# CV-Project2025/Project-NeRF

Hardware: AMD Instinct MI355X
Metric: train rays/sec + 800x800 render FPS, NeRF-Synthetic Lego; PSNR parity (higher is better)
Workload: dtype bf16; 1 GPU; Part 2 vanilla NeRF train step (L10/L4 Fourier, 8x256 skip-4 MLP, view 128), batch sampling included; rays_per_gpu=4096, samples_per_ray=64, global_rays=4096, parallelism=ray-dp1, weights=random init (seed 0), frames=100 x 800x800 RGBA resident in HBM (uniform noise)

## Files before the change

### include/nerf_hip.h

```cpp
#ifndef NERF_HIP_H
#define NERF_HIP_H

#include <stddef.h>
#include <stdint.h>

#ifdef __cplusplus
extern "C" {
#endif

#define NERF_OK 0
#define NERF_EINVAL (-22)
#define NERF_ELAUNCH (-5)
#define NERF_ENOSYS (-38)

#define NERF_ABI_VERSION 11

typedef void* nerf_stream_t;

const char* nerf_last_error(void);
int nerf_abi_version(void);

int nerf_set_option(const char* name, int value);
int nerf_get_option(const char* name, int* value_out);

int nerf_sample_rays(const float* rays_o, const float* rays_d, const float* u,
                     int64_t n_rays, int n_samples, float near_plane, float far_plane,
                     float* z_out, float* pts_out, float* dirs_out, nerf_stream_t stream);

int nerf_gather_rays(const float* images, const float* poses, const int64_t* img_idx, const int64_t* pix_y,
                     const int64_t* pix_x, int64_t batch, int n_images, int H, int W, float focal,
                     float scene_scale, float* rays_o, float* rays_d, float* rgba, nerf_stream_t stream);

int nerf_gather_batch(const float* images, const float* poses, const int64_t* flat_idx, int64_t batch, int n_images,
                      int H, int W, float focal, float scene_scale, const float* bg, float* rays_o, float* rays_d,
                      float* rgba, float* target, nerf_stream_t stream);

int nerf_train_batch(const float* images, const float* poses, int n_images, int H, int W, float focal,
                     float scene_scale, const float* bg, uint64_t seed, uint64_t counter, int64_t batch,
                     int n_samples, float near_plane, float far_plane, int perturb, float* rays_o, float* rays_d,
                     float* rgba, float* target, float* z_out, nerf_stream_t stream);

int nerf_train_batch_shard(const float* images, const float* poses, int n_images, int H, int W, float focal,
                     float scene_scale, const float* bg, uint64_t seed, uint64_t counter, int64_t first_ray, int64_t batch,
                     int n_samples, float near_plane, float far_plane, int perturb, float* rays_o, float* rays_d,
                     float* rgba, float* target, float* z_out, nerf_stream_t stream);

int nerf_active_mask(const float* pts, int64_t n, const uint8_t* binary_grid, int resolution,
                     float bound, uint8_t* mask_out, int64_t* idx_out, nerf_stream_t stream);

int nerf_sample_compact(const float* rays_o, const float* rays_d, const float* u, int64_t n_rays,
                        int n_samples, float near_plane, float far_plane, const uint8_t* binary_grid,
                        int resolution, float bound, float* z_out, int* slot_of_sample, float* pts_compact,
                        float* dirs_compact, unsigned* active_count, nerf_stream_t stream);
int nerf_sample_compact_jitter(const float* rays_o, const float* rays_d, uint64_t seed, uint64_t counter,
                               int64_t n_rays, int n_samples, float near_plane, float far_plane,
                               const uint8_t* binary_grid, int resolution, float bound, float* z_out,
                               int* slot_of_sample, float* pts_compact, float* dirs_compact,
                               unsigned* active_count, nerf_stream_t stream);
int nerf_sample_compact_jitter_shard(const float* rays_o, const float* rays_d, uint64_t seed, uint64_t counter,
                                     int64_t first_ray, int64_t n_rays, int n_samples, float near_plane, float far_plane,
                                     const uint8_t* binary_grid, int resolution, float bound, float* z_out,
                                     int* slot_of_sample, float* pts_compact, float* dirs_compact,
                                     unsigned* active_count, nerf_stream_t stream);
#define NERF_COMPACT_CHAIN_WORDS 40
int nerf_sample_compact_jitter_chain(const float* rays_o, const float* rays_d, uint64_t seed, uint64_t counter,
                                     int64_t first_ray, int64_t n_rays, int n_samples, float near_plane, float far_plane,
                                     const uint8_t* binary_grid, int resolution, float bound, float* z_out,
                                     int* slot_of_sample, float* pts_compact, float* dirs_compact,
                                     unsigned* chain_state, int turn, unsigned* count_host, unsigned seq, nerf_stream_t stream);

int nerf_train_batch_compact(const float* images, const float* poses, int n_images, int H, int W, float focal,
                             float scene_scale, const float* bg, uint64_t seed, uint64_t counter, int64_t first_ray,
                             int64_t batch, int n_samples, float near_plane, float far_plane,
                             const uint8_t* binary_grid, int resolution, float bound, float* rays_o, float* rays_d,
                             float* rgba, float* target, float* z_out, int* slot_of_sample, float* pts_compact,
                             float* dirs_compact, unsigned* active_count, nerf_stream_t stream);
int nerf_train_batch_compact_chain(const float* images, const float* poses, int n_images, int H, int W, float focal,
                                   float scene_scale, const float* bg, uint64_t seed, uint64_t counter, int64_t first_ray,
                                   int64_t batch, int n_samples, float near_plane, float far_plane,
                                   const uint8_t* binary_grid, int resolution, float bound, float* rays_o, float* rays_d,
                                   float* rgba, float* target, float* z_out, int* slot_of_sample, float* pts_compact,
                                   float* dirs_compact, unsigned* chain_state, int turn, unsigned* count_host, unsigned seq,
                                   nerf_stream_t stream);

size_t nerf_sample_compact_ordered_scratch_bytes(int64_t n_rays, int n_samples);
int nerf_sample_compact_ordered(const float* rays_o, const float* rays_d, const float* u, int draw, uint64_t seed, uint64_t counter,
                                int64_t first_ray, int64_t n_rays, int n_samples, float near_plane, float far_plane,
                                const uint8_t* binary_grid, int resolution, float bound, float* z_out, int* slot_of_sample,
                                float* pts_compact, float* dirs_compact, unsigned* active_count, void* scratch,
                                size_t scratch_bytes, nerf_stream_t stream);

int nerf_sample_pdf(const float* z_coarse, const float* weights, const float* u, int64_t n_rays,
                    int n_coarse, int n_fine, float* z_out, nerf_stream_t stream);

int nerf_grid_lattice(float bound, int resolution, float* pts_out, nerf_stream_t stream);
int nerf_grid_update(const float* sigma, float* grid, uint8_t* binary_grid, int64_t n_cells,
                     float decay, int dynamic, float threshold, unsigned long long* active_count,
                     nerf_stream_t stream);

int nerf_fourier_encode(const float* x, int64_t n, int dim, int n_freq, float* out,
                        nerf_stream_t stream);

int nerf_composite_fwd(const float* rgb, const float* sigma, const float* z, const float* rays_d,
                       const float* bg, int64_t bg_rows, const float* extra,
                       int64_t n_rays, int n_samples,
                       float* out_rgb, float* out_depth, float* out_acc,
                       float* extra_map, float* weights_out, nerf_stream_t stream);

int nerf_composite_bwd(const float* rgb, const float* sigma, const float* z, const float* rays_d,
                       const float* bg, int64_t bg_rows, const float* extra,
                       const float* g_rgb, const float* g_depth, const float* g_acc,
                       const float* g_extra, int64_t n_rays, int n_samples,
                       float* d_rgb, float* d_sigma, float* d_extra, nerf_stream_t stream);

int nerf_composite_fwd_indexed(const float* rgb_compact, const float* sigma_compact, const int* slot_of_sample,
                               const float* z, const float* rays_d, const float* bg, int64_t bg_rows,
                               int64_t n_rays, int n_samples, float* out_rgb, float* out_depth,
                               float* out_acc, nerf_stream_t stream);
int nerf_composite_bwd_indexed(const float* rgb_compact, const float* sigma_compact, const int* slot_of_sample,
                               const float* z, const float* rays_d, const float* bg, int64_t bg_rows,
                               const float* g_rgb, const float* g_depth, const float* g_acc, int64_t n_rays,
                               int n_samples, float* d_rgb_compact, float* d_sigma_compact,
                               nerf_stream_t stream);

#define NERF_MLP_PARAM_COUNT 595844

size_t nerf_mlp_packed_bytes(void);
int nerf_mlp_pack(const float* params_f32, void* packed, nerf_stream_t stream);
int nerf_mlp_pack_streams(const float* params_f32, void* packed, int which, nerf_stream_t stream);

size_t nerf_mlp_stash_bytes(int64_t n);
int nerf_mlp_fwd(const void* packed, const float* rays_o, const float* rays_d, const float* z,
                 int64_t n, int n_samples, float* rgb, float* sigma, void* stash,
                 nerf_stream_t stream);

int nerf_mlp_fwd_encoded(const void* packed, const float* x_enc, const float* d_enc, int64_t n, float* rgb,
                         float* sigma, void* stash, nerf_stream_t stream);

size_t nerf_mlp_bwd_workspace_bytes(int64_t n);
int nerf_mlp_bwd(const void* packed, const void* stash, const float* rgb, const float* sigma,
                 const float* d_rgb, const float* d_sigma, int64_t n, float* grads_f32,
                 void* workspace, nerf_stream_t stream);
int nerf_mlp_bwd_dgrad(const void* packed, const void* stash, const float* rgb, const float* sigma,
                       const float* d_rgb, const float* d_sigma, int64_t n, void* workspace,
                       nerf_stream_t stream);
int nerf_mlp_bwd_dgrad_ex(const void* packed, const void* stash, const float* rgb, const float* sigma,
                          const float* d_rgb, const float* d_sigma, int64_t n, void* workspace,
                          const float* amax_dev, nerf_stream_t stream);
int64_t nerf_mlp_wgrad_part_split(void);
int nerf_mlp_bwd_wgrad_part(const void* stash, const void* workspace, int64_t n, float* grads_f32, int part,
                            nerf_stream_t stream);
int nerf_mlp_bwd_wgrad(const void* stash, const void* workspace, int64_t n, float* grads_f32,
                       nerf_stream_t stream);

int nerf_hash_encode_fwd(const float* pts, int64_t n, const float* table, int n_levels,
                         const float* scale_host, const unsigned* res_host, const unsigned* size_host,
                         const unsigned* offset_host, const unsigned* dense_host, float bound,
                         float* out_f32, void* out_nat_bf16, unsigned* idx_out, nerf_stream_t stream);
int nerf_hash_encode_fwd_f16(const float* pts, int64_t n, const void* table_f16, int n_levels,
                         const float* scale_host, const unsigned* res_host, const unsigned* size_host,
                         const unsigned* offset_host, const unsigned* dense_host, float bound,
                         float* out_f32, void* out_nat_bf16, nerf_stream_t stream);
int nerf_hash_encode_fwd_nat(const float* pts, int64_t n, const float* table_f32, const void* table_f16, int n_levels,
                             const float* scale_host, const unsigned* res_host, const unsigned* size_host,
                             const unsigned* offset_host, const unsigned* dense_host, float bound,
                             void* out_nat, int nat_dtype, nerf_stream_t stream);
int nerf_hash_encode_fwd_nat_tables(const float* pts, int64_t n, const void* tables_f16, int n_tables, int64_t table_stride,
                                    int n_levels, const float* scale_host, const unsigned* res_host, const unsigned* size_host,
                                    const unsigned* offset_host, const unsigned* dense_host, float bound, void* out_nat,
                                    int64_t out_stride_bytes, int nat_dtype, nerf_stream_t stream);
int nerf_f32_to_f16(const float* src, void* dst_f16, int64_t n, nerf_stream_t stream);
int nerf_hash_encode_bwd(const float* pts, int64_t n, int n_levels, const float* scale_host,
                         const unsigned* res_host, const unsigned* size_host, const unsigned* offset_host,
                         const unsigned* dense_host, float bound, const float* d_feat, float* d_table,
                         nerf_stream_t stream);
int nerf_hash_encode_bwd_levels(const float* pts, int64_t n, int n_levels, const float* scale_host,
                         const unsigned* res_host, const unsigned* size_host, const unsigned* offset_host,
                         const unsigned* dense_host, float bound, const float* d_feat, float* d_table, int first_level, int end_level,
                         nerf_stream_t stream);
size_t nerf_hash_encode_bwd_workspace_bytes(int64_t n, int n_levels);
int nerf_hash_encode_bwd_ws(const float* pts, int64_t n, int n_levels, const float* scale_host,
                         const unsigned* res_host, const unsigned* size_host, const unsigned* offset_host,
                         const unsigned* dense_host, float bound, const float* d_feat, float* d_table, int first_level, int end_level,
                         void* workspace, size_t workspace_bytes, nerf_stream_t stream);
int nerf_hash_encode_bwd_ws_store(const float* pts, int64_t n, int n_levels, const float* scale_host,
                                  const unsigned* res_host, const unsigned* size_host, const unsigned* offset_host,
                                  const unsigned* dense_host, float bound, const float* d_feat, float* d_table,
                                  int first_level, int end_level, void* workspace, size_t workspace_bytes,
                                  nerf_stream_t stream);
size_t nerf_hash_encode_bwd_tables_workspace_bytes(int64_t n, int n_levels, int n_tables);
int nerf_hash_encode_bwd_ws_store_tables(const float* pts, int64_t n, int n_tables, int64_t table_stride, int n_levels,
                                         const float* scale_host, const unsigned* res_host, const unsigned* size_host,
                                         const unsigned* offset_host, const unsigned* dense_host, float bound,
                                         const float* d_feat, int64_t dfeat_stride, float* d_table, void* workspace,
                                         size_t workspace_bytes, nerf_stream_t stream);
int nerf_hash_encode_bwd_ws_store_tables_spec(const float* pts, int64_t n, int n_tables, int64_t table_stride, int n_levels,
                                              const float* scale_host, const unsigned* res_host, const unsigned* size_host,
                                              const unsigned* offset_host, const unsigned* dense_host, float bound,
                                              const float* d_feat, int64_t dfeat_stride, float* d_table, void* workspace,
                                              size_t workspace_bytes, void* status_host, nerf_stream_t stream);
int nerf_hash_encode_fwd_f16_hist(const float* pts, int64_t n, const void* table_f16, int n_levels,
                                  const float* scale_host, const unsigned* res_host, const unsigned* size_host,
                                  const unsigned* offset_host, const unsigned* dense_host, float bound,
                                  void* out_nat_bf16, void* bwd_workspace, size_t bwd_workspace_bytes, nerf_stream_t stream);
#define NERF_AMAX_WORDS 32
int nerf_hash_encode_bwd_ws_slots(void* workspace, int64_t n, int n_levels, void** amax_bits_out, void** grad_lm_out);
int nerf_hash_encode_bwd_ws_store_precounted(const float* pts, int64_t n, int n_levels, const float* scale_host,
                                             const unsigned* res_host, const unsigned* size_host,
                                             const unsigned* offset_host, const unsigned* dense_host, float bound,
                                             float* d_table, void* workspace, size_t workspace_bytes, nerf_stream_t stream);
int nerf_hash_encode_bwd_spec_begin(void* workspace, nerf_stream_t stream);
int nerf_hash_encode_bwd_ws_store_spec(const float* pts, int64_t n, int n_levels, const float* scale_host,
                                       const unsigned* res_host, const unsigned* size_host, const unsigned* offset_host,
                                       const unsigned* dense_host, float bound, const float* d_feat, float* d_table, void* workspace,
                                       size_t workspace_bytes, void* status_host, nerf_stream_t stream);
int nerf_imlp_bwd_amax(const void* packed, void* workspace, const float* rgb, const float* sigma, const float* d_rgb,
                       const float* d_sigma, int64_t n, float* grads_f32, float* d_feat, void* amax_bits, nerf_stream_t stream);
const void* nerf_hash_encode_bwd_spec_status(const void* workspace);

int nerf_hash_encode_bwd_input(const float* pts, int64_t n, const float* table, int n_levels,
                               const float* scale_host, const unsigned* res_host, const unsigned* size_host,
                               const unsigned* offset_host, const unsigned* dense_host, float bound,
                               const float* d_feat, float* d_pts, nerf_stream_t stream);
int nerf_hash_encode_bwd_input_f16(const float* pts, int64_t n, const void* table_f16, int n_levels,
                                   const float* scale_host, const unsigned* res_host, const unsigned* size_host,
                                   const unsigned* offset_host, const unsigned* dense_host, float bound,
                                   const float* d_feat, float* d_pts, nerf_stream_t stream);
int nerf_hash_encode_bwd_input_f16_accum(const float* pts, int64_t n, const void* table_f16, int n_levels,
                                         const float* scale_host, const unsigned* res_host, const unsigned* size_host,
                                         const unsigned* offset_host, const unsigned* dense_host, float bound,
                                         const float* d_feat, float* d_pts, nerf_stream_t stream);
int nerf_hash_encode_bwd_input_lm_f16(const float* pts, int64_t n, const void* table_f16, int n_levels,
                                      const float* scale_host, const unsigned* res_host, const unsigned* size_host,
                                      const unsigned* offset_host, const unsigned* dense_host, float bound,
                                      const void* grad_lm, float* d_pts, int accumulate, nerf_stream_t stream);


size_t nerf_imlp_packed_bytes(void);
size_t nerf_imlp_workspace_bytes(int64_t n);
size_t nerf_imlp_hash_operand_offset(int64_t n);
int nerf_imlp_pack(const float* params_f32, void* packed, nerf_stream_t stream);
int nerf_imlp_fwd(const void* packed, void* workspace, const float* dirs, int64_t n, float* rgb,
                  float* sigma, int train, nerf_stream_t stream);
int nerf_imlp_fwd_encoded(const void* packed, void* workspace, const float* x_enc, const float* d_enc, int64_t n,
                          float* rgb, float* sigma, int train, nerf_stream_t stream);
int nerf_imlp_bwd(const void* packed, void* workspace, const float* rgb, const float* sigma,
                  const float* d_rgb, const float* d_sigma, int64_t n, float* grads_f32,
                  float* d_feat, nerf_stream_t stream);
int nerf_imlp_bwd_lm(const void* packed, void* workspace, const float* rgb, const float* sigma,
                     const float* d_rgb, const float* d_sigma, int64_t n, float* grads_f32,
                     void* grad_lm, void* amax_bits, nerf_stream_t stream);

size_t nerf_render_rays_workspace_bytes(int64_t chunk_rays, int n_samples);
int nerf_render_rays_fwd(const void* packed, const float* rays_o, const float* rays_d, int64_t n_rays,
                         int n_samples, float near_plane, float far_plane, const float* bg, int64_t bg_rows,
                         int64_t chunk_rays, void* workspace, float* out_rgb, float* out_depth, float* out_acc,
                         nerf_stream_t stream);

size_t nerf_instant_render_workspace_bytes(int64_t chunk_rays, int n_samples);
int nerf_instant_render_rays_fwd(const void* imlp_packed, const float* table_f32, const void* table_f16, int n_levels,
                                 const float* scale_host, const unsigned* res_host, const unsigned* size_host,
                                 const unsigned* offset_host, const unsigned* dense_host, float hash_bound,
                                 const uint8_t* binary_grid, int grid_resolution, float grid_bound,
                                 const float* rays_o, const float* rays_d, int64_t n_rays, int n_samples,
                                 float near_plane, float far_plane, const float* bg, int64_t bg_rows,
                                 int64_t chunk_rays, void* workspace, float* out_rgb, float* out_depth, float* out_acc,
                                 nerf_stream_t stream);

size_t nerf_render_rays_grid_workspace_bytes(int64_t chunk_rays, int n_samples);
int nerf_render_rays_grid_fwd(const void* packed, const uint8_t* binary_grid, int grid_resolution, float grid_bound,
                              const float* rays_o, const float* rays_d, int64_t n_rays, int n_samples,
                              float near_plane, float far_plane, const float* bg, int64_t bg_rows,
                              int64_t chunk_rays, void* workspace, float* out_rgb, float* out_depth, float* out_acc,
                              nerf_stream_t stream);

#define NERF_SUM_WS_FLOATS 12288
int nerf_composite_mse_bwd(const float* rgb, const float* sigma, const int* slot_of_sample, const float* z,
                           const float* rays_d, const float* bg, int64_t bg_rows, const float* target,
                           float loss_weight, int64_t n_rays, int n_samples, float* pred_out, float* loss_accum,
                           float* d_rgb, float* d_sigma, float* amax_accum, float* sum_ws, nerf_stream_t stream);
int nerf_composite_mse_reg_bwd(const float* rgb, const float* sigma, const int* slot_of_sample, const float* z,
                               const float* rays_d, const float* bg, int64_t bg_rows, const float* target,
                               float loss_weight, const float* extra, float reg_weight, int64_t n_rays, int n_samples,
                               float* pred_out, float* extra_map, float* loss_accum, float* reg_accum, float* d_rgb,
                               float* d_sigma, float* d_extra, float* sum_ws, nerf_stream_t stream);

int nerf_adam_step(float* params, const float* grads, float* exp_avg, float* exp_avg_sq,
                   int64_t n, int step, float lr, float beta1, float beta2, float eps,
                   float weight_decay, const float* grad_scale_dev, nerf_stream_t stream);

#define NERF_NORMSQ_WS_FLOATS 4136
int nerf_tv_normsq(const float* params, float* grads, int64_t n, float tv_weight, float grad_scale,
                   float* normsq_dev, nerf_stream_t stream);
int nerf_tv_normsq_accum(const float* params, float* grads, int64_t n, float tv_weight, float grad_scale,
                         float* normsq_dev, nerf_stream_t stream);
int nerf_tv_normsq_accum_tables(const float* params, float* grads, int64_t n, int n_tables, float tv_weight, float grad_scale,
                                float* normsq_dev, nerf_stream_t stream);
int nerf_adamw_clip_step(float* params, const float* grads, float* exp_avg, float* exp_avg_sq, int64_t n,
                         int step, float lr, float beta1, float beta2, float eps, float weight_decay,
                         const float* normsq_dev, float max_norm, float grad_scale, nerf_stream_t stream);
int nerf_adamw_clip_step_shadow(float* params, const float* grads, float* exp_avg, float* exp_avg_sq, int64_t n,
                         int step, float lr, float beta1, float beta2, float eps, float weight_decay,
                         const float* normsq_dev, float max_norm, float grad_scale, void* params_f16_out, nerf_stream_t stream);

size_t nerf_tv_codes_bytes(int64_t n);
int nerf_tv_normsq_codes(const float* params, const float* grads, int64_t n, int n_tables, float tv_weight, float grad_scale,
                         float* normsq_dev, int accumulate, void* tv_codes, nerf_stream_t stream);
int nerf_adamw_clip_step_tv(float* params, const float* grads, float* exp_avg, float* exp_avg_sq, int64_t n, int step, float lr,
                            float beta1, float beta2, float eps, float weight_decay, const float* normsq_dev, float max_norm,
                            float grad_scale, const void* tv_codes, int64_t tv_split, float tv_weight_lo, int64_t seg_lo,
                            float tv_weight_hi, int64_t seg_hi, int64_t lr_split, float lr_hi, void* params_f16_out,
                            nerf_stream_t stream);

int nerf_tv_normsq_codes_piece(const float* params, const float* grads, int64_t n, int64_t table_elems, int halo, float tv_weight,
                               float grad_scale, float* normsq_dev, int accumulate, void* tv_codes, nerf_stream_t stream);
int nerf_adamw_clip_step_tv_piece(float* params, const float* grads, float* exp_avg, float* exp_avg_sq, int64_t n, int step, float lr,
                                  float beta1, float beta2, float eps, float weight_decay, const float* normsq_dev, float max_norm,
                                  float grad_scale, const void* tv_codes, float tv_weight, int64_t table_elems, int halo_lo,
                                  void* params_f16_out, nerf_stream_t stream);

int nerf_clip_adamw_small(float* params, float* grads, float* exp_avg, float* exp_avg_sq, int64_t n, int step, float lr, float beta1,
                          float beta2, float eps, float weight_decay, float max_norm, float grad_scale, float* normsq_out,
                          int zero_grads, nerf_stream_t stream);

int64_t nerf_p4_param_count(void);
size_t nerf_p4_packed_bytes(void);
size_t nerf_p4_workspace_bytes(int64_t n);
size_t nerf_p4_infer_workspace_bytes(int64_t n);
size_t nerf_p4_workspace_offset(int64_t n, int which);
int nerf_p4_pack(const float* params_f32, void* packed, nerf_stream_t stream);
int nerf_p4_sample_inputs(const int* slot_of_sample, const float* pts_compact, const float* ray_times, int64_t n_rays,
                          int n_samples, float coord_noise_std, float time_noise_std, uint64_t seed, uint64_t counter,
                          int64_t first_ray, float* x_deform, float* t_deform, nerf_stream_t stream);
int nerf_p4_deform_fwd(const void* packed, const float* params_f32, void* workspace, const float* pts, const float* t_deform,
                       const float* blend, int64_t n, float* delta_x, float* x_canonical, int train, nerf_stream_t stream);
int nerf_p4_canon_fwd(const void* packed, void* workspace, const float* t_deform, const float* dirs, int64_t n, float* rgb,
                      float* sigma, int train, nerf_stream_t stream);
int nerf_p4_canon_bwd(const void* packed, void* workspace, const float* rgb, const float* sigma, const float* d_rgb,
                      const float* d_sigma, int64_t n, float* grads_f32, void* amax_bits, void* grad_lm, nerf_stream_t stream);
int nerf_p4_deform_bwd(const void* packed, const float* params_f32, void* workspace, const float* d_delta_x, int64_t n,
                       float* grads_f32, void* amax_bits, void* grad_lm, nerf_stream_t stream);

int64_t nerf_p3_deform_param_count(void);
size_t nerf_p3_deform_packed_bytes(void);
size_t nerf_p3_deform_workspace_bytes(int64_t n);
int nerf_p3_deform_pack(const float* params_f32, void* packed, nerf_stream_t stream);
int nerf_p3_deform_fwd(const void* packed, void* workspace, const float* x_code, const float* pts, const float* t_deform,
                       int64_t n, float* delta_x, float* x_canonical, int train, nerf_stream_t stream);
int nerf_p3_deform_bwd(const void* packed, void* workspace, const float* d_delta_x, int64_t n, float* grads_f32,
                       nerf_stream_t stream);

int64_t nerf_p3_canon_param_count(int time_dim);
size_t nerf_p3_canon_packed_bytes(void);
size_t nerf_p3_canon_workspace_bytes(int64_t n);
int nerf_p3_canon_pack(const float* params_f32, int time_dim, void* packed, nerf_stream_t stream);
int nerf_p3_canon_fwd(const void* packed, void* workspace, const float* x, const float* t, const float* dirs, int64_t n,
                      float* rgb, float* sigma, int train, nerf_stream_t stream);
int nerf_p3_canon_bwd(const void* packed, void* workspace, const float* x, const float* rgb, const float* sigma,
                      const float* d_rgb, const float* d_sigma, int64_t n, int time_dim, float* grads_f32, float* d_x,
                      nerf_stream_t stream);

int64_t nerf_p1_param_count(int L_embed, int use_pe, int hidden, int layers);
size_t nerf_p1_packed_bytes(int L_embed, int use_pe, int hidden, int layers);
// ... 37 lines not shown
```

### project-nerf_amd/_lib.py

```python
import ctypes
import os

_HERE = os.path.dirname(os.path.abspath(__file__))
LIB_PATH = os.path.join(_HERE, "libnerf_hip.so")

c_f32p = ctypes.c_void_p
c_ptr = ctypes.c_void_p
i64 = ctypes.c_int64
i32 = ctypes.c_int
f32 = ctypes.c_float
size_t = ctypes.c_size_t

PROTOTYPES = {
    "nerf_last_error": (ctypes.c_char_p, []),
    "nerf_abi_version": (i32, []),
    "nerf_set_option": (i32, [ctypes.c_char_p, i32]),
    "nerf_get_option": (i32, [ctypes.c_char_p, ctypes.POINTER(i32)]),
    "nerf_sample_rays": (i32, [c_ptr, c_ptr, c_ptr, i64, i32, f32, f32, c_ptr, c_ptr, c_ptr, c_ptr]),
    "nerf_gather_rays": (i32, [c_ptr, c_ptr, c_ptr, c_ptr, c_ptr, i64, i32, i32, i32, f32, f32, c_ptr, c_ptr, c_ptr, c_ptr]),
    "nerf_gather_batch": (i32, [c_ptr, c_ptr, c_ptr, i64, i32, i32, i32, f32, f32, c_ptr, c_ptr, c_ptr, c_ptr, c_ptr, c_ptr]),
    "nerf_train_batch": (i32, [c_ptr, c_ptr, i32, i32, i32, f32, f32, c_ptr, ctypes.c_uint64, ctypes.c_uint64, i64, i32, f32, f32,
                               i32, c_ptr, c_ptr, c_ptr, c_ptr, c_ptr, c_ptr]),
    "nerf_train_batch_shard": (i32, [c_ptr, c_ptr, i32, i32, i32, f32, f32, c_ptr, ctypes.c_uint64, ctypes.c_uint64, i64, i64, i32, f32, f32,
                                     i32, c_ptr, c_ptr, c_ptr, c_ptr, c_ptr, c_ptr]),
    "nerf_active_mask": (i32, [c_ptr, i64, c_ptr, i32, f32, c_ptr, c_ptr, c_ptr]),
    "nerf_sample_compact": (i32, [c_ptr, c_ptr, c_ptr, i64, i32, f32, f32, c_ptr, i32, f32, c_ptr, c_ptr, c_ptr, c_ptr, c_ptr, c_ptr]),
    "nerf_sample_compact_jitter": (i32, [c_ptr, c_ptr, ctypes.c_uint64, ctypes.c_uint64, i64, i32, f32, f32, c_ptr, i32, f32,
                                         c_ptr, c_ptr, c_ptr, c_ptr, c_ptr, c_ptr]),
    "nerf_sample_compact_jitter_shard": (i32, [c_ptr, c_ptr, ctypes.c_uint64, ctypes.c_uint64, i64, i64, i32, f32, f32, c_ptr, i32, f32,
                                               c_ptr, c_ptr, c_ptr, c_ptr, c_ptr, c_ptr]),
    "nerf_sample_compact_jitter_chain": (i32, [c_ptr, c_ptr, ctypes.c_uint64, ctypes.c_uint64, i64, i64, i32, f32, f32, c_ptr, i32, f32,
                                               c_ptr, c_ptr, c_ptr, c_ptr, c_ptr, i32, c_ptr, ctypes.c_uint32, c_ptr]),
    "nerf_train_batch_compact": (i32, [c_ptr, c_ptr, i32, i32, i32, f32, f32, c_ptr, ctypes.c_uint64, ctypes.c_uint64, i64, i64, i32, f32, f32,
                                       c_ptr, i32, f32, c_ptr, c_ptr, c_ptr, c_ptr, c_ptr, c_ptr, c_ptr, c_ptr, c_ptr, c_ptr]),
    "nerf_train_batch_compact_chain": (i32, [c_ptr, c_ptr, i32, i32, i32, f32, f32, c_ptr, ctypes.c_uint64, ctypes.c_uint64, i64, i64, i32, f32,
                                             f32, c_ptr, i32, f32, c_ptr, c_ptr, c_ptr, c_ptr, c_ptr, c_ptr, c_ptr, c_ptr, c_ptr, i32, c_ptr,
                                             ctypes.c_uint32, c_ptr]),
    "nerf_composite_fwd_indexed": (i32, [c_ptr, c_ptr, c_ptr, c_ptr, c_ptr, c_ptr, i64, i64, i32, c_ptr, c_ptr, c_ptr, c_ptr]),
    "nerf_composite_bwd_indexed": (i32, [c_ptr, c_ptr, c_ptr, c_ptr, c_ptr, c_ptr, i64, c_ptr, c_ptr, c_ptr, i64, i32, c_ptr, c_ptr, c_ptr]),
    "nerf_sample_pdf": (i32, [c_ptr, c_ptr, c_ptr, i64, i32, i32, c_ptr, c_ptr]),
    "nerf_grid_lattice": (i32, [f32, i32, c_ptr, c_ptr]),
    "nerf_grid_update": (i32, [c_ptr, c_ptr, c_ptr, i64, f32, i32, f32, c_ptr, c_ptr]),
    "nerf_fourier_encode": (i32, [c_ptr, i64, i32, i32, c_ptr, c_ptr]),
    "nerf_composite_fwd": (i32, [c_ptr, c_ptr, c_ptr, c_ptr, c_ptr, i64, c_ptr, i64, i32,
                                 c_ptr, c_ptr, c_ptr, c_ptr, c_ptr, c_ptr]),
    "nerf_composite_bwd": (i32, [c_ptr, c_ptr, c_ptr, c_ptr, c_ptr, i64, c_ptr, c_ptr, c_ptr, c_ptr,
                                 c_ptr, i64, i32, c_ptr, c_ptr, c_ptr, c_ptr]),
    "nerf_render_rays_workspace_bytes": (size_t, [i64, i32]),
    "nerf_render_rays_fwd": (i32, [c_ptr, c_ptr, c_ptr, i64, i32, f32, f32, c_ptr, i64, i64, c_ptr, c_ptr, c_ptr, c_ptr, c_ptr]),
    "nerf_instant_render_workspace_bytes": (size_t, [i64, i32]),
    "nerf_instant_render_rays_fwd": (i32, [c_ptr, c_ptr, c_ptr, i32, c_ptr, c_ptr, c_ptr, c_ptr, c_ptr, f32, c_ptr, i32, f32, c_ptr, c_ptr, i64, i32,
                                           f32, f32, c_ptr, i64, i64, c_ptr, c_ptr, c_ptr, c_ptr, c_ptr]),
    "nerf_render_rays_grid_workspace_bytes": (size_t, [i64, i32]),
    "nerf_render_rays_grid_fwd": (i32, [c_ptr, c_ptr, i32, f32, c_ptr, c_ptr, i64, i32, f32, f32, c_ptr, i64, i64, c_ptr, c_ptr, c_ptr, c_ptr,
                                        c_ptr]),
    "nerf_mlp_packed_bytes": (size_t, []),
    "nerf_mlp_pack": (i32, [c_ptr, c_ptr, c_ptr]),
    "nerf_mlp_pack_streams": (i32, [c_ptr, c_ptr, i32, c_ptr]),
    "nerf_mlp_stash_bytes": (size_t, [i64]),
    "nerf_mlp_fwd": (i32, [c_ptr, c_ptr, c_ptr, c_ptr, i64, i32, c_ptr, c_ptr, c_ptr, c_ptr]),
    "nerf_mlp_fwd_encoded": (i32, [c_ptr, c_ptr, c_ptr, i64, c_ptr, c_ptr, c_ptr, c_ptr]),
    "nerf_mlp_bwd_workspace_bytes": (size_t, [i64]),
    "nerf_mlp_bwd": (i32, [c_ptr, c_ptr, c_ptr, c_ptr, c_ptr, c_ptr, i64, c_ptr, c_ptr, c_ptr]),
    "nerf_mlp_bwd_dgrad": (i32, [c_ptr, c_ptr, c_ptr, c_ptr, c_ptr, c_ptr, i64, c_ptr, c_ptr]),
    "nerf_mlp_bwd_wgrad": (i32, [c_ptr, c_ptr, i64, c_ptr, c_ptr]),
    "nerf_mlp_bwd_dgrad_ex": (i32, [c_ptr, c_ptr, c_ptr, c_ptr, c_ptr, c_ptr, i64, c_ptr, c_ptr, c_ptr]),
    "nerf_composite_mse_bwd": (i32, [c_ptr, c_ptr, c_ptr, c_ptr, c_ptr, c_ptr, i64, c_ptr, f32, i64, i32, c_ptr, c_ptr,
                                     c_ptr, c_ptr, c_ptr, c_ptr, c_ptr]),
    "nerf_mlp_wgrad_part_split": (i64, []),
    "nerf_mlp_bwd_wgrad_part": (i32, [c_ptr, c_ptr, i64, c_ptr, i32, c_ptr]),
    "nerf_hash_encode_fwd": (i32, [c_ptr, i64, c_ptr, i32, c_ptr, c_ptr, c_ptr, c_ptr, c_ptr, f32, c_ptr, c_ptr, c_ptr, c_ptr]),
    "nerf_hash_encode_fwd_f16": (i32, [c_ptr, i64, c_ptr, i32, c_ptr, c_ptr, c_ptr, c_ptr, c_ptr, f32, c_ptr, c_ptr, c_ptr]),
    "nerf_hash_encode_fwd_nat": (i32, [c_ptr, i64, c_ptr, c_ptr, i32, c_ptr, c_ptr, c_ptr, c_ptr, c_ptr, f32, c_ptr, i32, c_ptr]),
    "nerf_hash_encode_fwd_nat_tables": (i32, [c_ptr, i64, c_ptr, i32, i64, i32, c_ptr, c_ptr, c_ptr, c_ptr, c_ptr, f32, c_ptr, i64, i32, c_ptr]),
    "nerf_f32_to_f16": (i32, [c_ptr, c_ptr, i64, c_ptr]),
    "nerf_hash_encode_bwd": (i32, [c_ptr, i64, i32, c_ptr, c_ptr, c_ptr, c_ptr, c_ptr, f32, c_ptr, c_ptr, c_ptr]),
    "nerf_hash_encode_bwd_levels": (i32, [c_ptr, i64, i32, c_ptr, c_ptr, c_ptr, c_ptr, c_ptr, f32, c_ptr, c_ptr, i32, i32, c_ptr]),
    "nerf_hash_encode_bwd_workspace_bytes": (size_t, [i64, i32]),
    "nerf_hash_encode_bwd_ws": (i32, [c_ptr, i64, i32, c_ptr, c_ptr, c_ptr, c_ptr, c_ptr, f32, c_ptr, c_ptr, i32, i32, c_ptr, size_t, c_ptr]),
    "nerf_hash_encode_bwd_ws_store": (i32, [c_ptr, i64, i32, c_ptr, c_ptr, c_ptr, c_ptr, c_ptr, f32, c_ptr, c_ptr, i32, i32, c_ptr, size_t, c_ptr]),
    "nerf_hash_encode_bwd_tables_workspace_bytes": (size_t, [i64, i32, i32]),
    "nerf_hash_encode_bwd_ws_store_tables": (i32, [c_ptr, i64, i32, i64, i32, c_ptr, c_ptr, c_ptr, c_ptr, c_ptr, f32, c_ptr, i64, c_ptr, c_ptr, size_t, c_ptr]),
    "nerf_hash_encode_bwd_ws_store_tables_spec": (i32, [c_ptr, i64, i32, i64, i32, c_ptr, c_ptr, c_ptr, c_ptr, c_ptr, f32, c_ptr, i64, c_ptr, c_ptr, size_t,
                                                        c_ptr, c_ptr]),
    "nerf_hash_encode_fwd_f16_hist": (i32, [c_ptr, i64, c_ptr, i32, c_ptr, c_ptr, c_ptr, c_ptr, c_ptr, f32, c_ptr, c_ptr, size_t, c_ptr]),
    "nerf_hash_encode_bwd_ws_slots": (i32, [c_ptr, i64, i32, ctypes.POINTER(c_ptr), ctypes.POINTER(c_ptr)]),
    "nerf_hash_encode_bwd_ws_store_precounted": (i32, [c_ptr, i64, i32, c_ptr, c_ptr, c_ptr, c_ptr, c_ptr, f32, c_ptr, c_ptr, size_t, c_ptr]),
    "nerf_hash_encode_bwd_spec_begin": (i32, [c_ptr, c_ptr]),
    "nerf_hash_encode_bwd_ws_store_spec": (i32, [c_ptr, i64, i32, c_ptr, c_ptr, c_ptr, c_ptr, c_ptr, f32, c_ptr, c_ptr, c_ptr, size_t, c_ptr, c_ptr]),
    "nerf_imlp_bwd_amax": (i32, [c_ptr, c_ptr, c_ptr, c_ptr, c_ptr, c_ptr, i64, c_ptr, c_ptr, c_ptr, c_ptr]),
    "nerf_hash_encode_bwd_spec_status": (c_ptr, [c_ptr]),
    "nerf_imlp_bwd_lm": (i32, [c_ptr, c_ptr, c_ptr, c_ptr, c_ptr, c_ptr, i64, c_ptr, c_ptr, c_ptr, c_ptr]),
    "nerf_hash_encode_bwd_input": (i32, [c_ptr, i64, c_ptr, i32, c_ptr, c_ptr, c_ptr, c_ptr, c_ptr, f32, c_ptr, c_ptr, c_ptr]),
    "nerf_hash_encode_bwd_input_f16": (i32, [c_ptr, i64, c_ptr, i32, c_ptr, c_ptr, c_ptr, c_ptr, c_ptr, f32, c_ptr, c_ptr, c_ptr]),
    "nerf_hash_encode_bwd_input_f16_accum": (i32, [c_ptr, i64, c_ptr, i32, c_ptr, c_ptr, c_ptr, c_ptr, c_ptr, f32, c_ptr, c_ptr, c_ptr]),
    "nerf_hash_encode_bwd_input_lm_f16": (i32, [c_ptr, i64, c_ptr, i32, c_ptr, c_ptr, c_ptr, c_ptr, c_ptr, f32, c_ptr, c_ptr, i32, c_ptr]),
    "nerf_imlp_packed_bytes": (size_t, []),
    "nerf_imlp_workspace_bytes": (size_t, [i64]),
    "nerf_imlp_hash_operand_offset": (size_t, [i64]),
    "nerf_imlp_pack": (i32, [c_ptr, c_ptr, c_ptr]),
    "nerf_imlp_fwd": (i32, [c_ptr, c_ptr, c_ptr, i64, c_ptr, c_ptr, i32, c_ptr]),
    "nerf_imlp_fwd_encoded": (i32, [c_ptr, c_ptr, c_ptr, c_ptr, i64, c_ptr, c_ptr, i32, c_ptr]),
    "nerf_imlp_bwd": (i32, [c_ptr, c_ptr, c_ptr, c_ptr, c_ptr, c_ptr, i64, c_ptr, c_ptr, c_ptr]),
    "nerf_adam_step": (i32, [c_ptr, c_ptr, c_ptr, c_ptr, i64, i32, f32, f32, f32, f32, f32, c_ptr, c_ptr]),
    "nerf_tv_normsq": (i32, [c_ptr, c_ptr, i64, f32, f32, c_ptr, c_ptr]),
    "nerf_tv_normsq_accum": (i32, [c_ptr, c_ptr, i64, f32, f32, c_ptr, c_ptr]),
    "nerf_tv_normsq_accum_tables": (i32, [c_ptr, c_ptr, i64, i32, f32, f32, c_ptr, c_ptr]),
    "nerf_composite_mse_reg_bwd": (i32, [c_ptr, c_ptr, c_ptr, c_ptr, c_ptr, c_ptr, i64, c_ptr, f32, c_ptr, f32, i64, i32, c_ptr, c_ptr,
                                         c_ptr, c_ptr, c_ptr, c_ptr, c_ptr, c_ptr, c_ptr]),
    "nerf_sample_compact_ordered_scratch_bytes": (size_t, [i64, i32]),
    "nerf_sample_compact_ordered": (i32, [c_ptr, c_ptr, c_ptr, i32, ctypes.c_uint64, ctypes.c_uint64, i64, i64, i32, f32, f32, c_ptr, i32, f32,
                                          c_ptr, c_ptr, c_ptr, c_ptr, c_ptr, c_ptr, size_t, c_ptr]),
    "nerf_p4_param_count": (i64, []),
    "nerf_p4_packed_bytes": (size_t, []),
    "nerf_p4_workspace_bytes": (size_t, [i64]),
    "nerf_p4_infer_workspace_bytes": (size_t, [i64]),
    "nerf_p4_workspace_offset": (size_t, [i64, i32]),
    "nerf_p4_pack": (i32, [c_ptr, c_ptr, c_ptr]),
    "nerf_p4_sample_inputs": (i32, [c_ptr, c_ptr, c_ptr, i64, i32, f32, f32, ctypes.c_uint64, ctypes.c_uint64, i64, c_ptr, c_ptr, c_ptr]),
    "nerf_p4_deform_fwd": (i32, [c_ptr, c_ptr, c_ptr, c_ptr, c_ptr, c_ptr, i64, c_ptr, c_ptr, i32, c_ptr]),
    "nerf_p4_canon_fwd": (i32, [c_ptr, c_ptr, c_ptr, c_ptr, i64, c_ptr, c_ptr, i32, c_ptr]),
    "nerf_p4_canon_bwd": (i32, [c_ptr, c_ptr, c_ptr, c_ptr, c_ptr, c_ptr, i64, c_ptr, c_ptr, c_ptr, c_ptr]),
    "nerf_p4_deform_bwd": (i32, [c_ptr, c_ptr, c_ptr, c_ptr, i64, c_ptr, c_ptr, c_ptr, c_ptr]),
    "nerf_p3_deform_param_count": (i64, []),
    "nerf_p3_deform_packed_bytes": (size_t, []),
    "nerf_p3_deform_workspace_bytes": (size_t, [i64]),
    "nerf_p3_deform_pack": (i32, [c_ptr, c_ptr, c_ptr]),
    "nerf_p3_deform_fwd": (i32, [c_ptr, c_ptr, c_ptr, c_ptr, c_ptr, i64, c_ptr, c_ptr, i32, c_ptr]),
    "nerf_p3_deform_bwd": (i32, [c_ptr, c_ptr, c_ptr, i64, c_ptr, c_ptr]),
    "nerf_p3_canon_param_count": (i64, [i32]),
    "nerf_p3_canon_packed_bytes": (size_t, []),
    "nerf_p3_canon_workspace_bytes": (size_t, [i64]),
    "nerf_p3_canon_pack": (i32, [c_ptr, i32, c_ptr, c_ptr]),
    "nerf_p3_canon_fwd": (i32, [c_ptr, c_ptr, c_ptr, c_ptr, c_ptr, i64, c_ptr, c_ptr, i32, c_ptr]),
    "nerf_p3_canon_bwd": (i32, [c_ptr, c_ptr, c_ptr, c_ptr, c_ptr, c_ptr, c_ptr, i64, i32, c_ptr, c_ptr, c_ptr]),
    "nerf_p1_param_count": (i64, [i32, i32, i32, i32]),
    "nerf_p1_packed_bytes": (size_t, [i32, i32, i32, i32]),
    "nerf_p1_workspace_bytes": (size_t, [i64, i32, i32, i32, i32]),
    "nerf_p1_pack": (i32, [c_ptr, i32, i32, i32, i32, c_ptr, c_ptr]),
    "nerf_p1_fwd": (i32, [c_ptr, c_ptr, i64, i32, i32, i32, i32, c_ptr, c_ptr]),
    "nerf_p1_fwd_loss_bwd": (i32, [c_ptr, c_ptr, c_ptr, c_ptr, c_ptr, i64, i32, i32, i32, i32, c_ptr, c_ptr, c_ptr]),
    "nerf_p2_param_count": (i64, [i32] * 6),
    "nerf_p2_packed_bytes": (size_t, [i32] * 6),
    "nerf_p2_workspace_bytes": (size_t, [i64] + [i32] * 6),
    "nerf_p2_pack": (i32, [c_ptr] + [i32] * 6 + [c_ptr, c_ptr]),
    "nerf_p2_fwd": (i32, [c_ptr, c_ptr, c_ptr, c_ptr, i64, i32] + [i32] * 6 + [c_ptr, c_ptr, c_ptr]),
    "nerf_p2_fwd_train": (i32, [c_ptr, c_ptr, c_ptr, c_ptr, c_ptr, i64, i32] + [i32] * 6 + [c_ptr, c_ptr, c_ptr]),
    "nerf_p2_bwd": (i32, [c_ptr, c_ptr, c_ptr, c_ptr, c_ptr, c_ptr, i64] + [i32] * 6 + [c_ptr, c_ptr]),
    "nerf_imlp_shape_param_count": (i64, [i32] * 3),
    "nerf_imlp_shape_packed_bytes": (size_t, [i32] * 3),
    "nerf_imlp_shape_workspace_bytes": (size_t, [i64] + [i32] * 3),
    "nerf_imlp_shape_hash_operand_offset": (size_t, [i64] + [i32] * 3),
    "nerf_imlp_shape_pack": (i32, [c_ptr] + [i32] * 3 + [c_ptr, c_ptr]),
    "nerf_imlp_shape_fwd": (i32, [c_ptr, c_ptr, c_ptr, i64] + [i32] * 3 + [c_ptr, c_ptr, i32, c_ptr]),
    "nerf_imlp_shape_bwd": (i32, [c_ptr, c_ptr, c_ptr, c_ptr, c_ptr, c_ptr, i64] + [i32] * 3 + [c_ptr, c_ptr, c_ptr]),
    "nerf_tv_codes_bytes": (size_t, [i64]),
    "nerf_tv_normsq_codes": (i32, [c_ptr, c_ptr, i64, i32, f32, f32, c_ptr, i32, c_ptr, c_ptr]),
    "nerf_clip_adamw_small": (i32, [c_ptr, c_ptr, c_ptr, c_ptr, i64, i32, f32, f32, f32, f32, f32, f32, f32, c_ptr, i32, c_ptr]),
    "nerf_adamw_clip_step_tv": (i32, [c_ptr, c_ptr, c_ptr, c_ptr, i64, i32, f32, f32, f32, f32, f32, c_ptr, f32, f32, c_ptr, i64, f32, i64,
                                      f32, i64, i64, f32, c_ptr, c_ptr]),
    "nerf_tv_normsq_codes_piece": (i32, [c_ptr, c_ptr, i64, i64, i32, f32, f32, c_ptr, i32, c_ptr, c_ptr]),
    "nerf_adamw_clip_step_tv_piece": (i32, [c_ptr, c_ptr, c_ptr, c_ptr, i64, i32, f32, f32, f32, f32, f32, c_ptr, f32, f32, c_ptr, f32, i64, i32,
                                            c_ptr, c_ptr]),
    "nerf_adamw_clip_step": (i32, [c_ptr, c_ptr, c_ptr, c_ptr, i64, i32, f32, f32, f32, f32, f32, c_ptr, f32, f32, c_ptr]),
    "nerf_adamw_clip_step_shadow": (i32, [c_ptr, c_ptr, c_ptr, c_ptr, i64, i32, f32, f32, f32, f32, f32, c_ptr, f32, f32, c_ptr, c_ptr]),
}

ABI_VERSION = 11

_lib = None


class NerfHipError(RuntimeError):
    pass


def load():
    global _lib
    if _lib is not None:
        return _lib
    if not os.path.exists(LIB_PATH):
        raise NerfHipError(
            f"{LIB_PATH} not found: build it with `python project-nerf_amd/build.py` "
            "(hipcc --offload-arch=gfx950).  There is no fallback path.")
    import torch
    lib = ctypes.CDLL(LIB_PATH, mode=ctypes.RTLD_GLOBAL)
    for name, (res, args) in PROTOTYPES.items():
        fn = getattr(lib, name)
        fn.restype = res
        fn.argtypes = args
    if lib.nerf_abi_version() != ABI_VERSION:
        raise NerfHipError(f"ABI version mismatch: {LIB_PATH} reports {lib.nerf_abi_version()}, this binding was written against "
                           f"{ABI_VERSION} (rebuild with `python project-nerf_amd/build.py`)")
    _lib = lib
    return lib


NORMSQ_WS_FLOATS = 4136
COMPACT_CHAIN_WORDS = 40
SUM_WS_FLOATS = 12288


def set_option(name: str, value: int) -> None:
    check(load().nerf_set_option(name.encode(), int(value)), f"nerf_set_option({name})")


def get_option(name: str) -> int:
    out = i32(0)
    check(load().nerf_get_option(name.encode(), ctypes.byref(out)), f"nerf_get_option({name})")
    return out.value


def check(code, what):
    if code != 0:
        msg = load().nerf_last_error().decode("utf-8", "replace")
        raise NerfHipError(f"{what} failed ({code}): {msg}")
```

### project-nerf_amd/csrc/adam.hip

```cpp
#include "common.h"

namespace nerf {

typedef float f4 __attribute__((ext_vector_type(4)));

__device__ __forceinline__ void adam_update(float& p, float g, float& m, float& v, float lr, float beta1, float beta2,
                                            float eps, float wd, float inv_bc1, float inv_sqrt_bc2) {
  float pi = p;
  if (wd != 0.0f) pi *= (1.0f - lr * wd);
  const float mi = beta1 * m + (1.0f - beta1) * g;
  const float vi = beta2 * v + (1.0f - beta2) * g * g;
  m = mi;
  v = vi;
  p = pi - (lr * inv_bc1) * (mi / (sqrtf(vi) * inv_sqrt_bc2 + eps));
}

template <bool VEC>
__device__ __forceinline__ void adam_sweep(float* __restrict__ p, const float* __restrict__ g, float* __restrict__ m,
                                           float* __restrict__ v, int64_t n, float gs, float lr, float beta1, float beta2,
                                           float eps, float wd, float inv_bc1, float inv_sqrt_bc2, _Float16* __restrict__ shadow = nullptr) {
  const int64_t tid = blockIdx.x * (int64_t)blockDim.x + threadIdx.x, stride = (int64_t)gridDim.x * blockDim.x;
  const int64_t n4 = VEC ? n / 4 : 0;
  for (int64_t i = tid; i < n4; i += stride) {
    f4 pp = reinterpret_cast<f4*>(p)[i], mm = reinterpret_cast<f4*>(m)[i], vv = reinterpret_cast<f4*>(v)[i];
    const f4 gg = reinterpret_cast<const f4*>(g)[i];
#pragma unroll
    for (int e = 0; e < 4; ++e) {
      float pe = pp[e], me = mm[e], ve = vv[e];
      adam_update(pe, gg[e] * gs, me, ve, lr, beta1, beta2, eps, wd, inv_bc1, inv_sqrt_bc2);
      pp[e] = pe; mm[e] = me; vv[e] = ve;
    }
    reinterpret_cast<f4*>(m)[i] = mm;
    reinterpret_cast<f4*>(v)[i] = vv;
    reinterpret_cast<f4*>(p)[i] = pp;
    if (shadow != nullptr) {
      typedef _Float16 h4 __attribute__((ext_vector_type(4)));
      h4 hh = {(_Float16)pp[0], (_Float16)pp[1], (_Float16)pp[2], (_Float16)pp[3]};
      reinterpret_cast<h4*>(shadow)[i] = hh;
    }
  }
  for (int64_t i = 4 * n4 + tid; i < n; i += stride) {
    adam_update(p[i], g[i] * gs, m[i], v[i], lr, beta1, beta2, eps, wd, inv_bc1, inv_sqrt_bc2);
    if (shadow != nullptr) shadow[i] = (_Float16)p[i];
  }
}

template <bool VEC>
__global__ void __launch_bounds__(256)
adam_kernel(float* __restrict__ p, const float* __restrict__ g, float* __restrict__ m,
            float* __restrict__ v, int64_t n, float lr, float beta1, float beta2, float eps, float wd,
            float inv_bc1, float inv_sqrt_bc2, const float* __restrict__ grad_scale) {
  adam_sweep<VEC>(p, g, m, v, n, grad_scale ? *grad_scale : 1.0f, lr, beta1, beta2, eps, wd, inv_bc1, inv_sqrt_bc2);
}

__host__ inline bool aligned16(const void* a, const void* b, const void* c, const void* d) {
  return (((uintptr_t)a | (uintptr_t)b | (uintptr_t)c | (uintptr_t)d) & 15) == 0;
}

}

extern "C" int nerf_adam_step(float* params, const float* grads, float* exp_avg, float* exp_avg_sq,
                              int64_t n, int step, float lr, float beta1, float beta2, float eps,
                              float weight_decay, const float* grad_scale_dev, nerf_stream_t stream) {
  NERF_REQUIRE(n >= 0 && step >= 1, "nerf_adam_step: n=%lld step=%d", (long long)n, step);
  if (n == 0) return NERF_OK;
  NERF_REQUIRE(params && grads && exp_avg && exp_avg_sq, "nerf_adam_step: NULL pointer");
  const double bc1 = 1.0 - pow((double)beta1, step), bc2 = 1.0 - pow((double)beta2, step);
  int64_t blocks = (n / 4 + 255) / 256 + 1;
  if (blocks > 2048) blocks = 2048;
  if (nerf::aligned16(params, grads, exp_avg, exp_avg_sq))
    hipLaunchKernelGGL(nerf::adam_kernel<true>, dim3((int)blocks), dim3(256), 0, nerf::as_stream(stream), params,
                       grads, exp_avg, exp_avg_sq, n, lr, beta1, beta2, eps, weight_decay,
                       (float)(1.0 / bc1), (float)(1.0 / sqrt(bc2)), grad_scale_dev);
  else
    hipLaunchKernelGGL(nerf::adam_kernel<false>, dim3((int)blocks), dim3(256), 0, nerf::as_stream(stream), params,
                       grads, exp_avg, exp_avg_sq, n, lr, beta1, beta2, eps, weight_decay,
                       (float)(1.0 / bc1), (float)(1.0 / sqrt(bc2)), grad_scale_dev);
  return nerf::check_launch("nerf_adam_step");
}

namespace nerf {

__device__ __forceinline__ float sgn(float x) { return (x > 0.0f) - (x < 0.0f); }

__device__ __forceinline__ float tv_term(float prev, float cur, float next, bool has_prev, bool has_next) {
  float t = 0.0f;
  if (has_prev) t += sgn(cur - prev);
  if (has_next) t -= sgn(next - cur);
  return t;
}

template <bool VEC>
__global__ void __launch_bounds__(256)
tv_normsq_kernel(const float* __restrict__ p, float* __restrict__ g, int64_t n, float tv_scale, float grad_scale,
                 float* __restrict__ normsq, int64_t seg) {
  auto starts = [seg](int64_t e) { return e == 0 || e == seg || e == 2 * seg || e == 3 * seg; };
  const bool rewrite = tv_scale != 0.0f || grad_scale != 1.0f;
  float local = 0.0f;
// ... 477 lines not shown
```

### project-nerf_amd/csrc/api.cpp

```cpp
#include <stdlib.h>
#include <string.h>
#include <mutex>
#include "common.h"

namespace nerf {
static thread_local char g_err[512] = "";

int fail(int code, const char* fmt, ...) {
  va_list ap;
  va_start(ap, fmt);
  vsnprintf(g_err, sizeof(g_err), fmt, ap);
  va_end(ap);
  return code;
}

struct OptionSlot { const char* name; const char* env; int Options::*field; };
static const OptionSlot kSlots[] = {
    {"chain_legacy", "NERF_CHAIN_LEGACY", &Options::chain_legacy},
    {"fwd_cycles", "NERF_FWD_CYCLES", &Options::fwd_cycles},
    {"wgrad_overhead", "NERF_WGRAD_OVH", &Options::wgrad_overhead},
    {"wgrad_bw_x16", "NERF_WGRAD_BW", &Options::wgrad_bw_x16},
    {"wgrad_fixed", "NERF_WGRAD_FIXED", &Options::wgrad_fixed},
    {"wgrad_debug", "NERF_WGRAD_DEBUG", &Options::wgrad_debug},
    {"wgrad_small_span", "NERF_WGRAD_SMALL_SPAN", &Options::wgrad_small_span},
    {"wgrad_small_cap", "NERF_WGRAD_SMALL_CAP", &Options::wgrad_small_cap},
    {"wgrad_only", "NERF_WGRAD_ONLY", &Options::wgrad_only},
    {"hash_bwd_only_level", "NERF_HASH_BWD_ONLY_LEVEL", &Options::hash_bwd_only_level},
    {"hash_bwd_atomic", "NERF_HASH_BWD_ATOMIC", &Options::hash_bwd_atomic},
    {"wgrad_atomic", "NERF_WGRAD_ATOMIC", &Options::wgrad_atomic},
    {"wgrad_k16", "NERF_WGRAD_K16", &Options::wgrad_k16},
    {"wgrad_big_only", "NERF_WGRAD_BIG_ONLY", &Options::wgrad_big_only},
    {"infer_shape32", "NERF_INFER_SHAPE32", &Options::infer_shape32},
    {"infer64", "NERF_INFER64", &Options::infer64},
    {"stash_fp8", "NERF_STASH_FP8", &Options::stash_fp8},
    {"chain_grid", "NERF_CHAIN_GRID", &Options::chain_grid},
    {"wgrad_grid", "NERF_WGRAD_GRID", &Options::wgrad_grid},
    {"hash_fwd_lds_kb", "NERF_HASH_FWD_LDS_KB", &Options::hash_fwd_lds_kb},
    {"hash_xcd", "NERF_HASH_XCD", &Options::hash_xcd},
    {"composite_wgs_per_cu", "NERF_COMPOSITE_WGS", &Options::composite_wgs_per_cu},
    {"deterministic", "NERF_DETERMINISTIC", &Options::deterministic},
    {"tv_blocks", "NERF_TV_BLOCKS", &Options::tv_blocks},
};

Options& options() {
  static Options o;
  static std::once_flag once;
  std::call_once(once, [] {
    for (const OptionSlot& s : kSlots)
      if (const char* v = getenv(s.env)) o.*(s.field) = (*v == 0) ? 1 : atoi(v);
  });
  return o;
}

namespace {
constexpr int kMaxDevices = 64, kMaxKernels = 64;
struct DeviceFacts {
  int n_cu = 0;
  int n_kernels = 0;
  const void* kernels[kMaxKernels];
};
DeviceFacts g_dev[kMaxDevices];
std::mutex g_dev_mutex;
}

int device_cu_count(int* n_cu) {
  int dev = 0;
  if (hipGetDevice(&dev) != hipSuccess || dev < 0 || dev >= kMaxDevices) return fail(NERF_ELAUNCH, "cannot query the current device");
  std::lock_guard<std::mutex> lock(g_dev_mutex);
  if (g_dev[dev].n_cu == 0) {
    hipDeviceProp_t prop;
    if (hipGetDeviceProperties(&prop, dev) != hipSuccess) return fail(NERF_ELAUNCH, "cannot query device %d", dev);
    g_dev[dev].n_cu = prop.multiProcessorCount;
  }
  *n_cu = g_dev[dev].n_cu;
  return NERF_OK;
}

int ensure_dynamic_lds(const void* kernel, int bytes, const char* what) {
  int dev = 0;
  if (hipGetDevice(&dev) != hipSuccess || dev < 0 || dev >= kMaxDevices) return fail(NERF_ELAUNCH, "cannot query the current device");
  std::lock_guard<std::mutex> lock(g_dev_mutex);
  DeviceFacts& d = g_dev[dev];
  for (int i = 0; i < d.n_kernels; ++i)
    if (d.kernels[i] == kernel) return NERF_OK;
  if (hipFuncSetAttribute(kernel, hipFuncAttributeMaxDynamicSharedMemorySize, bytes) != hipSuccess)
    return fail(NERF_ELAUNCH, "%s: cannot raise the dynamic LDS limit to %d on device %d", what, bytes, dev);
  if (d.n_kernels < kMaxKernels) d.kernels[d.n_kernels++] = kernel;
  return NERF_OK;
}
}

extern "C" const char* nerf_last_error(void) { return nerf::g_err; }
extern "C" int nerf_abi_version(void) { return NERF_ABI_VERSION; }

extern "C" int nerf_set_option(const char* name, int value) {
  NERF_REQUIRE(name != nullptr, "nerf_set_option: NULL name");
  for (const nerf::OptionSlot& s : nerf::kSlots)
    if (strcmp(s.name, name) == 0) {
      nerf::options().*(s.field) = value;
      return NERF_OK;
    }
  return nerf::fail(NERF_EINVAL, "nerf_set_option: unknown option '%s'", name);
}

extern "C" int nerf_get_option(const char* name, int* value) {
  NERF_REQUIRE(name != nullptr && value != nullptr, "nerf_get_option: NULL argument");
  for (const nerf::OptionSlot& s : nerf::kSlots)
    if (strcmp(s.name, name) == 0) {
      *value = nerf::options().*(s.field);
      return NERF_OK;
    }
  return nerf::fail(NERF_EINVAL, "nerf_get_option: unknown option '%s'", name);
// ... 2 lines not shown
```

### project-nerf_amd/csrc/common.h

```cpp
#pragma once
#include <hip/hip_runtime.h>
#include <stdarg.h>
#include <stdint.h>
#include <stdio.h>
#include "../../include/nerf_hip.h"

namespace nerf {

constexpr int kWave = 64;

int fail(int code, const char* fmt, ...);

inline int check_launch(const char* what) {
  hipError_t e = hipGetLastError();
  if (e != hipSuccess) return fail(NERF_ELAUNCH, "%s: %s", what, hipGetErrorString(e));
  return NERF_OK;
}

inline hipStream_t as_stream(nerf_stream_t s) { return reinterpret_cast<hipStream_t>(s); }

struct Options {
  int chain_legacy = 0;
  int fwd_cycles = 0;
  int wgrad_overhead = 98304;
  int wgrad_bw_x16 = 192;
  int wgrad_fixed = 2000;
  int wgrad_debug = 0;
  int wgrad_small_span = 32;
  int wgrad_small_cap = 3;
  int wgrad_only = -1;
  int hash_bwd_only_level = -1;
  int wgrad_big_only = 0;
  int wgrad_k16 = 0;
  int wgrad_atomic = 0;
  int hash_bwd_atomic = 0;
  int infer_shape32 = 0;
  int infer64 = 1;
  int stash_fp8 = 0;
  int chain_grid = 0;
  int wgrad_grid = 0;
  int composite_wgs_per_cu = 2;
  int hash_xcd = 1;
  int hash_fwd_lds_kb = 36;
  int tv_blocks = 0;
  int deterministic = 0;
};
Options& options();

int device_cu_count(int* n_cu);
int ensure_dynamic_lds(const void* kernel, int bytes, const char* what);

int hash_fwd_counted(const float* pts, const unsigned* count, int64_t capacity, const float* table_f32, const void* table_f16,
                     int n_levels, const float* scale_host, const unsigned* res_host, const unsigned* size_host,
                     const unsigned* offset_host, const unsigned* dense_host, float bound, void* out_nat, nerf_stream_t stream);
int imlp_fwd_counted(const void* packed, const void* hash_nat, const float* dirs, const unsigned* count, int64_t capacity, float* rgb,
                     float* sigma, nerf_stream_t stream);
int mlp_fwd_counted(const void* packed, const float* pts, const float* dirs, const unsigned* count, int64_t capacity, float* rgb,
                    float* sigma, nerf_stream_t stream);

#define NERF_REQUIRE(cond, ...) \
  do {                          \
    if (!(cond)) return ::nerf::fail(NERF_EINVAL, __VA_ARGS__); \
  } while (0)

__device__ __forceinline__ uint32_t squares32(uint64_t ctr, uint64_t key) {
  uint64_t x = ctr * key, y = x, z = y + key;
  x = x * x + y; x = (x >> 32) | (x << 32);
  x = x * x + z; x = (x >> 32) | (x << 32);
  x = x * x + y; x = (x >> 32) | (x << 32);
  return (uint32_t)((x * x + z) >> 32);
}

inline uint64_t squares_key(uint64_t seed) {
  uint64_t key = seed + 0x9E3779B97F4A7C15ull;
  key = (key ^ (key >> 30)) * 0xBF58476D1CE4E5B9ull;
  key = (key ^ (key >> 27)) * 0x94D049BB133111EBull;
  return (key ^ (key >> 31)) | 1ull;
}
__device__ __forceinline__ float squares_uniform(uint64_t counter, uint64_t index, uint64_t key) {
  return (float)(squares32((counter << 40) + index, key) >> 8) * 5.9604644775390625e-08f;
}

__device__ __forceinline__ float mul_rn(float a, float b) {
#pragma clang fp contract(off)
  return a * b;
}
__device__ __forceinline__ float add_rn(float a, float b) {
#pragma clang fp contract(off)
  return a + b;
}
__device__ __forceinline__ float sub_rn(float a, float b) {
#pragma clang fp contract(off)
  return a - b;
}

template <int N>
__device__ __forceinline__ float dpp_row_shr(float v, float identity) {
  return __builtin_bit_cast(float, __builtin_amdgcn_update_dpp(__builtin_bit_cast(int, identity),
                                                              __builtin_bit_cast(int, v),
                                                              0x110 + N, 0xF, 0xF, false));
}
template <int N>
__device__ __forceinline__ float dpp_row_shl(float v, float identity) {
  return __builtin_bit_cast(float, __builtin_amdgcn_update_dpp(__builtin_bit_cast(int, identity),
                                                              __builtin_bit_cast(int, v),
                                                              0x100 + N, 0xF, 0xF, false));
}
__device__ __forceinline__ float lane_read(float v, int lane) {
  return __builtin_bit_cast(float, __builtin_amdgcn_readlane(__builtin_bit_cast(int, v), lane));
}

__device__ __forceinline__ float wave_inclusive_prod(float v) {
  v *= dpp_row_shr<1>(v, 1.0f);
  v *= dpp_row_shr<2>(v, 1.0f);
  v *= dpp_row_shr<4>(v, 1.0f);
  v *= dpp_row_shr<8>(v, 1.0f);
  const int lane = __lane_id();
// ... 86 lines not shown
```

### project-nerf_amd/csrc/composite.hip

```cpp
#include "common.h"

namespace nerf {

constexpr int kMaxPerLane = 16;

template <int K>
struct RayCtx {
  float e[K];
  float alpha[K];
  float q[K];
  float T[K];
  float z[K];
  float delta[K];
};

__device__ __forceinline__ int64_t row_of(const int* __restrict__ slots, int64_t dense_index) {
  return slots == nullptr ? dense_index : (int64_t)slots[dense_index];
}

template <int K>
__device__ __forceinline__ void ray_setup(const float* __restrict__ sigma, const float* __restrict__ z,
                                          const float* __restrict__ rays_d, const int* __restrict__ slots,
                                          int64_t r, int S, int lane, RayCtx<K>& c, float* sig_out, int64_t* row_out) {
  const float dx = rays_d[r * 3 + 0], dy = rays_d[r * 3 + 1], dz = rays_d[r * 3 + 2];
// ... 95 lines not shown
      out_rgb[r * 3 + 2] = a2;
      out_depth[r] = ad;
      out_acc[r] = aw;
      if (extra_map != nullptr) {
        extra_map[r * 3 + 0] = x0;
        extra_map[r * 3 + 1] = x1;
        extra_map[r * 3 + 2] = x2;
      }
    }
  }
}

template <int K>
__global__ void __launch_bounds__(256)
composite_bwd_kernel(const float* __restrict__ rgb, const float* __restrict__ sigma,
                     const float* __restrict__ z, const float* __restrict__ rays_d,
                     const float* __restrict__ bg, int64_t bg_rows, const float* __restrict__ extra,
                     const float* __restrict__ g_rgb, const float* __restrict__ g_depth,
                     const float* __restrict__ g_acc, const float* __restrict__ g_extra,
                     const int* __restrict__ slots, int64_t R, int S,
                     float* __restrict__ d_rgb, float* __restrict__ d_sigma, float* __restrict__ d_extra) {
  const int lane = threadIdx.x & 63;
  const int64_t wave = (blockIdx.x * (int64_t)blockDim.x + threadIdx.x) >> 6;
  const int64_t nwave = ((int64_t)gridDim.x * blockDim.x) >> 6;
  for (int64_t r = wave; r < R; r += nwave) {
    RayCtx<K> c;
    float sg[K];
    int64_t row[K];
    ray_setup<K>(sigma, z, rays_d, slots, r, S, lane, c, sg, row);
    const float gr0 = g_rgb[r * 3 + 0], gr1 = g_rgb[r * 3 + 1], gr2 = g_rgb[r * 3 + 2];
    const float gd = g_depth ? g_depth[r] : 0.0f;
    float ga = g_acc ? g_acc[r] : 0.0f;
    if (bg != nullptr) {
      const float* b = bg + (bg_rows > 1 ? r * 3 : 0);
      ga -= gr0 * b[0] + gr1 * b[1] + gr2 * b[2];
    }
    float gx0 = 0.f, gx1 = 0.f, gx2 = 0.f;
    if (g_extra != nullptr) { gx0 = g_extra[r * 3 + 0]; gx1 = g_extra[r * 3 + 1]; gx2 = g_extra[r * 3 + 2]; }
    float G[K], w[K];
    float local = 0.0f;
#pragma unroll
    for (int k = 0; k < K; ++k) {
      const int s = lane * K + k;
      G[k] = 0.0f;
      w[k] = 0.0f;
      if (s < S) {
        w[k] = c.alpha[k] * c.T[k];
        float g = gd * c.z[k] + ga;
        if (row[k] >= 0) {
          const float* p = rgb + row[k] * 3;
          g += gr0 * p[0] + gr1 * p[1] + gr2 * p[2];
          float* o = d_rgb + row[k] * 3;
          o[0] = w[k] * gr0;
          o[1] = w[k] * gr1;
          o[2] = w[k] * gr2;
        }
        if (extra != nullptr && g_extra != nullptr && row[k] >= 0) {
          const float* q = extra + row[k] * 3;
          g += gx0 * q[0] + gx1 * q[1] + gx2 * q[2];
          if (d_extra != nullptr) {
            float* oe = d_extra + row[k] * 3;
            oe[0] = w[k] * gx0;
            oe[1] = w[k] * gx1;
            oe[2] = w[k] * gx2;
          }
        }
        G[k] = g;
        local += g * w[k];
      }
    }
    float after = wave_exclusive_suffix_sum(local);
#pragma unroll
    for (int k = K - 1; k >= 0; --k) {
      const int s = lane * K + k;
      if (s < S && row[k] >= 0) {
        const float dalpha = G[k] * c.T[k] - after / c.q[k];
        d_sigma[row[k]] = dalpha * c.delta[k] * c.e[k];
      }
      after += G[k] * w[k];
    }
  }
}

template <int K>
__global__ void __launch_bounds__(256)
composite_mse_bwd_kernel(const float* __restrict__ rgb, const float* __restrict__ sigma, const float* __restrict__ z,
                         const float* __restrict__ rays_d, const float* __restrict__ bg, int64_t bg_rows,
                         const float* __restrict__ target, float loss_weight, const int* __restrict__ slots, int64_t R, int S,
                         float* __restrict__ pred_out, float* __restrict__ loss_out, float* __restrict__ d_rgb,
                         float* __restrict__ d_sigma, float* __restrict__ amax_out,
                         const float* __restrict__ extra, float reg_weight, float* __restrict__ d_extra,
                         float* __restrict__ reg_out, float* __restrict__ extra_map, unsigned* __restrict__ sum_ws) {
  const int lane = threadIdx.x & 63;
  const int64_t wave = (blockIdx.x * (int64_t)blockDim.x + threadIdx.x) >> 6;
  const int64_t nwave = ((int64_t)gridDim.x * blockDim.x) >> 6;
  float loss_local = 0.0f, amax = 0.0f, reg_local = 0.0f;
  for (int64_t r = wave; r < R; r += nwave) {
    RayCtx<K> c;
    float sg[K];
    int64_t row[K];
    ray_setup<K>(sigma, z, rays_d, slots, r, S, lane, c, sg, row);
    float col[K][3], w[K];
    float a0 = 0.f, a1 = 0.f, a2 = 0.f, aw = 0.f;
    float m0 = 0.f, m1 = 0.f, m2 = 0.f;
#pragma unroll
    for (int k = 0; k < K; ++k) {
      const int s = lane * K + k;
      w[k] = 0.0f;
      col[k][0] = col[k][1] = col[k][2] = 0.0f;
      if (s < S) {
        w[k] = c.alpha[k] * c.T[k];
        if (row[k] >= 0) {
          const float* p = rgb + row[k] * 3;
          col[k][0] = p[0]; col[k][1] = p[1]; col[k][2] = p[2];
          a0 += w[k] * p[0]; a1 += w[k] * p[1]; a2 += w[k] * p[2];
          if (extra != nullptr) {
            const float* e = extra + row[k] * 3;
            m0 += w[k] * e[0]; m1 += w[k] * e[1]; m2 += w[k] * e[2];
          }
        }
        aw += w[k];
      }
    }
    a0 = wave_sum(a0); a1 = wave_sum(a1); a2 = wave_sum(a2); aw = wave_sum(aw);
    float gm0 = 0.f, gm1 = 0.f, gm2 = 0.f;
    if (extra != nullptr) {
      m0 = wave_sum(m0); m1 = wave_sum(m1); m2 = wave_sum(m2);
      gm0 = 2.0f * reg_weight * m0; gm1 = 2.0f * reg_weight * m1; gm2 = 2.0f * reg_weight * m2;
      if (lane == 0) {
        reg_local += reg_weight * (m0 * m0 + m1 * m1 + m2 * m2);
        if (extra_map != nullptr) { extra_map[r * 3 + 0] = m0; extra_map[r * 3 + 1] = m1; extra_map[r * 3 + 2] = m2; }
      }
    }
    float b0 = 0.f, b1 = 0.f, b2 = 0.f;
    if (bg != nullptr) {
      const float* b = bg + (bg_rows > 1 ? r * 3 : 0);
      b0 = b[0]; b1 = b[1]; b2 = b[2];
      const float rest = 1.0f - aw;
      a0 += rest * b0; a1 += rest * b1; a2 += rest * b2;
    }
    const float e0 = a0 - target[r * 3 + 0], e1 = a1 - target[r * 3 + 1], e2 = a2 - target[r * 3 + 2];
    if (lane == 0) {
      loss_local += (e0 * e0 + e1 * e1 + e2 * e2) * loss_weight;
      if (pred_out != nullptr) { pred_out[r * 3 + 0] = a0; pred_out[r * 3 + 1] = a1; pred_out[r * 3 + 2] = a2; }
    }
    const float gr0 = 2.0f * e0 * loss_weight, gr1 = 2.0f * e1 * loss_weight, gr2 = 2.0f * e2 * loss_weight;
    const float ga = -(gr0 * b0 + gr1 * b1 + gr2 * b2);
    float G[K], local = 0.0f;
#pragma unroll
    for (int k = 0; k < K; ++k) {
      const int s = lane * K + k;
      G[k] = 0.0f;
      if (s < S) {
        float g = ga;
        if (row[k] >= 0) {
          g += gr0 * col[k][0] + gr1 * col[k][1] + gr2 * col[k][2];
          if (extra != nullptr) {
            const float* e = extra + row[k] * 3;
            g += gm0 * e[0] + gm1 * e[1] + gm2 * e[2];
            float* oe = d_extra + row[k] * 3;
            oe[0] = w[k] * gm0; oe[1] = w[k] * gm1; oe[2] = w[k] * gm2;
          }
          float* o = d_rgb + row[k] * 3;
          const float d0 = w[k] * gr0, d1 = w[k] * gr1, d2 = w[k] * gr2;
          o[0] = d0; o[1] = d1; o[2] = d2;
          if (amax_out != nullptr)
            amax = fmaxf(amax, fmaxf(fabsf(d0 * col[k][0] * (1.0f - col[k][0])),
                                     fmaxf(fabsf(d1 * col[k][1] * (1.0f - col[k][1])), fabsf(d2 * col[k][2] * (1.0f - col[k][2])))));
        }
        G[k] = g;
        local += g * w[k];
      }
    }
    float after = wave_exclusive_suffix_sum(local);
#pragma unroll
    for (int k = K - 1; k >= 0; --k) {
      const int s = lane * K + k;
      if (s < S && row[k] >= 0) {
        const float dalpha = G[k] * c.T[k] - after / c.q[k];
        const float ds = dalpha * c.delta[k] * c.e[k];
        d_sigma[row[k]] = ds;
        if (amax_out != nullptr && sg[k] > 0.0f) amax = fmaxf(amax, fabsf(ds));
      }
      after += G[k] * w[k];
    }
  }
  __shared__ float part[12];
  loss_local = wave_sum(loss_local);
  reg_local = wave_sum(reg_local);
#pragma unroll
  for (int off = 32; off > 0; off >>= 1) amax = fmaxf(amax, __shfl_xor(amax, off));
  if (lane == 0) { part[threadIdx.x >> 6] = loss_local; part[4 + (threadIdx.x >> 6)] = amax; part[8 + (threadIdx.x >> 6)] = reg_local; }
  __syncthreads();
  if (sum_ws != nullptr) {
    if (threadIdx.x == 0) {
      float* ws = reinterpret_cast<float*>(sum_ws);
      ws[blockIdx.x] = (part[0] + part[1]) + (part[2] + part[3]);
      ws[gridDim.x + blockIdx.x] = (part[8] + part[9]) + (part[10] + part[11]);
      ws[2 * gridDim.x + blockIdx.x] = fmaxf(fmaxf(part[4], part[5]), fmaxf(part[6], part[7]));
    }
    return;
  }
  if (threadIdx.x == 0) {
    atomicAdd(loss_out, (part[0] + part[1]) + (part[2] + part[3]));
    if (reg_out != nullptr) atomicAdd(reg_out, (part[8] + part[9]) + (part[10] + part[11]));
    if (amax_out != nullptr) {
      const float m = fmaxf(fmaxf(part[4], part[5]), fmaxf(part[6], part[7]));
      if (m == m && m < 3.0e38f) atomicMax(reinterpret_cast<unsigned*>(amax_out), __builtin_bit_cast(unsigned, m));
    }
  }
}

__global__ void __launch_bounds__(256) composite_sums_kernel(const float* __restrict__ ws, int n_blocks, float* __restrict__ loss_out,
                                                             float* __restrict__ reg_out, float* __restrict__ amax_out) {
  __shared__ float part[3][4];
  float s0 = 0.0f, s1 = 0.0f, m = 0.0f;
  for (int b = threadIdx.x; b < n_blocks; b += 256) {
    s0 += ws[b];
    s1 += ws[n_blocks + b];
    const float v = ws[2 * n_blocks + b];
    if (v == v && v < 3.0e38f) m = fmaxf(m, v);
  }
  s0 = wave_sum(s0);
  s1 = wave_sum(s1);
#pragma unroll
  for (int off = 32; off > 0; off >>= 1) m = fmaxf(m, __shfl_xor(m, off));
  if ((threadIdx.x & 63) == 0) { part[0][threadIdx.x >> 6] = s0; part[1][threadIdx.x >> 6] = s1; part[2][threadIdx.x >> 6] = m; }
  __syncthreads();
  if (threadIdx.x == 0) {
    *loss_out += (part[0][0] + part[0][1]) + (part[0][2] + part[0][3]);
    if (reg_out != nullptr) *reg_out += (part[1][0] + part[1][1]) + (part[1][2] + part[1][3]);
    if (amax_out != nullptr) *amax_out = fmaxf(*amax_out, fmaxf(fmaxf(part[2][0], part[2][1]), fmaxf(part[2][2], part[2][3])));
  }
}

static int per_lane(int S) {
  const int k = (S + 63) / 64;
  return k <= 4 ? k : (k <= 6 ? 6 : (k <= 8 ? 8 : (k <= 12 ? 12 : 16)));
}

}

using namespace nerf;

#define DISPATCH_K(K, KERNEL, ...)                                                        \
  switch (K) {                                                                            \
    case 1: hipLaunchKernelGGL(KERNEL<1>, grid, dim3(256), 0, as_stream(stream), __VA_ARGS__); break; \
    case 2: hipLaunchKernelGGL(KERNEL<2>, grid, dim3(256), 0, as_stream(stream), __VA_ARGS__); break; \
    case 3: hipLaunchKernelGGL(KERNEL<3>, grid, dim3(256), 0, as_stream(stream), __VA_ARGS__); break; \
    case 4: hipLaunchKernelGGL(KERNEL<4>, grid, dim3(256), 0, as_stream(stream), __VA_ARGS__); break; \
    case 6: hipLaunchKernelGGL(KERNEL<6>, grid, dim3(256), 0, as_stream(stream), __VA_ARGS__); break; \
    case 8: hipLaunchKernelGGL(KERNEL<8>, grid, dim3(256), 0, as_stream(stream), __VA_ARGS__); break; \
    case 12: hipLaunchKernelGGL(KERNEL<12>, grid, dim3(256), 0, as_stream(stream), __VA_ARGS__); break; \
    default: hipLaunchKernelGGL(KERNEL<16>, grid, dim3(256), 0, as_stream(stream), __VA_ARGS__); break; \
  }

static int composite_fwd_impl(const float* rgb, const float* sigma, const float* z, const float* rays_d,
                              const float* bg, int64_t bg_rows, const float* extra, const int* slots,
                              int64_t n_rays, int n_samples, float* out_rgb, float* out_depth, float* out_acc,
                              float* extra_map, float* weights_out, nerf_stream_t stream) {
  NERF_REQUIRE(n_rays >= 0 && n_samples >= 1 && n_samples <= 64 * kMaxPerLane,
               "nerf_composite_fwd: n_rays=%lld n_samples=%d (max %d)", (long long)n_rays, n_samples,
               64 * kMaxPerLane);
  if (n_rays == 0) return NERF_OK;
  NERF_REQUIRE(rgb && sigma && z && rays_d && out_rgb && out_depth && out_acc,
               "nerf_composite_fwd: NULL pointer");
  NERF_REQUIRE(bg == nullptr || bg_rows == 1 || bg_rows == n_rays, "nerf_composite_fwd: bg_rows=%lld",
               (long long)bg_rows);
  NERF_REQUIRE((extra == nullptr) == (extra_map == nullptr), "nerf_composite_fwd: extra/extra_map mismatch");
  int64_t blocks = (n_rays + 3) / 4;
  if (blocks > 256 * 8) blocks = 256 * 8;
  const dim3 grid((int)blocks);
  DISPATCH_K(per_lane(n_samples), composite_fwd_kernel, rgb, sigma, z, rays_d, bg, bg_rows, extra, slots, n_rays,
             n_samples, out_rgb, out_depth, out_acc, extra_map, weights_out);
  return check_launch("nerf_composite_fwd");
}

extern "C" int nerf_composite_fwd(const float* rgb, const float* sigma, const float* z,
                                  const float* rays_d, const float* bg, int64_t bg_rows,
                                  const float* extra, int64_t n_rays, int n_samples, float* out_rgb,
                                  float* out_depth, float* out_acc, float* extra_map,
                                  float* weights_out, nerf_stream_t stream) {
  return composite_fwd_impl(rgb, sigma, z, rays_d, bg, bg_rows, extra, nullptr, n_rays, n_samples, out_rgb, out_depth,
                            out_acc, extra_map, weights_out, stream);
}

extern "C" int nerf_composite_fwd_indexed(const float* rgb_compact, const float* sigma_compact, const int* slot_of_sample,
                                          const float* z, const float* rays_d, const float* bg, int64_t bg_rows,
                                          int64_t n_rays, int n_samples, float* out_rgb, float* out_depth,
                                          float* out_acc, nerf_stream_t stream) {
  NERF_REQUIRE(n_rays == 0 || slot_of_sample != nullptr, "nerf_composite_fwd_indexed: slot map is NULL");
  return composite_fwd_impl(rgb_compact, sigma_compact, z, rays_d, bg, bg_rows, nullptr, slot_of_sample, n_rays, n_samples,
                            out_rgb, out_depth, out_acc, nullptr, nullptr, stream);
}

static int composite_bwd_impl(const float* rgb, const float* sigma, const float* z, const float* rays_d,
                              const float* bg, int64_t bg_rows, const float* extra, const float* g_rgb,
                              const float* g_depth, const float* g_acc, const float* g_extra, const int* slots,
                              int64_t n_rays, int n_samples, float* d_rgb, float* d_sigma, float* d_extra,
                              nerf_stream_t stream) {
  NERF_REQUIRE(n_rays >= 0 && n_samples >= 1 && n_samples <= 64 * kMaxPerLane,
               "nerf_composite_bwd: n_rays=%lld n_samples=%d", (long long)n_rays, n_samples);
  if (n_rays == 0) return NERF_OK;
  NERF_REQUIRE(rgb && sigma && z && rays_d && g_rgb && d_rgb && d_sigma, "nerf_composite_bwd: NULL pointer");
  NERF_REQUIRE(bg == nullptr || bg_rows == 1 || bg_rows == n_rays, "nerf_composite_bwd: bg_rows=%lld",
               (long long)bg_rows);
  int64_t blocks = (n_rays + 3) / 4;
  if (blocks > 256 * 8) blocks = 256 * 8;
  const dim3 grid((int)blocks);
  DISPATCH_K(per_lane(n_samples), composite_bwd_kernel, rgb, sigma, z, rays_d, bg, bg_rows, extra, g_rgb,
             g_depth, g_acc, g_extra, slots, n_rays, n_samples, d_rgb, d_sigma, d_extra);
  return check_launch("nerf_composite_bwd");
}

extern "C" int nerf_composite_bwd(const float* rgb, const float* sigma, const float* z,
                                  const float* rays_d, const float* bg, int64_t bg_rows,
                                  const float* extra, const float* g_rgb, const float* g_depth,
                                  const float* g_acc, const float* g_extra, int64_t n_rays,
                                  int n_samples, float* d_rgb, float* d_sigma, float* d_extra,
                                  nerf_stream_t stream) {
  return composite_bwd_impl(rgb, sigma, z, rays_d, bg, bg_rows, extra, g_rgb, g_depth, g_acc, g_extra, nullptr, n_rays,
                            n_samples, d_rgb, d_sigma, d_extra, stream);
}

extern "C" int nerf_composite_bwd_indexed(const float* rgb_compact, const float* sigma_compact, const int* slot_of_sample,
                                          const float* z, const float* rays_d, const float* bg, int64_t bg_rows,
                                          const float* g_rgb, const float* g_depth, const float* g_acc, int64_t n_rays,
                                          int n_samples, float* d_rgb_compact, float* d_sigma_compact,
                                          nerf_stream_t stream) {
  NERF_REQUIRE(n_rays == 0 || slot_of_sample != nullptr, "nerf_composite_bwd_indexed: slot map is NULL");
  return composite_bwd_impl(rgb_compact, sigma_compact, z, rays_d, bg, bg_rows, nullptr, g_rgb, g_depth, g_acc, nullptr,
                            slot_of_sample, n_rays, n_samples, d_rgb_compact, d_sigma_compact, nullptr, stream);
}

static int64_t mse_blocks(int64_t n_rays, bool partials) {
  int n_cu = 256;
  (void)device_cu_count(&n_cu);
  const int per_cu = partials ? 8 : (options().composite_wgs_per_cu < 1 ? 1 : options().composite_wgs_per_cu);
  int64_t cap = (int64_t)n_cu * per_cu;
  if (cap > kOrderedSumMaxBlocks) cap = kOrderedSumMaxBlocks;
  const int64_t blocks = (n_rays + 3) / 4;
  return blocks < cap ? blocks : cap;
}
static int finish_sums(const float* sum_ws, unsigned n_blocks, float* loss, float* reg, float* amax, nerf_stream_t stream) {
  static_assert(NERF_SUM_WS_FLOATS >= 3 * kOrderedSumMaxBlocks, "three partials per workgroup");
  if (sum_ws == nullptr) return NERF_OK;
  hipLaunchKernelGGL(composite_sums_kernel, dim3(1), dim3(256), 0, as_stream(stream), sum_ws, (int)n_blocks, loss, reg, amax);
  return check_launch("nerf_composite_mse_bwd (sums)");
}

extern "C" int nerf_composite_mse_bwd(const float* rgb, const float* sigma, const int* slot_of_sample, const float* z,
                                      const float* rays_d, const float* bg, int64_t bg_rows, const float* target,
                                      float loss_weight, int64_t n_rays, int n_samples, float* pred_out, float* loss_accum,
                                      float* d_rgb, float* d_sigma, float* amax_accum, float* sum_ws, nerf_stream_t stream) {
  NERF_REQUIRE(n_rays >= 0 && n_samples >= 1 && n_samples <= 64 * kMaxPerLane,
               "nerf_composite_mse_bwd: n_rays=%lld n_samples=%d (max %d)", (long long)n_rays, n_samples, 64 * kMaxPerLane);
  if (n_rays == 0) return NERF_OK;
  NERF_REQUIRE(rgb && sigma && z && rays_d && target && loss_accum && d_rgb && d_sigma, "nerf_composite_mse_bwd: NULL pointer");
  NERF_REQUIRE(bg == nullptr || bg_rows == 1 || bg_rows == n_rays, "nerf_composite_mse_bwd: bg_rows=%lld", (long long)bg_rows);
  const dim3 grid((unsigned)mse_blocks(n_rays, sum_ws != nullptr));
  DISPATCH_K(per_lane(n_samples), composite_mse_bwd_kernel, rgb, sigma, z, rays_d, bg, bg_rows, target, loss_weight,
             slot_of_sample, n_rays, n_samples, pred_out, loss_accum, d_rgb, d_sigma, amax_accum,
             (const float*)nullptr, 0.0f, (float*)nullptr, (float*)nullptr, (float*)nullptr, reinterpret_cast<unsigned*>(sum_ws));
  if (int rc = check_launch("nerf_composite_mse_bwd"); rc != NERF_OK) return rc;
  return finish_sums(sum_ws, grid.x, loss_accum, nullptr, amax_accum, stream);
}

extern "C" int nerf_composite_mse_reg_bwd(const float* rgb, const float* sigma, const int* slot_of_sample, const float* z,
                                          const float* rays_d, const float* bg, int64_t bg_rows, const float* target,
                                          float loss_weight, const float* extra, float reg_weight, int64_t n_rays, int n_samples,
                                          float* pred_out, float* extra_map, float* loss_accum, float* reg_accum, float* d_rgb,
                                          float* d_sigma, float* d_extra, float* sum_ws, nerf_stream_t stream) {
  NERF_REQUIRE(n_rays >= 0 && n_samples >= 1 && n_samples <= 64 * kMaxPerLane,
               "nerf_composite_mse_reg_bwd: n_rays=%lld n_samples=%d (max %d)", (long long)n_rays, n_samples, 64 * kMaxPerLane);
  if (n_rays == 0) return NERF_OK;
  NERF_REQUIRE(rgb && sigma && z && rays_d && target && loss_accum && d_rgb && d_sigma && extra && d_extra && reg_accum,
               "nerf_composite_mse_reg_bwd: NULL pointer");
  NERF_REQUIRE(bg == nullptr || bg_rows == 1 || bg_rows == n_rays, "nerf_composite_mse_reg_bwd: bg_rows=%lld", (long long)bg_rows);
  const dim3 grid((unsigned)mse_blocks(n_rays, sum_ws != nullptr));
  DISPATCH_K(per_lane(n_samples), composite_mse_bwd_kernel, rgb, sigma, z, rays_d, bg, bg_rows, target, loss_weight,
             slot_of_sample, n_rays, n_samples, pred_out, loss_accum, d_rgb, d_sigma, (float*)nullptr, extra, reg_weight, d_extra,
             reg_accum, extra_map, reinterpret_cast<unsigned*>(sum_ws));
  if (int rc = check_launch("nerf_composite_mse_reg_bwd"); rc != NERF_OK) return rc;
  return finish_sums(sum_ws, grid.x, loss_accum, reg_accum, nullptr, stream);
}
```

### project-nerf_amd/csrc/mlp_bwd.hip

```cpp
#include "mlp_chain_body.h"
#include "mlp_stash.h"

namespace nerf {
using namespace plan;

struct BwdArgs {
  const char* packed;
  const float* rgb;
  const float* sigma;
  const float* d_rgb;
  const float* d_sigma;
  int64_t n, n_pad;
  const uint4* st_mask;
  __bf16* dsmall;
  __bf16* dhv;
  __bf16* dfeat;
  __bf16* dh;
  float* amax;
  const float* amax_src;
};

__global__ void __launch_bounds__(256) bwd_amax_kernel(const BwdArgs a) {
  float m = 0.0f;
  for (int64_t n = blockIdx.x * 256 + threadIdx.x; n < a.n; n += (int64_t)gridDim.x * 256) {
// ... 11 lines not shown
    if (m == m && m < 3.0e38f) atomicMax(reinterpret_cast<unsigned*>(a.amax), __builtin_bit_cast(unsigned, m));
  }
}

__global__ void __launch_bounds__(kChainThreads, 2) mlp_bwd_kernel(const BwdArgs a) {
  extern __shared__ __attribute__((aligned(16))) char smem[];
  const int tid = threadIdx.x, lane = tid & 63;
  const int wave = __builtin_amdgcn_readfirstlane(tid >> 6);
  const int col = lane & 31, half = lane >> 5;
  chain_dgrad<kPackBwdOff>(a, smem, tid, lane, wave, col, half);
}

}

#include <stddef.h>
#include "mlp_stream_asm.h"

namespace nerf {

static_assert(offsetof(BwdArgs, n_pad) == 48 && offsetof(BwdArgs, st_mask) == 56 && offsetof(BwdArgs, dhv) == 72 &&
              offsetof(BwdArgs, dfeat) == 80 && offsetof(BwdArgs, dh) == 88, "kernarg offsets used by the stream asm");

template <bool IMG16>
__global__ void __launch_bounds__(kChainThreads, 2) mlp_bwd_stream_kernel(const BwdArgs a) {
  extern __shared__ __attribute__((aligned(16))) char smem[];
  const int tid = threadIdx.x, lane = tid & 63;
  const int wave = __builtin_amdgcn_readfirstlane(tid >> 6);
  const int col = lane & 31, half = lane >> 5;

  BwdChain::Ring ring;
  ring.init(a.packed + kPackBwdOff, smem + kBiasLdsBytes, wave, lane);
  ring.template issue<0>(0);
  ring.template issue<1>(1);
  asm volatile("s_waitcnt vmcnt(0)" ::: "memory");
  __syncthreads();

  const unsigned ab0 = lds_addr(smem + kBiasLdsBytes) + 16u * lane, ab1 = ab0 + kRingSlotBytes;
  const unsigned ldsw = __builtin_amdgcn_readfirstlane(lds_addr(smem + kBiasLdsBytes) + 1024u * wave);
  const unsigned voff = 1024u * wave + 16u * lane;
  const char* src = a.packed + kPackBwdOff;
  const void* karg = (const void*)__builtin_amdgcn_kernarg_segment_ptr();

  float gscale = 1.0f;
  if constexpr (!IMG16) {
    set_fp8_saturate();
    const float amax_in = *a.amax_src;
    if (a.amax_src != a.amax && blockIdx.x == 0 && tid == 0) *a.amax = amax_in;
    gscale = __builtin_bit_cast(float, __builtin_amdgcn_readfirstlane(__builtin_bit_cast(int, grad_image_scale(amax_in))));
  }
  const int64_t n_tiles = a.n_pad / kTileSamples;
  for (int64_t tile = blockIdx.x; tile < n_tiles; tile += gridDim.x) {
    const int64_t wave_tile = tile * 8 + wave;
    const int64_t n = wave_tile * kWaveSamples + col;
    const bool live = n < a.n;
    float g0 = 0.f, g1 = 0.f, g2 = 0.f, gs = 0.f;
    if (live) out_derivs(a, n, g0, g1, g2, gs);
    bf16x8 small, in_rgb, in_sigma;
#pragma unroll
    for (int j = 0; j < 8; ++j) small[j] = in_sigma[j] = (__bf16)0.0f;
    if (half == 0) {
      small[0] = (__bf16)g0; small[1] = (__bf16)g1; small[2] = (__bf16)g2; small[3] = (__bf16)gs;
      in_sigma[0] = (__bf16)gs;
    }
    if constexpr (IMG16) stash_nat(a.dsmall, wave_tile, 1, 0, col, half, small);
    else stash_nat8<true>(reinterpret_cast<char*>(a.dsmall), wave_tile, 1, 0, col, half, small, gscale);
    in_rgb = small;
    in_rgb[3] = (__bf16)0.0f;

    const unsigned lane32 = IMG16 ? block_lane_offset(col, half) : block8_lane_offset(col, half);
    const unsigned blk = IMG16 ? 2048u : 1024u;
    const unsigned so8 = (unsigned)wave_tile * (8u * blk) + lane32, so4 = (unsigned)wave_tile * (4u * blk) + lane32;
    const unsigned mo0 = (unsigned)tile * (72u * 512u * 2u) + 2u * tid;
    const bool more = tile + gridDim.x < n_tiles;
    const unsigned mo0n = more ? (unsigned)(tile + gridDim.x) * (72u * 512u * 2u) + 2u * tid : mo0;
    const unsigned first = __builtin_amdgcn_readfirstlane(tile == (int64_t)blockIdx.x ? 1u : 0u);
    if constexpr (IMG16) bwd16_stream_pass(ab0, ab1, in_rgb, in_sigma, src, voff, ldsw, so8, so4, mo0, mo0n, first, karg, gscale);
    else bwd_stream_pass(ab0, ab1, in_rgb, in_sigma, src, voff, ldsw, so8, so4, mo0, mo0n, first, karg, gscale);
  }
  asm volatile("s_waitcnt vmcnt(0)" ::: "memory");
}

}

using namespace nerf;

int nerf_launch_wgrad(const char* stash, const StashLayout& sl, const char* work, const BwdLayout& bl,
                      int64_t n, float* grads, int part, hipStream_t stream, size_t zero_lo, size_t zero_hi);

extern "C" size_t nerf_mlp_bwd_workspace_bytes(int64_t n) { return n > 0 ? bwd_layout(n).total : 0; }

static int launch_dgrad(const void* packed, const void* stash, const float* rgb, const float* sigma,
                        const float* d_rgb, const float* d_sigma, int64_t n, void* workspace,
                        const float* amax_dev, nerf_stream_t stream) {
  NERF_REQUIRE(n > 0 && n < (int64_t)1 << 31, "nerf_mlp_bwd: n=%lld out of range", (long long)n);
  NERF_REQUIRE(packed && stash && rgb && sigma && d_rgb && d_sigma && workspace, "nerf_mlp_bwd: NULL pointer");
  NERF_REQUIRE(((uintptr_t)packed & 255) == 0 && ((uintptr_t)stash & 255) == 0 && ((uintptr_t)workspace & 255) == 0,
               "nerf_mlp_bwd: packed/stash/workspace must be 256-byte aligned");
  const StashLayout sl = stash_layout(n);
  const BwdLayout bl = bwd_layout(n);
  BwdArgs a{};
  a.packed = static_cast<const char*>(packed);
  a.rgb = rgb; a.sigma = sigma; a.d_rgb = d_rgb; a.d_sigma = d_sigma;
  a.n = n; a.n_pad = bl.n_pad;
  a.st_mask = reinterpret_cast<const uint4*>(static_cast<const char*>(stash) + sl.mask);
  char* w = static_cast<char*>(workspace);
  a.dsmall = reinterpret_cast<__bf16*>(w + bl.dsmall);
  a.dhv = reinterpret_cast<__bf16*>(w + bl.dhv);
  a.dfeat = reinterpret_cast<__bf16*>(w + bl.dfeat);
  a.dh = reinterpret_cast<__bf16*>(w + bl.dh);
  a.amax = reinterpret_cast<float*>(w + bl.amax);
  a.amax_src = amax_dev != nullptr ? amax_dev : a.amax;
  int n_cu = 0;
  if (int rc = device_cu_count(&n_cu); rc != NERF_OK) return rc;
  const bool stream_family = chain_use_stream(n, true);
  const void* kernel = stream_family ? (bl.fp8 ? (const void*)mlp_bwd_stream_kernel<false> : (const void*)mlp_bwd_stream_kernel<true>)
                                     : (const void*)mlp_bwd_kernel;
  if (int rc = ensure_dynamic_lds(kernel, kChainLds, "nerf_mlp_bwd"); rc != NERF_OK) return rc;
  const int64_t tiles = bl.n_pad / kTileSamples;
  if (options().chain_grid > 0 && options().chain_grid < n_cu) n_cu = options().chain_grid;
  const int grid = (int)(tiles < n_cu ? tiles : n_cu);
  if (bl.fp8 && amax_dev == nullptr) {
    if (hipMemsetAsync(a.amax, 0, sizeof(float), as_stream(stream)) != hipSuccess)
      return fail(NERF_ELAUNCH, "nerf_mlp_bwd: memset failed");
    const int64_t want = (n + 1023) / 1024;
    hipLaunchKernelGGL(bwd_amax_kernel, dim3((int)(want < 1024 ? want : 1024)), dim3(256), 0, as_stream(stream), a);
  }
  if (stream_family && bl.fp8)
    hipLaunchKernelGGL(mlp_bwd_stream_kernel<false>, dim3(grid), dim3(kChainThreads), kChainLds, as_stream(stream), a);
  else if (stream_family)
    hipLaunchKernelGGL(mlp_bwd_stream_kernel<true>, dim3(grid), dim3(kChainThreads), kChainLds, as_stream(stream), a);
  else
    hipLaunchKernelGGL(mlp_bwd_kernel, dim3(grid), dim3(kChainThreads), kChainLds, as_stream(stream), a);
  return check_launch("nerf_mlp_bwd (dgrad chain)");
}

static int launch_wgrad(const void* stash, const void* workspace, int64_t n, float* grads_f32, int part,
                        nerf_stream_t stream) {
  NERF_REQUIRE(grads_f32 != nullptr, "nerf_mlp_bwd: grads_f32 is NULL");
  NERF_REQUIRE(part >= 0 && part <= 2, "nerf_mlp_bwd_wgrad_part: part=%d (0 all, 1 late layers, 2 early layers)", part);
  const size_t lo = part == 1 ? (size_t)plan::kW4 : 0, hi = part == 2 ? (size_t)plan::kW4 : (size_t)plan::kParamCount;
  if (n == 0) {
    if (hipMemsetAsync(grads_f32 + lo, 0, sizeof(float) * (hi - lo), as_stream(stream)) != hipSuccess)
      return fail(NERF_ELAUNCH, "nerf_mlp_bwd: memset failed");
    return NERF_OK;
  }
  NERF_REQUIRE(stash && workspace, "nerf_mlp_bwd: NULL pointer");
  return nerf_launch_wgrad(static_cast<const char*>(stash), stash_layout(n), static_cast<const char*>(workspace),
                           bwd_layout(n), n, grads_f32, part, as_stream(stream), lo, hi);
}

extern "C" int nerf_mlp_bwd_dgrad(const void* packed, const void* stash, const float* rgb, const float* sigma,
                                  const float* d_rgb, const float* d_sigma, int64_t n, void* workspace,
                                  nerf_stream_t stream) {
  if (n == 0) return NERF_OK;
  return launch_dgrad(packed, stash, rgb, sigma, d_rgb, d_sigma, n, workspace, nullptr, stream);
}

extern "C" int nerf_mlp_bwd_dgrad_ex(const void* packed, const void* stash, const float* rgb, const float* sigma,
                                     const float* d_rgb, const float* d_sigma, int64_t n, void* workspace,
                                     const float* amax_dev, nerf_stream_t stream) {
  if (n == 0) return NERF_OK;
  return launch_dgrad(packed, stash, rgb, sigma, d_rgb, d_sigma, n, workspace, amax_dev, stream);
}

extern "C" int nerf_mlp_bwd_wgrad(const void* stash, const void* workspace, int64_t n, float* grads_f32,
                                  nerf_stream_t stream) {
  return launch_wgrad(stash, workspace, n, grads_f32, 0, stream);
}

extern "C" int64_t nerf_mlp_wgrad_part_split(void) { return plan::kW4; }
// ... 17 lines not shown
```

### project-nerf_amd/csrc/mlp_pack.hip

```cpp
#include "common.h"
#include "mlp_plan.h"

namespace nerf {
using namespace plan;

struct FragTable {
  int v[kFwdFrags + kBwdFrags];
};

constexpr FragTable make_frag_table() {
  FragTable t{};
  int f = 0;
  for (int kind = 0; kind < kNumKinds; ++kind) {
    const int ks = step_ks(kind);
    for (int m = 0; m < step_of(kind).mt; ++m)
      for (int k = 0; k < ks; ++k) t.v[f++] = (kind << 16) | (m << 8) | k;
  }
  return t;
}
__constant__ FragTable g_frag_table = make_frag_table();

__device__ __forceinline__ int src_index(int kind, int row, int k, bool nat) {
  if (kind <= F_PTS7) {
    const int l = kind;
    const int in_dim = pts_in_dim(l);
    int col;
    if (l == 0) col = k < 63 ? k : -1;
    else if (l == 4) col = nat ? (k < 63 ? 256 + k : -1) : k;
    else col = k;
    return col < 0 ? -1 : pts_weight_off(l) + row * in_dim + col;
  }
  switch (kind) {
    case F_HEAD: return row < 256 ? kWFeat + row * 256 + k : (row == 256 ? kWSigma + k : -1);
    case F_VIEW: return nat ? (k < 27 ? kWView + row * 283 + 256 + k : -1) : kWView + row * 283 + k;
    case F_RGB: return row < 3 ? kWRgb + row * 128 + k : -1;
    case B_RGB: return k < 3 ? kWRgb + k * 128 + row : -1;
    case B_VIEW: return kWView + k * 283 + row;
    case B_HEAD: return nat ? (k == 0 ? kWSigma + row : -1) : kWFeat + k * 256 + row;
    default: {
      const int l = 7 - (kind - B_PTS7);
      return pts_weight_off(l) + k * pts_in_dim(l) + row;
    }
  }
}

__global__ void __launch_bounds__(256) pack16_kernel(const float* __restrict__ params, __bf16* __restrict__ packed_fwd16) {
  const int total = kFwdFrags * 64;
  for (int t = blockIdx.x * blockDim.x + threadIdx.x; t < total; t += gridDim.x * blockDim.x) {
    const int frag = t >> 6, lane = t & 63;
    const int desc = g_frag_table.v[frag];
    const int kind = desc >> 16, mt = (desc >> 8) & 0xFF, ks = desc & 0xFF;
    const Step st = step_of(kind);
    const int row = mt * 32 + 16 * (ks & 1) + (lane & 15), q = lane >> 4;
    const bool nat = ks >= st.ks_acc;
    const int kk = nat ? (ks - st.ks_acc) >> 1 : ks >> 1;
    typedef __bf16 bf16x8 __attribute__((ext_vector_type(8)));
    bf16x8 out;
#pragma unroll
    for (int j = 0; j < 8; ++j) {
      const int k = nat ? 32 * kk + 8 * q + j : 32 * kk + 16 * (j >> 2) + 4 * q + (j & 3);
      const int src = src_index(kind, row, k, nat);
      out[j] = (__bf16)(src >= 0 ? params[src] : 0.0f);
    }
    *reinterpret_cast<bf16x8*>(packed_fwd16 + (size_t)frag * 512 + lane * 8) = out;
  }
}

__global__ void __launch_bounds__(256)
pack_kernel(const float* __restrict__ params, __bf16* __restrict__ packed_fwd,
            __bf16* __restrict__ packed_bwd, float* __restrict__ bias) {
  const int total = (kFwdFrags + kBwdFrags) * 64;
  for (int t = blockIdx.x * blockDim.x + threadIdx.x; t < total; t += gridDim.x * blockDim.x) {
    const int frag = t >> 6, lane = t & 63;
    const int desc = g_frag_table.v[frag];
    const int kind = desc >> 16, mt = (desc >> 8) & 0xFF, ks = desc & 0xFF;
    const Step st = step_of(kind);
    const int row = mt * 32 + (lane & 31), h = lane >> 5;
    const bool nat = ks >= st.ks_acc;
    typedef __bf16 bf16x8 __attribute__((ext_vector_type(8)));
    bf16x8 out;
#pragma unroll
    for (int j = 0; j < 8; ++j) {
      const int k = frag_column(nat ? ks - st.ks_acc : ks, h, j, nat);
      const int src = src_index(kind, row, k, nat);
      out[j] = (__bf16)(src >= 0 ? params[src] : 0.0f);
    }
    __bf16* dst = frag < kFwdFrags ? packed_fwd + (size_t)frag * 512 : packed_bwd + (size_t)(frag - kFwdFrags) * 512;
    *reinterpret_cast<bf16x8*>(dst + lane * 8) = out;
  }
  for (int i = blockIdx.x * blockDim.x + threadIdx.x; i < kBiasFloats; i += gridDim.x * blockDim.x) {
    float b = 0.0f;
    if (i < 2048) b = params[pts_bias_off(i >> 8) + (i & 255)];
    else if (i < 2048 + 288) { const int r = i - 2048; b = r < 256 ? params[kBFeat + r] : (r == 256 ? params[kBSigma] : 0.0f); }
    else if (i < 2048 + 288 + 128) b = params[kBView + (i - 2048 - 288)];
    else { const int r = i - 2048 - 288 - 128; b = r < 3 ? params[kBRgb + r] : 0.0f; }
    bias[i] = b;
  }
}

}

extern "C" size_t nerf_mlp_packed_bytes(void) { return nerf::plan::kPackBytes; }

extern "C" int nerf_mlp_pack_streams(const float* params_f32, void* packed, int which, nerf_stream_t stream) {
  using namespace nerf;
  NERF_REQUIRE(params_f32 && packed, "nerf_mlp_pack: NULL pointer");
  NERF_REQUIRE(((uintptr_t)packed & 255) == 0, "nerf_mlp_pack: packed buffer must be 256-byte aligned");
  NERF_REQUIRE(which >= 1 && which <= 3, "nerf_mlp_pack_streams: which=%d (1 training streams + biases, 2 inference stream, 3 all)", which);
  char* base = static_cast<char*>(packed);
  if (which & 1)
    hipLaunchKernelGGL(pack_kernel, dim3(512), dim3(256), 0, as_stream(stream), params_f32,
                       reinterpret_cast<__bf16*>(base + plan::kPackFwdOff),
                       reinterpret_cast<__bf16*>(base + plan::kPackBwdOff),
                       reinterpret_cast<float*>(base + plan::kPackBiasOff));
  if (which & 2)
    hipLaunchKernelGGL(pack16_kernel, dim3(304), dim3(256), 0, as_stream(stream), params_f32,
                       reinterpret_cast<__bf16*>(base + plan::kPackFwd16Off));
  return check_launch("nerf_mlp_pack");
}

extern "C" int nerf_mlp_pack(const float* params_f32, void* packed, nerf_stream_t stream) {
  return nerf_mlp_pack_streams(params_f32, packed, 3, stream);
}
```

### project-nerf_amd/csrc/mlp_wgrad.h

```cpp
#pragma once
#include <hip/hip_runtime.h>
#include <stdint.h>

namespace nerf {

constexpr int kMaxJobs = 12;
constexpr int kWgStages = 4;
constexpr int kWgStageA = 16 * 1024, kWgStageB = 16 * 1024, kWgStageN = 4 * 1024;
constexpr int kWgStageBytes = kWgStageA + kWgStageB + kWgStageN;
constexpr int kWgLds = kWgStages * kWgStageBytes;
constexpr int kWgScratch = 256;
constexpr int kMaxTiles = 10;
constexpr size_t kSmallSlabBytes = 8u << 20;

struct WgradJob {
  const char* a;
  const char* b_acc;
  const char* b_nat;
  int a_bytes;
  int b_acc_bytes, b_nat_bytes;
  int a_nat;
  int mt_a;
  int nt_acc, nt_nat, ones;
  int split_n;
  int kind;
  int w_off, w_ld;
  int o_row0, o_valid;
  int acc_valid, acc_col0;
  int nat_valid, nat_col0;
  int bias_off, bias_nat_col;
  const char* a2;
  int w2_off, bias2_off, o2_row, n2;
  long long cost0;
  int cost;
  long long slab_off;
  int part0, n_parts, p_stride;
};

struct WgradArgs {
  WgradJob jobs[kMaxJobs];
  int n_jobs;
  int wave_tiles;
  long long total_cost;
  float* grads;
  float* slab;
  int slab_accumulate;
  const float* amax;
  int k16;
  int debug;
};

static inline WgradJob make_job(const char* w, size_t a_off, int a_bytes, int mt_a, size_t b_off, int nt_acc, size_t bn_off, int nt_nat,
                                int kind) {
  WgradJob j{};
  j.a = w + a_off; j.a_bytes = a_bytes; j.mt_a = mt_a;
  if (nt_acc) { j.b_acc = w + b_off; j.b_acc_bytes = nt_acc * 2048; j.nt_acc = nt_acc; }
  if (nt_nat) { j.b_nat = w + bn_off; j.b_nat_bytes = nt_nat * 2048; j.nt_nat = nt_nat; }
  j.bias_nat_col = -1; j.kind = kind;
  return j;
}

struct InstantImages { size_t hs1, h16, denc, hc1, hc2, dzs2, dzc1, dzc2, dsmall; };
static inline void instant_common_jobs(WgradArgs& wa, const char* w, const InstantImages& o, int s2, int c1, int c2, int c3) {
  { WgradJob j = make_job(w, o.dzs2, 2048, 1, o.hs1, 2, 0, 0, 7); j.w_off = s2; j.w_ld = 64; j.o_valid = 16; j.acc_valid = 64; wa.jobs[1] = j; }
  { WgradJob j = make_job(w, o.dzc1, 4096, 2, o.h16, 1, o.denc, 1, 8); j.w_off = c1; j.w_ld = 48; j.o_valid = 64; j.acc_valid = 16; j.nat_valid = 27; j.nat_col0 = 16; wa.jobs[2] = j; }
  { WgradJob j = make_job(w, o.dzc2, 4096, 2, o.hc1, 2, 0, 0, 7); j.w_off = c2; j.w_ld = 64; j.o_valid = 64; j.acc_valid = 64; wa.jobs[3] = j; }
  { WgradJob j = make_job(w, o.dsmall, 1024, 1, o.hc2, 2, 0, 0, 9); j.a_nat = 1; j.split_n = 1; j.w_off = c3; j.w_ld = 64; j.o_valid = 3; j.acc_valid = 64; wa.jobs[4] = j; }
}

int wgrad_launch(WgradArgs& args, int64_t n_samples, float* grads, hipStream_t stream, float* slab = nullptr,
                 size_t slab_bytes = 0, size_t zero_lo = 0, size_t zero_hi = 0);

}
```

### project-nerf_amd/csrc/mlp_wgrad.hip

```cpp
#include <stdlib.h>
#include "mlp_chain.h"
#include "mlp_stash.h"
#include "mlp_wgrad.h"

namespace nerf {
using namespace plan;

typedef short s16x4 __attribute__((ext_vector_type(4)));
typedef short s16x8 __attribute__((ext_vector_type(8)));
typedef __attribute__((address_space(3))) s16x4* lds_s16x4_t;

__device__ __forceinline__ void dma_1k(const char* gsrc_lane, unsigned lds_dst) {
  unsigned keep;
  asm volatile("s_mov_b32 %0, m0\n\ts_mov_b32 m0, %2\n\ts_nop 0\n\tglobal_load_lds_dwordx4 %1, off nt\n\ts_mov_b32 m0, %0"
               : "=&s"(keep) : "v"(gsrc_lane), "s"(lds_dst) : "memory");
}

template <int STRIDE>
__device__ __forceinline__ bf16x8 tr_frag(const char* p) {
  const s16x4 lo = __builtin_amdgcn_ds_read_tr16_b64_v4i16((lds_s16x4_t)(p));
  const s16x4 hi = __builtin_amdgcn_ds_read_tr16_b64_v4i16((lds_s16x4_t)(p + STRIDE));
  s16x8 v = {lo[0], lo[1], lo[2], lo[3], hi[0], hi[1], hi[2], hi[3]};
  return __builtin_bit_cast(bf16x8, v);
}

struct BigStage { static constexpr int A = kWgStageA, B = kWgStageB, Bytes = kWgStageBytes; };
struct SmallStage { static constexpr int A = 4096, B = 4096, N = 2048, Bytes = 4096 + 4096 + 2048; };
struct SmallStageP4 { static constexpr int A = 4096, B = 4096, N = 4096, Bytes = 4096 + 4096 + 4096; };
struct NatStage { static constexpr int A = kWgStageA, B = 0, Bytes = kWgStageA + 6 * 1024; };

struct LaneGeo {
  int lane, wave, fhalf, off_acc, off_nat;
  int off_acc8, off_nat8;
};

typedef int i32x2 __attribute__((ext_vector_type(2)));
typedef int i32x8 __attribute__((ext_vector_type(8)));
typedef __attribute__((address_space(3))) i32x2* lds_i32x2_t;
__device__ __forceinline__ long tr_frag8(const char* p) {
  return __builtin_bit_cast(long, __builtin_amdgcn_ds_read_tr8_b64_v2i32((lds_i32x2_t)(p)));
}
__device__ __forceinline__ int phi8(int r) { return (r & 3) + 8 * ((r & 15) >> 2) + 4 * (r >> 4); }

template <int NT_ACC, int NT_NAT, bool ONES, bool SPLIT, bool FP8, int NT>
__device__ __forceinline__ void flush_tiles(const WgradArgs& args, const WgradJob& job, const f32x16 (&acc)[NT], const LaneGeo g,
                                            bool active) {
  const int wave = g.wave, lane = g.lane;
  if (!active || (args.debug & 4)) return;
  const int c32 = lane & 31, hrow = lane >> 5;
  const int m_tile = SPLIT ? 0 : wave;
  const int c_acc = FP8 ? phi8(c32) : c32;
  float w_scale = 1.0f, b_scale = 1.0f;
  if constexpr (FP8) {
    b_scale = grad_image_scale(*args.amax);
    w_scale = b_scale * kActScale;
  }
#pragma unroll
  for (int k = 0; k < NT; ++k) {
    int col = -1, bias_here = 0;
    bool use = true;
    if constexpr (SPLIT) {
      if (k == 0) { use = wave < NT_ACC; const int i = wave * 32 + c_acc; if (i < job.acc_valid) col = job.acc_col0 + i; }
      else { use = ONES && wave == NT_ACC % 8; bias_here = (c32 == 0); }
    } else {
      if (k < NT_ACC) { const int i = k * 32 + c_acc; if (i < job.acc_valid) col = job.acc_col0 + i; }
      else if (k < NT_ACC + NT_NAT) {
        const int i = (k - NT_ACC) * 32 + c32;
        if (i < job.nat_valid) col = job.nat_col0 + i;
        bias_here = (i == job.bias_nat_col);
      } else bias_here = (c32 == 0);
    }
    if (!use) continue;
    const bool ones_tile = SPLIT ? k == 1 : k == NT_ACC + NT_NAT;
    if (args.slab != nullptr) {
      float* tile = args.slab + job.slab_off + (long long)((int)blockIdx.x - job.part0) * job.p_stride;
#pragma unroll
      for (int r = 0; r < 16; ++r) {
        const int row = (r & 3) + 8 * (r >> 2) + 4 * hrow;
        const int o = 32 * m_tile + ((FP8 && !SPLIT) ? phi8(row) : row) - job.o_row0;
        if (o >= 0 && o < job.o_valid) {
          if (col >= 0) tile[o * job.w_ld + col] = acc[k][r] * w_scale;
          if (bias_here) tile[job.o_valid * job.w_ld + o] = acc[k][r] * (ones_tile ? b_scale : w_scale);
        }
      }
      continue;
    }
// ... 475 lines not shown
  const int q8 = i16 >> 1, p8 = i16 & 1;
  g.off_acc8 = 256 * hh + 32 * q8 + 16 * g.fhalf + 8 * p8;
  g.off_nat8 = 512 * g.fhalf + 16 * (8 * hh + q8) + 8 * p8;

  const long long lo = args.total_cost * blockIdx.x / gridDim.x;
  const long long hi = args.total_cost * (blockIdx.x + 1) / gridDim.x;
  for (int j = 0; j < args.n_jobs; ++j) {
    const WgradJob job = args.jobs[j];
    const long long j0 = job.cost0, j1 = job.cost0 + (long long)job.cost * args.wave_tiles;
    if (hi <= j0 || lo >= j1) continue;
    const long long a0 = lo > j0 ? lo - j0 : 0, a1 = (hi < j1 ? hi : j1) - j0;
    const int wt0 = (int)((a0 + job.cost - 1) / job.cost), wt1 = (int)((a1 + job.cost - 1) / job.cost);
    if (wt0 >= wt1) continue;
    if constexpr (FP8) {
      switch (job.kind) {
        case 0: run_job8<8, 0, true>(args, job, wt0, wt1, smem, g); break;
        case 1: run_job8<8, 2, false>(args, job, wt0, wt1, smem, g); break;
        case 2: run_job8<0, 2, false>(args, job, wt0, wt1, smem, g); break;
        case 3: run_job8<8, 1, false>(args, job, wt0, wt1, smem, g); break;
        case 4: run_job<8, 0, true, true, true>(args, job, wt0, wt1, smem, g); break;
        default: run_job<4, 0, true, true, true>(args, job, wt0, wt1, smem, g); break;
      }
    } else {
    switch (job.kind) {
      case 0: run_job16<16, 16, 0, 8, 0, true, false>(args, job, wt0, wt1, smem, g); break;
      case 1: run_job16<16, 16, 4, 8, 2, false, false>(args, job, wt0, wt1, smem, g); break;
      case 2: run_job16<16, 0, 4, 0, 2, false, false>(args, job, wt0, wt1, smem, g); break;
      case 3: run_job16<8, 16, 2, 8, 1, false, false>(args, job, wt0, wt1, smem, g); break;
      case 4: run_job16<1, 16, 0, 8, 0, true, true>(args, job, wt0, wt1, smem, g); break;
      case 5: run_job16<1, 8, 0, 4, 0, true, true>(args, job, wt0, wt1, smem, g); break;
      case 13: run_job16<16, 16, 0, 8, 0, true, false, true>(args, job, wt0, wt1, smem, g); break;
      case 14: run_job16<16, 0, 6, 0, 3, false, false, false, NatStage>(args, job, wt0, wt1, smem, g); break;
      case 6: run_job<0, 1, false, false, false>(args, job, wt0, wt1, smem, g); break;
      case 7: run_job<2, 0, false, false, false>(args, job, wt0, wt1, smem, g); break;
      case 8: run_job<1, 1, false, false, false>(args, job, wt0, wt1, smem, g); break;
      default: run_job<2, 0, false, true, false>(args, job, wt0, wt1, smem, g); break;
    }
    }
  }
}

template <bool P4>
__global__ void __launch_bounds__(512, P4 ? 4 : 6) mlp_wgrad_small_kernel(const WgradArgs args) {
  using Stage = std::conditional_t<P4, SmallStageP4, SmallStage>;
  extern __shared__ __attribute__((aligned(16))) char smem[];
  LaneGeo g;
  g.lane = threadIdx.x & 63;
  g.wave = __builtin_amdgcn_readfirstlane(threadIdx.x >> 6);
  const int grp = g.lane >> 4, i16 = g.lane & 15, q = i16 >> 2, p = i16 & 3;
  const int hh = grp >> 1;
  g.fhalf = grp & 1;
  g.off_acc = 512 * hh + 128 * g.fhalf + 64 * (p & 1) + 16 * q + 8 * (p >> 1);
  g.off_nat = 32 * (8 * hh + q) + 16 * (p >> 1) + 8 * (p & 1) + 1024 * g.fhalf;
  g.off_acc8 = g.off_nat8 = 0;
  const long long lo = args.total_cost * blockIdx.x / gridDim.x;
  const long long hi = args.total_cost * (blockIdx.x + 1) / gridDim.x;
  for (int j = 0; j < args.n_jobs; ++j) {
    const WgradJob job = args.jobs[j];
    const long long j0 = job.cost0, j1 = job.cost0 + (long long)job.cost * args.wave_tiles;
    if (hi <= j0 || lo >= j1) continue;
    const long long a0 = lo > j0 ? lo - j0 : 0, a1 = (hi < j1 ? hi : j1) - j0;
    const int wt0 = (int)((a0 + job.cost - 1) / job.cost), wt1 = (int)((a1 + job.cost - 1) / job.cost);
    if (wt0 >= wt1) continue;
    if constexpr (P4) {
      switch (job.kind) {
        case 10: run_job16<4, 4, 0, 2, 0, true, false, false, Stage>(args, job, wt0, wt1, smem, g); continue;
        case 11: run_job16<4, 4, 2, 2, 1, false, false, false, Stage>(args, job, wt0, wt1, smem, g); continue;
        case 12: run_job16<4, 0, 4, 0, 2, false, false, false, Stage>(args, job, wt0, wt1, smem, g); continue;
        default: break;
      }
    }
    switch (job.kind) {
      case 6: run_job16<4, 0, 2, 0, 1, false, false, false, Stage>(args, job, wt0, wt1, smem, g); break;
      case 7:
        if (job.mt_a == 2) run_job16<4, 4, 0, 2, 0, false, false, false, Stage>(args, job, wt0, wt1, smem, g);
        else run_job16<2, 4, 0, 2, 0, false, false, false, Stage>(args, job, wt0, wt1, smem, g);
        break;
      case 8: run_job16<4, 2, 2, 1, 1, false, false, false, Stage>(args, job, wt0, wt1, smem, g); break;
      default: run_job16<1, 4, 0, 2, 0, false, true, false, Stage>(args, job, wt0, wt1, smem, g); break;
    }
  }
}

__global__ void __launch_bounds__(256) wgrad_reduce_kernel(const WgradArgs args) {
  const WgradJob& job = args.jobs[blockIdx.y];
  const int n_w = job.o_valid * job.w_ld, n_b = n_w + job.o_valid, n_all = n_b + job.n2;
  const float* tile = args.slab + job.slab_off;
  for (int i = blockIdx.x * blockDim.x + threadIdx.x; i < n_all; i += gridDim.x * blockDim.x) {
    float s0 = 0.0f, s1 = 0.0f, s2 = 0.0f, s3 = 0.0f;
    int t = 0;
    for (; t + 4 <= job.n_parts; t += 4) {
      s0 += tile[(long long)(t + 0) * job.p_stride + i];
      s1 += tile[(long long)(t + 1) * job.p_stride + i];
      s2 += tile[(long long)(t + 2) * job.p_stride + i];
      s3 += tile[(long long)(t + 3) * job.p_stride + i];
    }
    for (; t < job.n_parts; ++t) s0 += tile[(long long)t * job.p_stride + i];
    const float sum = (s0 + s1) + (s2 + s3);
    float* dst = i < n_w ? args.grads + job.w_off + i
               : i < n_b ? ((job.ones || job.bias_nat_col >= 0) ? args.grads + job.bias_off + (i - n_w) : nullptr)
               : i < n_all - 1 ? args.grads + job.w2_off + (i - n_b)
                               : args.grads + job.bias2_off;
    if (dst != nullptr) *dst = args.slab_accumulate ? *dst + sum : sum;
  }
}

}

using namespace nerf;

int nerf_launch_wgrad(const char* stash, const StashLayout& sl, const char* work, const BwdLayout& bl,
                      int64_t n, float* grads, int part, hipStream_t stream, size_t zero_lo, size_t zero_hi) {
  WgradArgs args{};
  const size_t np = (size_t)sl.n_pad, eb = sl.fp8 ? 1 : 2;
  if (sl.fp8 != bl.fp8) return fail(NERF_EINVAL, "nerf_mlp_bwd: stash and workspace disagree on the image width");
  args.amax = sl.fp8 ? reinterpret_cast<const float*>(work + bl.amax) : nullptr;
  const char* xenc = stash + sl.xenc;
  const char* denc = stash + sl.denc;
  auto st_h = [&](int l) { return stash + sl.h + (size_t)l * np * 256 * eb; };
  auto dh = [&](int l) { return work + bl.dh + (size_t)l * np * 256 * eb; };
  int nj = 0;
  auto add = [&](WgradJob j) {
    args.jobs[nj++] = j;
  };
  {
    WgradJob j{};
    j.a = dh(0); j.a_bytes = 16384; j.mt_a = 8;
    j.b_nat = xenc; j.b_nat_bytes = 4096; j.nt_nat = 2;
    j.w_off = kW0; j.w_ld = 63; j.o_valid = 256; j.nat_valid = 63; j.nat_col0 = 0;
    j.bias_off = kB0; j.bias_nat_col = 63; j.kind = 2;
    add(j);
  }
  for (int l = 1; l < 8; ++l) {
    WgradJob j{};
    j.a = dh(l); j.a_bytes = 16384; j.mt_a = 8;
    j.b_acc = st_h(l - 1); j.b_acc_bytes = 16384; j.nt_acc = 8;
    j.w_off = pts_weight_off(l); j.w_ld = pts_in_dim(l); j.o_valid = 256; j.acc_valid = 256;
    j.bias_off = pts_bias_off(l);
    if (l == 4) {
      j.b_nat = xenc; j.b_nat_bytes = 4096; j.nt_nat = 2; j.nat_valid = 63; j.nat_col0 = 256; j.bias_nat_col = 63;
      j.kind = 1;
    } else {
      j.ones = 1; j.bias_nat_col = -1; j.kind = 0;
    }
    add(j);
  }
  {
    WgradJob j{};
    j.a = work + bl.dfeat; j.a_bytes = 16384; j.mt_a = 8;
    j.b_acc = st_h(7); j.b_acc_bytes = 16384; j.nt_acc = 8; j.ones = 1; j.bias_nat_col = -1;
    j.w_off = kWFeat; j.w_ld = 256; j.o_valid = 256; j.acc_valid = 256; j.bias_off = kBFeat; j.kind = 0;
    if (!sl.fp8) {
      j.a2 = work + bl.dsmall; j.w2_off = kWSigma; j.bias2_off = kBSigma; j.o2_row = 3; j.n2 = 257; j.kind = 13;
    }
    add(j);
  }
  if (sl.fp8) {
    WgradJob j{};
    j.a = work + bl.dsmall; j.a_bytes = 1024; j.a_nat = 1; j.mt_a = 1; j.split_n = 1;
    j.b_acc = st_h(7); j.b_acc_bytes = 16384; j.nt_acc = 8; j.ones = 1; j.bias_nat_col = -1;
    j.w_off = kWSigma; j.w_ld = 256; j.o_row0 = 3; j.o_valid = 1; j.acc_valid = 256; j.bias_off = kBSigma; j.kind = 4;
    add(j);
  }
  {
    WgradJob j{};
    j.a = work + bl.dhv; j.a_bytes = 8192; j.mt_a = 4;
    j.b_acc = stash + sl.feat; j.b_acc_bytes = 16384; j.nt_acc = 8;
    j.b_nat = denc; j.b_nat_bytes = 2048; j.nt_nat = 1; j.nat_valid = 27; j.nat_col0 = 256; j.bias_nat_col = 27;
    j.w_off = kWView; j.w_ld = 283; j.o_valid = 128; j.acc_valid = 256; j.bias_off = kBView; j.kind = 3;
    add(j);
  }
  {
    WgradJob j{};
    j.a = work + bl.dsmall; j.a_bytes = 1024; j.a_nat = 1; j.mt_a = 1; j.split_n = 1;
    j.b_acc = stash + sl.hv; j.b_acc_bytes = 8192; j.nt_acc = 4; j.ones = 1; j.bias_nat_col = -1;
    j.w_off = kWRgb; j.w_ld = 128; j.o_row0 = 0; j.o_valid = 3; j.acc_valid = 128; j.bias_off = kBRgb; j.kind = 5;
    add(j);
  }
  if (part != 0) {
    const int lo = part == 1 ? 4 : 0, hi = part == 1 ? nj : 4;
    for (int j = lo; j < hi; ++j) args.jobs[j - lo] = args.jobs[j];
    nj = hi - lo;
  }
  args.n_jobs = nj;
  float* slab = bl.slab_bytes ? reinterpret_cast<float*>(const_cast<char*>(work) + bl.slab) : nullptr;
  return wgrad_launch(args, n, grads, stream, slab, bl.slab_bytes, zero_lo, zero_hi);
}

int nerf::wgrad_launch(WgradArgs& args, int64_t n, float* grads, hipStream_t stream, float* slab, size_t slab_bytes,
                       size_t zero_lo, size_t zero_hi) {
  int nj = args.n_jobs;
  const int overhead = options().wgrad_overhead;
  for (int j = 0; j < nj; ++j) {
    WgradJob& jb = args.jobs[j];
    const int bytes = jb.a_bytes + jb.b_acc_bytes + jb.b_nat_bytes + (jb.a2 ? 1024 : 0);
    jb.cost = bytes + overhead;
    if (args.amax != nullptr) {
      const int nt = jb.nt_acc + jb.nt_nat + jb.ones;
      const int per_simd = jb.split_n ? (jb.nt_acc > 4 ? 3 : 2) : (jb.mt_a > 4 ? 2 : 1) * nt;
      const int t_mfma = (jb.split_n || options().wgrad_k16 ? 32 * 4 : 64) * per_simd, t_dma = bytes * 16 / options().wgrad_bw_x16;
      jb.cost = (t_mfma > t_dma ? t_mfma : t_dma) + options().wgrad_fixed;
    }
  }
  args.wave_tiles = args.amax != nullptr ? (int)((n + 63) / 64) : (int)((n + 31) / 32);
  long long c = 0;
  for (int j = 0; j < nj; ++j) {
    args.jobs[j].cost0 = c;
    c += (long long)args.jobs[j].cost * args.wave_tiles;
  }
  args.total_cost = c;
  args.grads = grads;
  args.debug = options().wgrad_debug;
  args.k16 = options().wgrad_k16;
  if (options().wgrad_only >= 0) {
    const int kind = options().wgrad_only;
    int m = 0;
    for (int j = 0; j < args.n_jobs; ++j) if (args.jobs[j].kind == kind) args.jobs[m++] = args.jobs[j];
    args.n_jobs = m;
    nj = m;
    long long cc = 0;
    for (int j = 0; j < nj; ++j) { args.jobs[j].cost0 = cc; cc += (long long)args.jobs[j].cost * args.wave_tiles; }
    args.total_cost = cc;
  }

  int n_cu = 0;
  if (int rc = device_cu_count(&n_cu); rc != NERF_OK) return rc;
  const bool fp8 = args.amax != nullptr;
  if (int rc = ensure_dynamic_lds(fp8 ? (const void*)mlp_wgrad_kernel<true> : (const void*)mlp_wgrad_kernel<false>, kWgLds + kWgScratch,
                                  "nerf_mlp_bwd (wgrad)"); rc != NERF_OK) return rc;
  bool small = args.amax == nullptr && !options().wgrad_big_only, p4 = false;
  for (int j = 0; j < args.n_jobs; ++j) {
    const WgradJob& jb = args.jobs[j];
    p4 = p4 || (jb.kind >= 10 && jb.kind <= 12);
    small = small && jb.kind >= 6 && jb.a_bytes <= SmallStage::A && jb.b_acc_bytes <= SmallStage::B && jb.b_nat_bytes <= SmallStageP4::N;
  }
  if (p4 && !small) return fail(NERF_EINVAL, "wgrad: Part 4 job kinds run on the small-stage kernel only");
  long long want = (long long)args.wave_tiles * nj / 4;
  if (options().wgrad_grid > 0 && options().wgrad_grid < n_cu) n_cu = options().wgrad_grid;
  int grid = (int)(want < 1 ? 1 : (want > n_cu ? n_cu : want));
  if (small) {
    const long long span = options().wgrad_small_span > 0 ? options().wgrad_small_span : 4;
    const long long cap = (long long)(slab != nullptr ? 1 : (options().wgrad_small_cap > 0 ? options().wgrad_small_cap : 3)) * n_cu;
    const long long want3 = (long long)args.wave_tiles * nj / span;
    grid = (int)(want3 < 1 ? 1 : (want3 > cap ? cap : want3));
  }
  args.slab = nullptr;
  args.slab_accumulate = small ? 1 : 0;
  if (slab != nullptr && args.n_jobs > 0 && args.total_cost > 0) {
    bool ok = true;
    long long off = 0;
    for (int j = 0; j < args.n_jobs && ok; ++j) {
      WgradJob& jb = args.jobs[j];
      const long long j0 = jb.cost0, j1 = jb.cost0 + (long long)jb.cost * args.wave_tiles;
      int first = -1, last = -1, count = 0;
      for (int b = 0; b < grid; ++b) {
        const long long lo = args.total_cost * b / grid, hi = args.total_cost * (b + 1) / grid;
        if (hi <= j0 || lo >= j1) continue;
        const long long a0 = lo > j0 ? lo - j0 : 0, a1 = (hi < j1 ? hi : j1) - j0;
        const int wt0 = (int)((a0 + jb.cost - 1) / jb.cost), wt1 = (int)((a1 + jb.cost - 1) / jb.cost);
        if (wt0 >= wt1) continue;
        if (first < 0) first = b;
        last = b;
        ++count;
      }
      ok = count > 0 && count == last - first + 1;
      jb.part0 = first;
      jb.n_parts = count;
      jb.p_stride = (jb.o_valid * jb.w_ld + jb.o_valid + jb.n2 + 63) / 64 * 64;
      jb.slab_off = off;
      off += (long long)count * jb.p_stride;
    }
    if (ok && (size_t)off * sizeof(float) <= slab_bytes) args.slab = slab;
    if (args.slab != nullptr && small && hipMemsetAsync(slab, 0, (size_t)off * sizeof(float), stream) != hipSuccess)
      return fail(NERF_ELAUNCH, "tiny-MLP wgrad: memset failed");
    if (args.slab == nullptr && small) return fail(NERF_EINVAL, "tiny-MLP wgrad (option \"deterministic\"): partial tiles need %zu bytes, %zu given%s",
                                (size_t)off * sizeof(float), slab_bytes, ok ? "" : " (a job's workgroups are not contiguous)");
  }
  if (args.slab == nullptr && zero_hi > zero_lo &&
      hipMemsetAsync(grads + zero_lo, 0, sizeof(float) * (zero_hi - zero_lo), stream) != hipSuccess)
    return fail(NERF_ELAUNCH, "nerf_mlp_bwd: memset failed");
  if (small) {
    if (p4) hipLaunchKernelGGL(mlp_wgrad_small_kernel<true>, dim3(grid), dim3(512), kWgStages * SmallStageP4::Bytes, stream, args);
    else hipLaunchKernelGGL(mlp_wgrad_small_kernel<false>, dim3(grid), dim3(512), kWgStages * SmallStage::Bytes, stream, args);
    if (args.slab != nullptr) {
      if (int rc = check_launch("tiny-MLP wgrad"); rc != NERF_OK) return rc;
      hipLaunchKernelGGL(wgrad_reduce_kernel, dim3(16, args.n_jobs), dim3(256), 0, stream, args);
      return check_launch("tiny-MLP wgrad (reduce)");
    }
    return check_launch("tiny-MLP wgrad");
  }
  if (fp8) hipLaunchKernelGGL(mlp_wgrad_kernel<true>, dim3(grid), dim3(512), kWgLds + kWgScratch, stream, args);
  else hipLaunchKernelGGL(mlp_wgrad_kernel<false>, dim3(grid), dim3(512), kWgLds + kWgScratch, stream, args);
  if (args.slab != nullptr) {
    if (int rc = check_launch("nerf_mlp_bwd (wgrad)"); rc != NERF_OK) return rc;
    hipLaunchKernelGGL(wgrad_reduce_kernel, dim3(160, args.n_jobs), dim3(256), 0, stream, args);
    return check_launch("nerf_mlp_bwd (wgrad reduce)");
  }
  return check_launch("nerf_mlp_bwd (wgrad)");
}
```

### project-nerf_amd/engine.py

```python
from __future__ import annotations

import os
from typing import Dict, Optional, Tuple

import torch

from . import flat_params, ops
from .flat_engine import LapSlots, ViewSlots, cosine_lr, render_chunks

Tensor = torch.Tensor


def param_shapes():
    return [(k, shape) for k, _, shape in flat_params.nerf_decoder_table("", 63, 27)]


def default_init(seed: int = 0) -> Tensor:
    g = torch.Generator().manual_seed(seed)
    parts, fan_in = [], 1
    for name, shape in param_shapes():
        if name.endswith("weight"):
            fan_in = shape[1]
        parts.append(((torch.rand(shape, generator=g) * 2 - 1) / fan_in ** 0.5).reshape(-1))
    return torch.cat(parts)


def flatten_state_dict(sd: Dict[str, Tensor], prefix: str = "decoder.") -> Tensor:
    return flat_params.flatten(flat_params.nerf_decoder_table(prefix, 63, 27), sd)


def unflatten(flat: Tensor, prefix: str = "decoder.") -> Dict[str, Tensor]:
    return flat_params.unflatten(flat_params.nerf_decoder_table(prefix, 63, 27), flat)


class VanillaNerfEngine:
    def __init__(self, params: Optional[Tensor] = None, device: str = "cuda", lr: float = 5e-4,
                 near: float = 2.0, far: float = 6.0, white_bkgd: bool = True, seed: int = 0,
                 world_size: int = 1, grid_resolution: int = 128, bound: float = 1.5, grid_threshold: float = 0.01):
        self.device = torch.device(device)
        flat = default_init(seed) if params is None else params.detach().float().reshape(-1)
        assert flat.numel() == ops.MLP_PARAM_COUNT
        self.params = flat.to(self.device).contiguous()
        self.exp_avg = torch.zeros_like(self.params)
        self.exp_avg_sq = torch.zeros_like(self.params)
        self.grads = torch.empty_like(self.params)
        self.packed = torch.empty(ops.mlp_packed_bytes(), dtype=torch.uint8, device=self.device)
        self.lr, self.near, self.far = lr, near, far
        self.bg = (torch.ones(3) if white_bkgd else torch.zeros(3)).to(self.device)
        self.step_count = 0
        self.world_size = world_size
        self.grad_scale = torch.full((1,), 1.0 / world_size, device=self.device)
        self._ws: Dict[Tuple[str, int], Tensor] = {}
        self._scalars = torch.zeros(2, 1024, device=self.device)
        self._slots = LapSlots(self._scalars)
        self._infer_stale = False
        self.grid_resolution, self.bound, self.grid_threshold = int(grid_resolution), float(bound), float(grid_threshold)
        self.grid: Optional[Tensor] = None
        self.binary_grid: Optional[Tensor] = None
        self._grid_ws: Dict[Tuple[int, int], Tensor] = {}
        self.seed, self._jitter_counter = int(seed), 0
        self._grid_train_ws: Dict[str, Tensor] = {}
        self.repack()

    def repack(self, training_only: bool = False) -> None:
        ops.mlp_pack(self.params, self.packed, which=1 if training_only else 3)
        self._infer_stale = training_only

    def _inference_weights(self) -> Tensor:
        if self._infer_stale:
            ops.mlp_pack(self.params, self.packed, which=2)
            self._infer_stale = False
        return self.packed

    def state_dict(self, prefix: str = "decoder.") -> Dict[str, Tensor]:
        return {k: v.clone() for k, v in unflatten(self.params, prefix).items()}

    def load_state_dict(self, sd: Dict[str, Tensor], prefix: str = "decoder.") -> None:
        self.params.copy_(flatten_state_dict(sd, prefix).to(self.device))
        self.repack()

    def _buf(self, kind: str, nbytes: int) -> Tensor:
        key = (kind, nbytes)
        if key not in self._ws:
            self._ws[key] = torch.empty(nbytes, dtype=torch.uint8, device=self.device)
        return self._ws[key]

    GRID_SLACK = (1.25, 1 << 20)

    def _grid_buf(self, kind: str, nbytes: int) -> Tensor:
        buf = self._grid_train_ws.get(kind)
        if buf is None or buf.numel() < nbytes:
            buf = None
            self._grid_train_ws.pop(kind, None)
            buf = self._grid_train_ws[kind] = torch.empty(int(nbytes * self.GRID_SLACK[0]) + self.GRID_SLACK[1], dtype=torch.uint8,
                                                          device=self.device)
        return buf

    def prepare_batch(self, rays_o: Tensor, rays_d: Tensor, n_samples: int = 64, u: Optional[Tensor] = None, first_ray: int = 0):
        grid = self._require_grid("prepare_batch")
        jitter = None
        if u is None:
            self._jitter_counter += 1
            jitter = (self.seed, self._jitter_counter)
        return ops.sample_compact_async(rays_o, rays_d, self.near, self.far, n_samples, grid, self.bound, u=u, jitter=jitter,
                                        first_ray=first_ray)

    def _grid_gradients(self, rays_o: Tensor, rays_d: Tensor, target: Tensor, n_samples: int, u, sync_grads, sync_grads_async, mark,
                        prepared) -> Tensor:
        mark = mark or (lambda name: None)
        if prepared is None:
            prepared = self.prepare_batch(rays_o, rays_d, n_samples, u=u)
        z, slots, pts, dirs = prepared.get()
        mark("sample")
        R, n = rays_o.shape[0], pts.shape[0]
        if n == 0:
            self.grads.zero_()
            loss = ((self.bg.expand(R, 3) - target) ** 2).mean()
            mark("fwd")
            mark("loss")
            mark("dgrad")
            if sync_grads_async is not None:
                split = ops._lib.load().nerf_mlp_wgrad_part_split()
                for h in [sync_grads_async(view) for view in (self.grads[split:], self.grads[:split])]:
                    if h is not None:
                        h.wait()
            mark("wgrad")
            if sync_grads is not None:
                sync_grads(self.grads)
            return loss
        stash = self._grid_buf("stash", ops.mlp_stash_bytes(n))
        rgb, sigma = ops.mlp_fwd(self.packed, pts, dirs, None, stash)
        mark("fwd")
        loss, amax = self._slots.take()
        d_rgb, d_sigma, _ = ops.composite_mse_bwd(rgb, sigma, z, rays_d, self.bg, target, loss, slots=slots, amax_accum=amax)
        mark("loss")
        ws = self._grid_buf("bwd", ops.mlp_bwd_workspace_bytes(n))
        if sync_grads_async is not None:
            ops.mlp_bwd_overlapped(self.packed, stash, rgb, sigma, d_rgb, d_sigma, self.grads, ws, sync_grads_async, amax=amax, mark=mark)
        else:
            ops.mlp_bwd(self.packed, stash, rgb, sigma, d_rgb, d_sigma, self.grads, ws, amax=amax, mark=mark)
        mark("wgrad")
        if sync_grads is not None:
            sync_grads(self.grads)
        return LapSlots.keep(loss)

    def compute_gradients(self, rays_o: Tensor, rays_d: Tensor, target: Tensor, n_samples: int = 64,
                   u: Optional[Tensor] = None, sync_grads=None, sync_grads_async=None, mark=None,
                   z: Optional[Tensor] = None, grid: bool = False, prepared=None) -> Tensor:
        if grid or prepared is not None:
            if z is not None:
                raise ValueError("compute_gradients: the grid step draws its own depths (z is for the dense step)")
            return self._grid_gradients(rays_o, rays_d, target, n_samples, u, sync_grads, sync_grads_async, mark, prepared)
        mark = mark or (lambda name: None)
        R = rays_o.shape[0]
        n = R * n_samples
        if z is None:
            if u is None:
                u = torch.rand(R, n_samples, device=self.device)
            z = ops.sample_rays(rays_o, rays_d, self.near, self.far, n_samples, u=u)
            mark("sample")
        stash = self._buf("stash", ops.mlp_stash_bytes(n))
        rgb, sigma = ops.mlp_fwd(self.packed, rays_o, rays_d, z, stash)
        mark("fwd")
        loss, amax = self._slots.take()
        d_rgb, d_sigma, _ = ops.composite_mse_bwd(rgb.view(R, n_samples, 3), sigma.view(R, n_samples), z, rays_d, self.bg,
                                                  target, loss, amax_accum=amax)
        mark("loss")
        if sync_grads_async is not None:
            ops.mlp_bwd_overlapped(self.packed, stash, rgb, sigma, d_rgb.view(n, 3), d_sigma.view(n), self.grads,
                                   self._buf("bwd", ops.mlp_bwd_workspace_bytes(n)), sync_grads_async, amax=amax, mark=mark)
        else:
            ops.mlp_bwd(self.packed, stash, rgb, sigma, d_rgb.view(n, 3), d_sigma.view(n), self.grads,
                        self._buf("bwd", ops.mlp_bwd_workspace_bytes(n)), amax=amax, mark=mark)
        mark("wgrad")
        if sync_grads is not None:
            sync_grads(self.grads)
        return LapSlots.keep(loss)

    def apply_gradients(self) -> None:
        self.step_count += 1
        ops.adam_step(self.params, self.grads, self.exp_avg, self.exp_avg_sq, self.step_count, self.lr,
                      grad_scale=self.grad_scale if self.world_size > 1 else None)
        self.repack(training_only=True)

    def train_step(self, rays_o: Tensor, rays_d: Tensor, target: Tensor, n_samples: int = 64,
                   u: Optional[Tensor] = None, sync_grads=None, sync_grads_async=None, mark=None,
                   z: Optional[Tensor] = None, grid: bool = False, prepared=None) -> Tensor:
        loss = self.compute_gradients(rays_o, rays_d, target, n_samples, u=u, sync_grads=sync_grads,
                                      sync_grads_async=sync_grads_async, mark=mark, z=z, grid=grid, prepared=prepared)
        self.apply_gradients()
        if mark is not None:
            mark("adam+pack")
        return loss

    @torch.no_grad()
    def render_rays(self, rays_o: Tensor, rays_d: Tensor, n_samples: int, u: Optional[Tensor] = None):
        z = ops.sample_rays(rays_o, rays_d, self.near, self.far, n_samples, u=u)
        rgb, sigma = ops.mlp_fwd(self._inference_weights(), rays_o, rays_d, z)
        R = rays_o.shape[0]
        c, depth, acc, _, _ = ops.composite_fwd(rgb.view(R, n_samples, 3), sigma.view(R, n_samples), z, rays_d, self.bg)
        return c, depth, acc

    @torch.no_grad()
    def render_rays_hierarchical(self, rays_o: Tensor, rays_d: Tensor, n_coarse: int, n_fine: int):
        R = rays_o.shape[0]
        z = ops.sample_rays(rays_o, rays_d, self.near, self.far, n_coarse)
        rgb, sigma = ops.mlp_fwd(self._inference_weights(), rays_o, rays_d, z)
        w = ops.composite_fwd(rgb.view(R, n_coarse, 3), sigma.view(R, n_coarse), z, rays_d, self.bg, want_weights=True)[4]
        z_all = ops.sample_pdf(z, w, n_fine)
        S = n_coarse + n_fine
        rgb, sigma = ops.mlp_fwd(self._inference_weights(), rays_o, rays_d, z_all)
        c, depth, acc, _, _ = ops.composite_fwd(rgb.view(R, S, 3), sigma.view(R, S), z_all, rays_d, self.bg)
        return c, depth, acc

    @torch.no_grad()
    def update_grid(self) -> float:
        res = self.grid_resolution
        pts = ops.grid_lattice(self.bound, res, self.device)
        sig = torch.empty(res ** 3, device=self.device)
        zeros = torch.zeros(2 ** 18, 3, device=self.device)
        packed = self._inference_weights()
        for i in range(0, pts.shape[0], 2 ** 18):
            p = pts[i:i + 2 ** 18]
            sig[i:i + 2 ** 18] = ops.mlp_fwd(packed, p, zeros[:p.shape[0]], None)[1]
        binary, ratio = ops.grid_threshold(sig.view(res, res, res), self.grid_threshold)
        if ratio <= 0.0:
            return 0.0
        self.grid, self.binary_grid = sig.view(res, res, res), binary
        return ratio

    def _require_grid(self, what: str) -> Tensor:
        if self.binary_grid is None:
            raise ValueError(f"{what}: no occupancy grid (call update_grid() or set binary_grid first)")
        return self.binary_grid

    @torch.no_grad()
    def render_rays_grid(self, rays_o: Tensor, rays_d: Tensor, n_samples: int):
        grid = self._require_grid("render_rays_grid")
        z, slots, pts, dirs = ops.sample_compact(rays_o, rays_d, self.near, self.far, n_samples, grid, self.bound)
        R = rays_o.shape[0]
        if pts.shape[0] == 0:
            bg = self.bg.expand(R, 3).clone() if self.bg.dim() == 1 else self.bg.clone()
            return bg, torch.zeros(R, device=self.device), torch.zeros(R, device=self.device)
        rgb, sigma = ops.mlp_fwd(self._inference_weights(), pts, dirs, None)
        return ops.composite_indexed(rgb, sigma, slots, z, rays_d, self.bg)

    def _render_image_grid_chain(self, rays_o: Tensor, rays_d: Tensor, n_samples: int, chunk: int) -> Tensor:
        grid = self._require_grid("render_image(grid=True)")
        shape = rays_o.shape[:-1]
        o, d = rays_o.reshape(-1, 3).contiguous(), rays_d.reshape(-1, 3).contiguous()
        chunk = max(1, min(int(chunk), max(o.shape[0], 1)))
        ws = self._grid_ws.get((chunk, n_samples))
        if ws is None:
            ws = self._grid_ws[(chunk, n_samples)] = torch.empty(ops.render_rays_grid_workspace_bytes(chunk, n_samples), dtype=torch.uint8,
                                                                 device=self.device)
        rgb = ops.render_rays_grid_fwd(self._inference_weights(), grid, self.bound, o, d, n_samples, self.near, self.far, self.bg, chunk,
                                       workspace=ws)[0]
        return rgb.view(*shape, 3)

    @torch.no_grad()
    def render_image(self, rays_o: Tensor, rays_d: Tensor, n_samples: int, chunk: int = 65536, n_fine: int = 0, grid=False) -> Tensor:
        if grid:
            if grid is not True and grid != "loop":
                raise ValueError(f"render_image: grid={grid!r} (False, True or 'loop')")
            if n_fine > 0:
                raise ValueError("render_image: hierarchical sampling (n_fine > 0) is not combined with the occupancy grid")
            self._require_grid(f"render_image(grid={grid!r})")
            if grid is True:
                return self._render_image_grid_chain(rays_o, rays_d, n_samples, chunk)
            return render_chunks(lambda o, d: self.render_rays_grid(o, d, n_samples), rays_o, rays_d, chunk, self.device)
        if n_fine == 0:
            shape = rays_o.shape[:-1]
            o, d = rays_o.reshape(-1, 3), rays_d.reshape(-1, 3)
# ... 318 lines not shown
```

### project-nerf_amd/ops.py

```python
from __future__ import annotations

from typing import Optional, Tuple

import torch

from . import _lib

Tensor = torch.Tensor


def _stream() -> int:
    return torch._C._cuda_getCurrentRawStream(torch._C._cuda_getDevice())


def _dev(t: Tensor, name: str, dtype=torch.float32) -> Tensor:
    if not isinstance(t, Tensor):
        raise TypeError(f"{name}: expected a tensor")
    if t.device.type != "cuda":
        raise _lib.NerfHipError(f"{name} is on {t.device}; the hot path only runs on a HIP device (no CPU fallback)")
    if t.dtype != dtype:
        raise TypeError(f"{name}: expected {dtype}, got {t.dtype}")
    return t if t.is_contiguous() else t.contiguous()


# ... 311 lines not shown
    z_coarse, weights = _dev(z_coarse, "z_coarse"), _dev(weights, "weights")
    R, S = z_coarse.shape
    if u is not None:
        u = _dev(u, "u")
    out = torch.empty(R, S + n_fine, device=z_coarse.device)
    _lib.check(lib.nerf_sample_pdf(_p(z_coarse), _p(weights), _p(u), R, S, n_fine, _p(out), _stream()), "nerf_sample_pdf")
    return out


def grid_lattice(bound: float, resolution: int, device) -> Tensor:
    lib = _lib.load()
    pts = torch.empty(resolution ** 3, 3, device=device, dtype=torch.float32)
    if pts.device.type != "cuda":
        raise _lib.NerfHipError("grid_lattice: the hot path only runs on a HIP device")
    _lib.check(lib.nerf_grid_lattice(float(bound), resolution, _p(pts), _stream()), "nerf_grid_lattice")
    return pts


def grid_threshold(sigma_grid: Tensor, threshold: float, prev: Optional[Tensor] = None, decay: float = 1.0):
    lib = _lib.load()
    cur = _dev(sigma_grid, "sigma_grid")
    grid = cur if prev is None else _dev(prev, "prev")
    binary = torch.empty(cur.shape, device=cur.device, dtype=torch.bool)
    count = torch.zeros(1, device=cur.device, dtype=torch.int64)
    _lib.check(lib.nerf_grid_update(_p(cur), _p(grid), _p(binary), cur.numel(), float(decay),
                                    0 if prev is None else 1, float(threshold), _p(count), _stream()),
               "nerf_grid_update")
    return binary, float(count.item()) / cur.numel()


def fourier_encode(x: Tensor, n_freq: int) -> Tensor:
    lib = _lib.load()
    x = _dev(x, "x")
    n, dim = x.shape
    out = torch.empty(n, dim + 2 * dim * n_freq, device=x.device, dtype=torch.float32)
    _lib.check(lib.nerf_fourier_encode(_p(x), n, dim, n_freq, _p(out), _stream()), "nerf_fourier_encode")
    return out


def composite_fwd(rgb: Tensor, sigma: Tensor, z: Tensor, rays_d: Tensor, bg: Optional[Tensor] = None,
                  extra: Optional[Tensor] = None, want_weights: bool = False):
    lib = _lib.load()
    rgb, sigma, z, rays_d = _dev(rgb, "rgb"), _dev(sigma, "sigma"), _dev(z, "z"), _dev(rays_d, "rays_d")
    R, S = z.shape
    bg = None if bg is None else _dev(bg, "bg")
    bg_rows = _bg_rows(bg)
    out_rgb = torch.empty(R, 3, device=z.device, dtype=torch.float32)
    depth = torch.empty(R, device=z.device, dtype=torch.float32)
    acc = torch.empty(R, device=z.device, dtype=torch.float32)
    extra_map = None
    if extra is not None:
        extra = _dev(extra, "extra")
        extra_map = torch.empty(R, 3, device=z.device, dtype=torch.float32)
    w = torch.empty(R, S, device=z.device, dtype=torch.float32) if want_weights else None
    _lib.check(lib.nerf_composite_fwd(_p(rgb), _p(sigma), _p(z), _p(rays_d), _p(bg), bg_rows, _p(extra),
                                      R, S, _p(out_rgb), _p(depth), _p(acc), _p(extra_map), _p(w), _stream()),
               "nerf_composite_fwd")
    return out_rgb, depth, acc, extra_map, w


def composite_bwd(rgb, sigma, z, rays_d, bg, extra, g_rgb, g_depth, g_acc, g_extra):
    lib = _lib.load()
    rgb, sigma, z, rays_d = _dev(rgb, "rgb"), _dev(sigma, "sigma"), _dev(z, "z"), _dev(rays_d, "rays_d")
    R, S = z.shape
    bg = None if bg is None else _dev(bg, "bg")
    bg_rows = _bg_rows(bg)
    g_rgb = _dev(g_rgb, "g_rgb")
    g_depth = None if g_depth is None else _dev(g_depth, "g_depth")
    g_acc = None if g_acc is None else _dev(g_acc, "g_acc")
    d_rgb = torch.empty(R, S, 3, device=z.device, dtype=torch.float32)
    d_sigma = torch.empty(R, S, device=z.device, dtype=torch.float32)
    d_extra = None
    if extra is not None and g_extra is not None:
        extra, g_extra = _dev(extra, "extra"), _dev(g_extra, "g_extra")
        d_extra = torch.empty(R, S, 3, device=z.device, dtype=torch.float32)
    else:
        extra = g_extra = None
    _lib.check(lib.nerf_composite_bwd(_p(rgb), _p(sigma), _p(z), _p(rays_d), _p(bg), bg_rows, _p(extra),
                                      _p(g_rgb), _p(g_depth), _p(g_acc), _p(g_extra), R, S,
                                      _p(d_rgb), _p(d_sigma), _p(d_extra), _stream()), "nerf_composite_bwd")
    return d_rgb, d_sigma, d_extra


def composite_mse_bwd(rgb: Tensor, sigma: Tensor, z: Tensor, rays_d: Tensor, bg: Optional[Tensor], target: Tensor,
                      loss_accum: Tensor, slots: Optional[Tensor] = None, amax_accum: Optional[Tensor] = None,
                      loss_weight: Optional[float] = None, want_pred: bool = False):
    lib = _lib.load()
    rgb, sigma, z, rays_d, target = _dev(rgb, "rgb"), _dev(sigma, "sigma"), _dev(z, "z"), _dev(rays_d, "rays_d"), _dev(target, "target")
    R, S = z.shape
    bg = None if bg is None else _dev(bg, "bg")
    bg_rows = _bg_rows(bg)
    d_rgb, d_sigma = torch.empty_like(rgb), torch.empty_like(sigma)
    pred = torch.empty(R, 3, device=z.device) if want_pred else None
    w = 1.0 / (3 * R) if loss_weight is None else loss_weight
    _lib.check(lib.nerf_composite_mse_bwd(_p(rgb), _p(sigma), _p(slots), _p(z), _p(rays_d), _p(bg), bg_rows, _p(target), w, R, S,
                                          _p(pred), _p(loss_accum), _p(d_rgb), _p(d_sigma), _p(amax_accum), _p(sum_ws(z.device)), _stream()),
               "nerf_composite_mse_bwd")
    return d_rgb, d_sigma, pred


class _Composite(torch.autograd.Function):

    @staticmethod
    def forward(ctx, rgb, sigma, z, rays_d, bg, extra):
        out_rgb, depth, acc, extra_map, _ = composite_fwd(rgb, sigma, z, rays_d, bg, extra)
        ctx.save_for_backward(rgb, sigma, z, rays_d, bg, extra)
        if extra_map is None:
            extra_map = out_rgb.new_zeros(0)
        return out_rgb, depth, acc, extra_map

    @staticmethod
    def backward(ctx, g_rgb, g_depth, g_acc, g_extra):
        rgb, sigma, z, rays_d, bg, extra = ctx.saved_tensors
        d_rgb, d_sigma, d_extra = composite_bwd(rgb, sigma, z, rays_d, bg, extra, g_rgb.contiguous(),
                                                g_depth.contiguous(), g_acc.contiguous(),
                                                None if extra is None else g_extra.contiguous())
        return d_rgb, d_sigma, None, None, None, d_extra


def composite(rgb: Tensor, sigma: Tensor, z: Tensor, rays_d: Tensor, bg: Optional[Tensor] = None,
              extra: Optional[Tensor] = None):
    out_rgb, depth, acc, extra_map = _Composite.apply(rgb, sigma, z, rays_d, bg, extra)
    return out_rgb, depth, acc, (extra_map if extra is not None else None)


MLP_PARAM_COUNT = 595844


def mlp_packed_bytes() -> int:
    return _lib.load().nerf_mlp_packed_bytes()


def mlp_pack(params: Tensor, packed: Optional[Tensor] = None, which: int = 3) -> Tensor:
    lib = _lib.load()
    params = _dev(params, "params")
    if params.numel() != MLP_PARAM_COUNT:
        raise ValueError(f"params must have {MLP_PARAM_COUNT} elements, got {params.numel()}")
    if packed is None:
        packed = torch.empty(lib.nerf_mlp_packed_bytes(), device=params.device, dtype=torch.uint8)
    _lib.check(lib.nerf_mlp_pack_streams(_p(params), _p(packed), which, _stream()), "nerf_mlp_pack")
    return packed


def mlp_stash_bytes(n: int) -> int:
    return _lib.load().nerf_mlp_stash_bytes(n)


def mlp_fwd(packed: Tensor, rays_o: Tensor, rays_d: Tensor, z: Optional[Tensor],
            stash: Optional[Tensor] = None) -> Tuple[Tensor, Tensor]:
    lib = _lib.load()
    rays_o, rays_d = _dev(rays_o, "rays_o"), _dev(rays_d, "rays_d")
    if z is not None:
        z = _dev(z, "z")
        n, S = z.numel(), z.shape[1]
    else:
        n, S = rays_o.shape[0], 0
    rgb = torch.empty(n, 3, device=rays_o.device, dtype=torch.float32)
    sigma = torch.empty(n, device=rays_o.device, dtype=torch.float32)
    _lib.check(lib.nerf_mlp_fwd(_p(packed), _p(rays_o), _p(rays_d), _p(z), n, S, _p(rgb), _p(sigma),
                                _p(stash), _stream()), "nerf_mlp_fwd")
    return rgb, sigma


def render_rays_fwd(packed: Tensor, rays_o: Tensor, rays_d: Tensor, n_samples: int, near: float, far: float,
                    bg: Optional[Tensor] = None, chunk: int = 65536, workspace: Optional[Tensor] = None):
    lib = _lib.load()
    rays_o, rays_d = _dev(rays_o, "rays_o"), _dev(rays_d, "rays_d")
    R = rays_o.shape[0]
    chunk = max(1, min(chunk, max(R, 1)))
    need = lib.nerf_render_rays_workspace_bytes(chunk, n_samples)
    if workspace is None or workspace.numel() < need:
        workspace = torch.empty(need, device=rays_o.device, dtype=torch.uint8)
    bg = None if bg is None else _dev(bg, "bg")
    bg_rows = _bg_rows(bg)
    out = torch.empty(R, 3, device=rays_o.device)
    depth, acc = torch.empty(R, device=rays_o.device), torch.empty(R, device=rays_o.device)
    _lib.check(lib.nerf_render_rays_fwd(_p(packed), _p(rays_o), _p(rays_d), R, n_samples, float(near), float(far), _p(bg), bg_rows,
                                        chunk, _p(workspace), _p(out), _p(depth), _p(acc), _stream()), "nerf_render_rays_fwd")
    return out, depth, acc


def render_rays_grid_workspace_bytes(chunk: int, n_samples: int) -> int:
    return _lib.load().nerf_render_rays_grid_workspace_bytes(chunk, n_samples)


def render_rays_grid_fwd(packed: Tensor, binary_grid: Tensor, grid_bound: float, rays_o: Tensor, rays_d: Tensor, n_samples: int,
                         near: float, far: float, bg: Optional[Tensor] = None, chunk: int = 65536, workspace: Optional[Tensor] = None):
    lib = _lib.load()
    rays_o, rays_d = _dev(rays_o, "rays_o"), _dev(rays_d, "rays_d")
    grid = _dev(binary_grid, "binary_grid", torch.bool)
    packed = _dev(packed, "packed", torch.uint8)
    R = rays_o.shape[0]
    chunk = max(1, min(int(chunk), max(R, 1)))
    need = lib.nerf_render_rays_grid_workspace_bytes(chunk, n_samples)
    if workspace is None:
        workspace = torch.empty(need, device=rays_o.device, dtype=torch.uint8)
    elif _dev(workspace, "workspace", torch.uint8).numel() < need:
        raise ValueError(f"render_rays_grid_fwd: workspace of {workspace.numel()} bytes, {need} needed for chunk {chunk} x {n_samples}")
    bg = None if bg is None else _dev(bg, "bg")
    out = torch.empty(R, 3, device=rays_o.device)
    depth, acc = torch.empty(R, device=rays_o.device), torch.empty(R, device=rays_o.device)
    _lib.check(lib.nerf_render_rays_grid_fwd(_p(packed), _p(grid), grid.shape[0], float(grid_bound), _p(rays_o), _p(rays_d), R, n_samples,
                                             float(near), float(far), _p(bg), _bg_rows(bg), chunk, _p(workspace), _p(out), _p(depth),
                                             _p(acc), _stream()), "nerf_render_rays_grid_fwd")
    return out, depth, acc


def mlp_bwd_workspace_bytes(n: int) -> int:
    return _lib.load().nerf_mlp_bwd_workspace_bytes(n)


def mlp_bwd(packed: Tensor, stash: Tensor, rgb: Tensor, sigma: Tensor, d_rgb: Tensor, d_sigma: Tensor,
            grads: Optional[Tensor] = None, workspace: Optional[Tensor] = None, amax: Optional[Tensor] = None,
            mark=None) -> Tensor:
    lib = _lib.load()
    rgb, sigma = _dev(rgb, "rgb"), _dev(sigma, "sigma")
    d_rgb, d_sigma = _dev(d_rgb, "d_rgb"), _dev(d_sigma, "d_sigma")
    n = sigma.numel()
    if grads is None:
        grads = torch.empty(MLP_PARAM_COUNT, device=rgb.device, dtype=torch.float32)
    if workspace is None:
        workspace = torch.empty(lib.nerf_mlp_bwd_workspace_bytes(n), device=rgb.device, dtype=torch.uint8)
    if amax is None:
        _lib.check(lib.nerf_mlp_bwd(_p(packed), _p(stash), _p(rgb), _p(sigma), _p(d_rgb), _p(d_sigma), n,
                                    _p(grads), _p(workspace), _stream()), "nerf_mlp_bwd")
    else:
        _lib.check(lib.nerf_mlp_bwd_dgrad_ex(_p(packed), _p(stash), _p(rgb), _p(sigma), _p(d_rgb), _p(d_sigma), n,
                                             _p(workspace), _p(amax), _stream()), "nerf_mlp_bwd_dgrad_ex")
        if mark is not None:
            mark("dgrad")
        _lib.check(lib.nerf_mlp_bwd_wgrad(_p(stash), _p(workspace), n, _p(grads), _stream()), "nerf_mlp_bwd_wgrad")
    return grads


def mlp_bwd_overlapped(packed: Tensor, stash: Tensor, rgb: Tensor, sigma: Tensor, d_rgb: Tensor, d_sigma: Tensor,
                       grads: Tensor, workspace: Tensor, reduce_async, amax: Optional[Tensor] = None, mark=None) -> None:
    lib = _lib.load()
    n = sigma.numel()
    _lib.check(lib.nerf_mlp_bwd_dgrad_ex(_p(packed), _p(stash), _p(rgb), _p(sigma), _p(d_rgb), _p(d_sigma), n,
                                         _p(workspace), _p(amax), _stream()), "nerf_mlp_bwd_dgrad")
    if mark is not None:
        mark("dgrad")
    split = lib.nerf_mlp_wgrad_part_split()
    handles = []
    for part, view in ((1, grads[split:]), (2, grads[:split])):
        _lib.check(lib.nerf_mlp_bwd_wgrad_part(_p(stash), _p(workspace), n, _p(grads), part, _stream()),
                   "nerf_mlp_bwd_wgrad_part")
        handles.append(reduce_async(view))
    for h in handles:
        if h is not None:
            h.wait()


class _Decoder(torch.autograd.Function):

    @staticmethod
    def forward(ctx, params, packed, rays_o, rays_d, z):
        n = z.numel() if z is not None else rays_o.shape[0]
        stash = torch.empty(mlp_stash_bytes(n), device=params.device, dtype=torch.uint8)
        rgb, sigma = mlp_fwd(packed, rays_o, rays_d, z, stash)
        ctx.save_for_backward(packed, stash, rgb, sigma)
        return rgb, sigma

    @staticmethod
    def backward(ctx, d_rgb, d_sigma):
        packed, stash, rgb, sigma = ctx.saved_tensors
        grads = mlp_bwd(packed, stash, rgb, sigma, d_rgb.contiguous(), d_sigma.contiguous())
        return grads, None, None, None, None


class _DecoderEncoded(torch.autograd.Function):

    @staticmethod
    def forward(ctx, params, packed, x_enc, d_enc, train):
        lib = _lib.load()
        n = x_enc.shape[0]
        rgb = torch.empty(n, 3, device=x_enc.device)
        sigma = torch.empty(n, device=x_enc.device)
        stash = torch.empty(mlp_stash_bytes(n), device=x_enc.device, dtype=torch.uint8) if train else None
        _lib.check(lib.nerf_mlp_fwd_encoded(_p(packed), _p(x_enc), _p(d_enc), n, _p(rgb), _p(sigma), _p(stash), _stream()),
                   "nerf_mlp_fwd_encoded")
        if train:
            ctx.save_for_backward(packed, stash, rgb, sigma)
        return rgb, sigma

    @staticmethod
    def backward(ctx, d_rgb, d_sigma):
        packed, stash, rgb, sigma = ctx.saved_tensors
        return mlp_bwd(packed, stash, rgb, sigma, d_rgb.contiguous(), d_sigma.contiguous()), None, None, None, None


def decoder_encoded(params: Tensor, packed: Tensor, x_enc: Tensor, d_enc: Tensor):
    x_enc, d_enc = _dev(x_enc, "x_enc"), _dev(d_enc, "d_enc")
    if x_enc.shape[1] != 63 or d_enc.shape[1] != 27 or x_enc.shape[0] != d_enc.shape[0]:
        raise ValueError(f"expected x_enc [n,63] and d_enc [n,27], got {tuple(x_enc.shape)} and {tuple(d_enc.shape)}")
    if x_enc.requires_grad or d_enc.requires_grad:
        raise NotImplementedError("gradients w.r.t. the Fourier codes are not produced (positions are not trainable)")
    if x_enc.shape[0] == 0:
        return x_enc.new_zeros(0, 3), x_enc.new_zeros(0)
    train = torch.is_grad_enabled() and params.requires_grad
    return _DecoderEncoded.apply(params, packed, x_enc, d_enc, train)


def decoder(params: Tensor, packed: Tensor, rays_o: Tensor, rays_d: Tensor, z: Optional[Tensor]):
    if torch.is_grad_enabled() and params.requires_grad:
        return _Decoder.apply(params, packed, rays_o, rays_d, z)
    return mlp_fwd(packed, rays_o, rays_d, z)


import ctypes as _ct
import math as _math

import numpy as _np


# ... 375 lines not shown
```

Measured before the change: 3.940 million rays/s.

## Fuse wgrad tile reduction, Adam and bf16 repack into a single step-tail pass

Adds a step-tail path for single-GPU training. The wgrad kernel keeps its per-tile partials in a descriptor, and one tail kernel then reduces them, applies Adam and scatters the updated parameters straight into the packed bf16 layout through a precomputed scatter table. The separate Adam and pack launches go away. The composite MSE backward also gains a last-block ticket reduction, so the loss sums finish inside the kernel without a separate sums launch. The cost is atomics and fences in the loss kernel, plus a more intricate scatter/reduce path that has to stay consistent with the packed layout.

Measured after the change: 3.947 million rays/s (median of 6 runs). Within noise of the previous version (+0.2%).

```diff
diff --git a/include/nerf_hip.h b/include/nerf_hip.h
--- a/include/nerf_hip.h
+++ b/include/nerf_hip.h
@@ -13,7 +13,7 @@
 #define NERF_ELAUNCH (-5)
 #define NERF_ENOSYS (-38)
 
-#define NERF_ABI_VERSION 11
+#define NERF_ABI_VERSION 12
 
 typedef void* nerf_stream_t;
 
@@ -152,6 +152,17 @@
                             nerf_stream_t stream);
 int nerf_mlp_bwd_wgrad(const void* stash, const void* workspace, int64_t n, float* grads_f32,
                        nerf_stream_t stream);
+
+size_t nerf_mlp_step_tail_desc_bytes(void);
+int nerf_mlp_bwd_wgrad_tiles(const void* stash, const void* workspace, int64_t n, float* grads_f32, void* tail_desc,
+                             nerf_stream_t stream);
+int nerf_mlp_step_tail_pending(const void* tail_desc);
+int nerf_mlp_step_tail(void* tail_desc, float* params, float* exp_avg, float* exp_avg_sq, int64_t n_params, int step,
+                       float lr, float beta1, float beta2, float eps, float weight_decay, const int* scatter_table,
+                       void* packed, nerf_stream_t stream);
+size_t nerf_mlp_scatter_table_bytes(void);
+int nerf_mlp_scatter_table(int* scatter_table, nerf_stream_t stream);
+int nerf_mlp_scatter_params(const float* params_f32, const int* scatter_table, void* packed, nerf_stream_t stream);
 
 int nerf_hash_encode_fwd(const float* pts, int64_t n, const float* table, int n_levels,
                          const float* scale_host, const unsigned* res_host, const unsigned* size_host,
@@ -279,6 +290,12 @@
                            const float* rays_d, const float* bg, int64_t bg_rows, const float* target,
                            float loss_weight, int64_t n_rays, int n_samples, float* pred_out, float* loss_accum,
                            float* d_rgb, float* d_sigma, float* amax_accum, float* sum_ws, nerf_stream_t stream);
+#define NERF_TICKET_WORDS 33
+int nerf_composite_mse_bwd_ticket(const float* rgb, const float* sigma, const int* slot_of_sample, const float* z,
+                                  const float* rays_d, const float* bg, int64_t bg_rows, const float* target,
+                                  float loss_weight, int64_t n_rays, int n_samples, float* pred_out, float* loss_accum,
+                                  float* d_rgb, float* d_sigma, float* amax_accum, float* sum_ws, unsigned* ticket,
+                                  float* loss_copy, nerf_stream_t stream);
 int nerf_composite_mse_reg_bwd(const float* rgb, const float* sigma, const int* slot_of_sample, const float* z,
                                const float* rays_d, const float* bg, int64_t bg_rows, const float* target,
                                float loss_weight, const float* extra, float reg_weight, int64_t n_rays, int n_samples,
diff --git a/project-nerf_amd/_lib.py b/project-nerf_amd/_lib.py
--- a/project-nerf_amd/_lib.py
+++ b/project-nerf_amd/_lib.py
@@ -69,6 +69,15 @@
                                      c_ptr, c_ptr, c_ptr, c_ptr, c_ptr]),
     "nerf_mlp_wgrad_part_split": (i64, []),
     "nerf_mlp_bwd_wgrad_part": (i32, [c_ptr, c_ptr, i64, c_ptr, i32, c_ptr]),
+    "nerf_mlp_step_tail_desc_bytes": (size_t, []),
+    "nerf_mlp_bwd_wgrad_tiles": (i32, [c_ptr, c_ptr, i64, c_ptr, c_ptr, c_ptr]),
+    "nerf_mlp_step_tail_pending": (i32, [c_ptr]),
+    "nerf_mlp_step_tail": (i32, [c_ptr, c_ptr, c_ptr, c_ptr, i64, i32, f32, f32, f32, f32, f32, c_ptr, c_ptr, c_ptr]),
+    "nerf_mlp_scatter_table_bytes": (size_t, []),
+    "nerf_mlp_scatter_table": (i32, [c_ptr, c_ptr]),
+    "nerf_mlp_scatter_params": (i32, [c_ptr, c_ptr, c_ptr, c_ptr]),
+    "nerf_composite_mse_bwd_ticket": (i32, [c_ptr, c_ptr, c_ptr, c_ptr, c_ptr, c_ptr, i64, c_ptr, f32, i64, i32, c_ptr, c_ptr,
+                                            c_ptr, c_ptr, c_ptr, c_ptr, c_ptr, c_ptr, c_ptr]),
     "nerf_hash_encode_fwd": (i32, [c_ptr, i64, c_ptr, i32, c_ptr, c_ptr, c_ptr, c_ptr, c_ptr, f32, c_ptr, c_ptr, c_ptr, c_ptr]),
     "nerf_hash_encode_fwd_f16": (i32, [c_ptr, i64, c_ptr, i32, c_ptr, c_ptr, c_ptr, c_ptr, c_ptr, f32, c_ptr, c_ptr, c_ptr]),
     "nerf_hash_encode_fwd_nat": (i32, [c_ptr, i64, c_ptr, c_ptr, i32, c_ptr, c_ptr, c_ptr, c_ptr, c_ptr, f32, c_ptr, i32, c_ptr]),
@@ -166,7 +175,7 @@
     "nerf_adamw_clip_step_shadow": (i32, [c_ptr, c_ptr, c_ptr, c_ptr, i64, i32, f32, f32, f32, f32, f32, c_ptr, f32, f32, c_ptr, c_ptr]),
 }
 
-ABI_VERSION = 11
+ABI_VERSION = 12
 
 _lib = None
 
diff --git a/project-nerf_amd/csrc/adam.hip b/project-nerf_amd/csrc/adam.hip
--- a/project-nerf_amd/csrc/adam.hip
+++ b/project-nerf_amd/csrc/adam.hip
@@ -1,19 +1,9 @@
 #include "common.h"
+#include "step_tail.h"
 
 namespace nerf {
 
 typedef float f4 __attribute__((ext_vector_type(4)));
-
-__device__ __forceinline__ void adam_update(float& p, float g, float& m, float& v, float lr, float beta1, float beta2,
-                                            float eps, float wd, float inv_bc1, float inv_sqrt_bc2) {
-  float pi = p;
-  if (wd != 0.0f) pi *= (1.0f - lr * wd);
-  const float mi = beta1 * m + (1.0f - beta1) * g;
-  const float vi = beta2 * v + (1.0f - beta2) * g * g;
-  m = mi;
-  v = vi;
-  p = pi - (lr * inv_bc1) * (mi / (sqrtf(vi) * inv_sqrt_bc2 + eps));
-}
 
 template <bool VEC>
 __device__ __forceinline__ void adam_sweep(float* __restrict__ p, const float* __restrict__ g, float* __restrict__ m,
diff --git a/project-nerf_amd/csrc/api.cpp b/project-nerf_amd/csrc/api.cpp
--- a/project-nerf_amd/csrc/api.cpp
+++ b/project-nerf_amd/csrc/api.cpp
@@ -28,6 +28,7 @@
     {"hash_bwd_only_level", "NERF_HASH_BWD_ONLY_LEVEL", &Options::hash_bwd_only_level},
     {"hash_bwd_atomic", "NERF_HASH_BWD_ATOMIC", &Options::hash_bwd_atomic},
     {"wgrad_atomic", "NERF_WGRAD_ATOMIC", &Options::wgrad_atomic},
+    {"step_tail", "NERF_STEP_TAIL", &Options::step_tail},
     {"wgrad_k16", "NERF_WGRAD_K16", &Options::wgrad_k16},
     {"wgrad_big_only", "NERF_WGRAD_BIG_ONLY", &Options::wgrad_big_only},
     {"infer_shape32", "NERF_INFER_SHAPE32", &Options::infer_shape32},
diff --git a/project-nerf_amd/csrc/common.h b/project-nerf_amd/csrc/common.h
--- a/project-nerf_amd/csrc/common.h
+++ b/project-nerf_amd/csrc/common.h
@@ -33,6 +33,7 @@
   int wgrad_big_only = 0;
   int wgrad_k16 = 0;
   int wgrad_atomic = 0;
+  int step_tail = 1;
   int hash_bwd_atomic = 0;
   int infer_shape32 = 0;
   int infer64 = 1;
diff --git a/project-nerf_amd/csrc/composite.hip b/project-nerf_amd/csrc/composite.hip
--- a/project-nerf_amd/csrc/composite.hip
+++ b/project-nerf_amd/csrc/composite.hip
@@ -201,6 +201,34 @@
   }
 }
 
+template <bool FENCED>
+__device__ __forceinline__ void composite_sums_body(const float* ws, int n_blocks, float* __restrict__ loss_out, float* __restrict__ reg_out,
+                                                    float* __restrict__ amax_out, float* __restrict__ loss_copy) {
+  __shared__ float part[3][4];
+  auto at = [ws](int i) {
+    return FENCED ? __uint_as_float(atomicOr(reinterpret_cast<unsigned*>(const_cast<float*>(ws)) + i, 0u)) : ws[i];
+  };
+  float s0 = 0.0f, s1 = 0.0f, m = 0.0f;
+  for (int b = threadIdx.x; b < n_blocks; b += 256) {
+    s0 += at(b);
+    s1 += at(n_blocks + b);
+    const float v = at(2 * n_blocks + b);
+    if (v == v && v < 3.0e38f) m = fmaxf(m, v);
+  }
+  s0 = wave_sum(s0);
+  s1 = wave_sum(s1);
+#pragma unroll
+  for (int off = 32; off > 0; off >>= 1) m = fmaxf(m, __shfl_xor(m, off));
+  if ((threadIdx.x & 63) == 0) { part[0][threadIdx.x >> 6] = s0; part[1][threadIdx.x >> 6] = s1; part[2][threadIdx.x >> 6] = m; }
+  __syncthreads();
+  if (threadIdx.x == 0) {
+    *loss_out += (part[0][0] + part[0][1]) + (part[0][2] + part[0][3]);
+    if (loss_copy != nullptr) *loss_copy = *loss_out;
+    if (reg_out != nullptr) *reg_out += (part[1][0] + part[1][1]) + (part[1][2] + part[1][3]);
+    if (amax_out != nullptr) *amax_out = fmaxf(*amax_out, fmaxf(fmaxf(part[2][0], part[2][1]), fmaxf(part[2][2], part[2][3])));
+  }
+}
+
 template <int K>
 __global__ void __launch_bounds__(256)
 composite_mse_bwd_kernel(const float* __restrict__ rgb, const float* __restrict__ sigma, const float* __restrict__ z,
@@ -209,7 +237,8 @@
                          float* __restrict__ pred_out, float* __restrict__ loss_out, float* __restrict__ d_rgb,
                          float* __restrict__ d_sigma, float* __restrict__ amax_out,
                          const float* __restrict__ extra, float reg_weight, float* __restrict__ d_extra,
-                         float* __restrict__ reg_out, float* __restrict__ extra_map, unsigned* __restrict__ sum_ws) {
+                         float* __restrict__ reg_out, float* __restrict__ extra_map, unsigned* __restrict__ sum_ws,
+                         unsigned* __restrict__ ticket, float* __restrict__ loss_copy) {
   const int lane = threadIdx.x & 63;
   const int64_t wave = (blockIdx.x * (int64_t)blockDim.x + threadIdx.x) >> 6;
   const int64_t nwave = ((int64_t)gridDim.x * blockDim.x) >> 6;
@@ -312,12 +341,41 @@
   if (lane == 0) { part[threadIdx.x >> 6] = loss_local; part[4 + (threadIdx.x >> 6)] = amax; part[8 + (threadIdx.x >> 6)] = reg_local; }
   __syncthreads();
   if (sum_ws != nullptr) {
+    const float p_loss = (part[0] + part[1]) + (part[2] + part[3]), p_reg = (part[8] + part[9]) + (part[10] + part[11]),
+                p_max = fmaxf(fmaxf(part[4], part[5]), fmaxf(part[6], part[7]));
+    if (ticket == nullptr) {
+      if (threadIdx.x == 0) {
+        float* ws = reinterpret_cast<float*>(sum_ws);
+        ws[blockIdx.x] = p_loss;
+        ws[gridDim.x + blockIdx.x] = p_reg;
+        ws[2 * gridDim.x + blockIdx.x] = p_max;
+      }
+      return;
+    }
+    __syncthreads();
     if (threadIdx.x == 0) {
-      float* ws = reinterpret_cast<float*>(sum_ws);
-      ws[blockIdx.x] = (part[0] + part[1]) + (part[2] + part[3]);
-      ws[gridDim.x + blockIdx.x] = (part[8] + part[9]) + (part[10] + part[11]);
-      ws[2 * gridDim.x + blockIdx.x] = fmaxf(fmaxf(part[4], part[5]), fmaxf(part[6], part[7]));
-    }
+      const unsigned B = gridDim.x;
+      unsigned seen = atomicExch(&sum_ws[blockIdx.x], __float_as_uint(p_loss));
+      seen |= atomicExch(&sum_ws[B + blockIdx.x], __float_as_uint(p_reg));
+      seen |= atomicExch(&sum_ws[2 * B + blockIdx.x], __float_as_uint(p_max));
+      asm volatile("" ::"v"(seen) : "memory");
+      const unsigned g = blockIdx.x % kOrderedSumGroups, in_group = (B - g + kOrderedSumGroups - 1) / kOrderedSumGroups;
+      bool last = false;
+      if (atomicAdd(&ticket[1 + g], 1u) == in_group - 1) {
+        atomicExch(&ticket[1 + g], 0u);
+        const unsigned groups = B < (unsigned)kOrderedSumGroups ? B : (unsigned)kOrderedSumGroups;
+        last = atomicAdd(&ticket[0], 1u) == groups - 1;
+      }
+      if (last) {
+        __builtin_amdgcn_fence(__ATOMIC_ACQUIRE, "agent");
+        asm volatile("s_waitcnt vmcnt(0)" ::: "memory");
+      }
+      part[0] = last ? 1.0f : 0.0f;
+    }
+    __syncthreads();
+    if (part[0] == 0.0f) return;
+    composite_sums_body<true>(reinterpret_cast<const float*>(sum_ws), (int)gridDim.x, loss_out, reg_out, amax_out, loss_copy);
+    if (threadIdx.x == 0) atomicExch(&ticket[0], 0u);
     return;
   }
   if (threadIdx.x == 0) {
@@ -332,25 +390,7 @@
 
 __global__ void __launch_bounds__(256) composite_sums_kernel(const float* __restrict__ ws, int n_blocks, float* __restrict__ loss_out,
                                                              float* __restrict__ reg_out, float* __restrict__ amax_out) {
-  __shared__ float part[3][4];
-  float s0 = 0.0f, s1 = 0.0f, m = 0.0f;
-  for (int b = threadIdx.x; b < n_blocks; b += 256) {
-    s0 += ws[b];
-    s1 += ws[n_blocks + b];
-    const float v = ws[2 * n_blocks + b];
-    if (v == v && v < 3.0e38f) m = fmaxf(m, v);
-  }
-  s0 = wave_sum(s0);
-  s1 = wave_sum(s1);
-#pragma unroll
-  for (int off = 32; off > 0; off >>= 1) m = fmaxf(m, __shfl_xor(m, off));
-  if ((threadIdx.x & 63) == 0) { part[0][threadIdx.x >> 6] = s0; part[1][threadIdx.x >> 6] = s1; part[2][threadIdx.x >> 6] = m; }
-  __syncthreads();
-  if (threadIdx.x == 0) {
-    *loss_out += (part[0][0] + part[0][1]) + (part[0][2] + part[0][3]);
-    if (reg_out != nullptr) *reg_out += (part[1][0] + part[1][1]) + (part[1][2] + part[1][3]);
-    if (amax_out != nullptr) *amax_out = fmaxf(*amax_out, fmaxf(fmaxf(part[2][0], part[2][1]), fmaxf(part[2][2], part[2][3])));
-  }
+  composite_sums_body<false>(ws, n_blocks, loss_out, reg_out, amax_out, nullptr);
 }
 
 static int per_lane(int S) {
@@ -480,9 +520,30 @@
   const dim3 grid((unsigned)mse_blocks(n_rays, sum_ws != nullptr));
   DISPATCH_K(per_lane(n_samples), composite_mse_bwd_kernel, rgb, sigma, z, rays_d, bg, bg_rows, target, loss_weight,
              slot_of_sample, n_rays, n_samples, pred_out, loss_accum, d_rgb, d_sigma, amax_accum,
-             (const float*)nullptr, 0.0f, (float*)nullptr, (float*)nullptr, (float*)nullptr, reinterpret_cast<unsigned*>(sum_ws));
+             (const float*)nullptr, 0.0f, (float*)nullptr, (float*)nullptr, (float*)nullptr, reinterpret_cast<unsigned*>(sum_ws),
+             (unsigned*)nullptr, (float*)nullptr);
   if (int rc = check_launch("nerf_composite_mse_bwd"); rc != NERF_OK) return rc;
   return finish_sums(sum_ws, grid.x, loss_accum, nullptr, amax_accum, stream);
+}
+
+static_assert(NERF_TICKET_WORDS == kOrderedSumTickets, "include/nerf_hip.h");
+extern "C" int nerf_composite_mse_bwd_ticket(const float* rgb, const float* sigma, const int* slot_of_sample, const float* z,
+                                             const float* rays_d, const float* bg, int64_t bg_rows, const float* target,
+                                             float loss_weight, int64_t n_rays, int n_samples, float* pred_out, float* loss_accum,
+                                             float* d_rgb, float* d_sigma, float* amax_accum, float* sum_ws, unsigned* ticket,
+                                             float* loss_copy, nerf_stream_t stream) {
+  NERF_REQUIRE(n_rays >= 0 && n_samples >= 1 && n_samples <= 64 * kMaxPerLane,
+               "nerf_composite_mse_bwd_ticket: n_rays=%lld n_samples=%d (max %d)", (long long)n_rays, n_samples, 64 * kMaxPerLane);
+  NERF_REQUIRE(sum_ws != nullptr && ticket != nullptr, "nerf_composite_mse_bwd_ticket: sum_ws and ticket are required");
+  if (n_rays == 0) return NERF_OK;
+  NERF_REQUIRE(rgb && sigma && z && rays_d && target && loss_accum && d_rgb && d_sigma, "nerf_composite_mse_bwd_ticket: NULL pointer");
+  NERF_REQUIRE(bg == nullptr || bg_rows == 1 || bg_rows == n_rays, "nerf_composite_mse_bwd_ticket: bg_rows=%lld", (long long)bg_rows);
+  const dim3 grid((unsigned)mse_blocks(n_rays, true));
+  DISPATCH_K(per_lane(n_samples), composite_mse_bwd_kernel, rgb, sigma, z, rays_d, bg, bg_rows, target, loss_weight,
+             slot_of_sample, n_rays, n_samples, pred_out, loss_accum, d_rgb, d_sigma, amax_accum,
+             (const float*)nullptr, 0.0f, (float*)nullptr, (float*)nullptr, (float*)nullptr, reinterpret_cast<unsigned*>(sum_ws),
+             ticket, loss_copy);
+  return check_launch("nerf_composite_mse_bwd_ticket");
 }
 
 extern "C" int nerf_composite_mse_reg_bwd(const float* rgb, const float* sigma, const int* slot_of_sample, const float* z,
@@ -499,7 +560,7 @@
   const dim3 grid((unsigned)mse_blocks(n_rays, sum_ws != nullptr));
   DISPATCH_K(per_lane(n_samples), composite_mse_bwd_kernel, rgb, sigma, z, rays_d, bg, bg_rows, target, loss_weight,
              slot_of_sample, n_rays, n_samples, pred_out, loss_accum, d_rgb, d_sigma, (float*)nullptr, extra, reg_weight, d_extra,
-             reg_accum, extra_map, reinterpret_cast<unsigned*>(sum_ws));
+             reg_accum, extra_map, reinterpret_cast<unsigned*>(sum_ws), (unsigned*)nullptr, (float*)nullptr);
   if (int rc = check_launch("nerf_composite_mse_reg_bwd"); rc != NERF_OK) return rc;
   return finish_sums(sum_ws, grid.x, loss_accum, reg_accum, nullptr, stream);
 }
diff --git a/project-nerf_amd/csrc/mlp_bwd.hip b/project-nerf_amd/csrc/mlp_bwd.hip
--- a/project-nerf_amd/csrc/mlp_bwd.hip
+++ b/project-nerf_amd/csrc/mlp_bwd.hip
@@ -117,10 +117,12 @@
 
 }
 
+namespace nerf { struct StepTailDesc; }
 using namespace nerf;
 
 int nerf_launch_wgrad(const char* stash, const StashLayout& sl, const char* work, const BwdLayout& bl,
-                      int64_t n, float* grads, int part, hipStream_t stream, size_t zero_lo, size_t zero_hi);
+                      int64_t n, float* grads, int part, hipStream_t stream, size_t zero_lo, size_t zero_hi,
+                      StepTailDesc* keep_tiles = nullptr);
 
 extern "C" size_t nerf_mlp_bwd_workspace_bytes(int64_t n) { return n > 0 ? bwd_layout(n).total : 0; }
 
diff --git a/project-nerf_amd/csrc/mlp_pack.hip b/project-nerf_amd/csrc/mlp_pack.hip
--- a/project-nerf_amd/csrc/mlp_pack.hip
+++ b/project-nerf_amd/csrc/mlp_pack.hip
@@ -1,5 +1,6 @@
 #include "common.h"
 #include "mlp_plan.h"
+#include "step_tail.h"
 
 namespace nerf {
 using namespace plan;
@@ -66,9 +67,12 @@
   }
 }
 
-__global__ void __launch_bounds__(256)
-pack_kernel(const float* __restrict__ params, __bf16* __restrict__ packed_fwd,
-            __bf16* __restrict__ packed_bwd, float* __restrict__ bias) {
+template <bool TABLE>
+__device__ __forceinline__ void pack_walk(const float* __restrict__ params, __bf16* __restrict__ packed_fwd,
+                                          __bf16* __restrict__ packed_bwd, float* __restrict__ bias, int* __restrict__ table) {
+  auto claim = [table](int entry, int value) {
+    if (atomicCAS(&table[entry], kScatterNone, value) != kScatterNone) atomicAdd(&table[2 * kParamCount], 1);
+  };
   const int total = (kFwdFrags + kBwdFrags) * 64;
   for (int t = blockIdx.x * blockDim.x + threadIdx.x; t < total; t += gridDim.x * blockDim.x) {
     const int frag = t >> 6, lane = t & 63;
@@ -83,21 +87,54 @@
     for (int j = 0; j < 8; ++j) {
       const int k = frag_column(nat ? ks - st.ks_acc : ks, h, j, nat);
       const int src = src_index(kind, row, k, nat);
-      out[j] = (__bf16)(src >= 0 ? params[src] : 0.0f);
+      if constexpr (TABLE) {
+        const size_t at = (frag < kFwdFrags ? kPackFwdOff + (size_t)frag * 1024 : kPackBwdOff + (size_t)(frag - kFwdFrags) * 1024) + lane * 16 + j * 2;
+        if (src >= 0) claim(2 * src + (frag < kFwdFrags ? 0 : 1), (int)at);
+      } else {
+        out[j] = (__bf16)(src >= 0 ? params[src] : 0.0f);
+      }
     }
-    __bf16* dst = frag < kFwdFrags ? packed_fwd + (size_t)frag * 512 : packed_bwd + (size_t)(frag - kFwdFrags) * 512;
-    *reinterpret_cast<bf16x8*>(dst + lane * 8) = out;
+    if constexpr (!TABLE) {
+      __bf16* dst = frag < kFwdFrags ? packed_fwd + (size_t)frag * 512 : packed_bwd + (size_t)(frag - kFwdFrags) * 512;
+      *reinterpret_cast<bf16x8*>(dst + lane * 8) = out;
+    }
   }
   for (int i = blockIdx.x * blockDim.x + threadIdx.x; i < kBiasFloats; i += gridDim.x * blockDim.x) {
     float b = 0.0f;
-    if (i < 2048) b = params[pts_bias_off(i >> 8) + (i & 255)];
-    else if (i < 2048 + 288) { const int r = i - 2048; b = r < 256 ? params[kBFeat + r] : (r == 256 ? params[kBSigma] : 0.0f); }
-    else if (i < 2048 + 288 + 128) b = params[kBView + (i - 2048 - 288)];
-    else { const int r = i - 2048 - 288 - 128; b = r < 3 ? params[kBRgb + r] : 0.0f; }
-    bias[i] = b;
+    int src = -1;
+    auto take = [&](int at) {
+      if constexpr (TABLE) { src = at; return 0.0f; } else return params[at];
+    };
+    if (i < 2048) b = take(pts_bias_off(i >> 8) + (i & 255));
+    else if (i < 2048 + 288) { const int r = i - 2048; b = r < 256 ? take(kBFeat + r) : (r == 256 ? take(kBSigma) : 0.0f); }
+    else if (i < 2048 + 288 + 128) b = take(kBView + (i - 2048 - 288));
+    else { const int r = i - 2048 - 288 - 128; b = r < 3 ? take(kBRgb + r) : 0.0f; }
+    if constexpr (TABLE) {
+      if (src >= 0) {
+        claim(2 * src, (int)(kPackBiasOff + (size_t)i * 4));
+        claim(2 * src + 1, kScatterBias);
+      }
+    } else {
+      bias[i] = b;
+    }
   }
 }
 
+__global__ void __launch_bounds__(256)
+pack_kernel(const float* __restrict__ params, __bf16* __restrict__ packed_fwd,
+            __bf16* __restrict__ packed_bwd, float* __restrict__ bias) {
+  pack_walk<false>(params, packed_fwd, packed_bwd, bias, nullptr);
+}
+
+__global__ void __launch_bounds__(256) scatter_table_kernel(int* __restrict__ table) {
+  pack_walk<true>(nullptr, nullptr, nullptr, nullptr, table);
+}
+
+__global__ void __launch_bounds__(256) scatter_params_kernel(const float* __restrict__ params, const int* __restrict__ table,
+                                                             char* __restrict__ packed) {
+  for (int i = blockIdx.x * blockDim.x + threadIdx.x; i < kParamCount; i += gridDim.x * blockDim.x)
+    scatter_param(params[i], table[2 * i], table[2 * i + 1], packed);
+}
 }
 
 extern "C" size_t nerf_mlp_packed_bytes(void) { return nerf::plan::kPackBytes; }
@@ -122,3 +159,24 @@
 extern "C" int nerf_mlp_pack(const float* params_f32, void* packed, nerf_stream_t stream) {
   return nerf_mlp_pack_streams(params_f32, packed, 3, stream);
 }
+
+extern "C" size_t nerf_mlp_scatter_table_bytes(void) { return nerf::kScatterInts * sizeof(int); }
+
+extern "C" int nerf_mlp_scatter_table(int* table, nerf_stream_t stream) {
+  using namespace nerf;
+  NERF_REQUIRE(table != nullptr && ((uintptr_t)table & 3) == 0, "nerf_mlp_scatter_table: NULL or unaligned table");
+  static_assert(plan::kPackBiasOff + plan::kBiasFloats * 4 < ((size_t)1 << 31), "packed positions fit an int32");
+  if (hipMemsetAsync(table, 0xFF, 2 * (size_t)plan::kParamCount * sizeof(int), as_stream(stream)) != hipSuccess ||
+      hipMemsetAsync(table + 2 * (size_t)plan::kParamCount, 0, sizeof(int), as_stream(stream)) != hipSuccess)
+    return fail(NERF_ELAUNCH, "nerf_mlp_scatter_table: memset failed");
+  hipLaunchKernelGGL(scatter_table_kernel, dim3(512), dim3(256), 0, as_stream(stream), table);
+  return check_launch("nerf_mlp_scatter_table");
+}
+
+extern "C" int nerf_mlp_scatter_params(const float* params_f32, const int* table, void* packed, nerf_stream_t stream) {
+  using namespace nerf;
+  NERF_REQUIRE(params_f32 && table && packed, "nerf_mlp_scatter_params: NULL pointer");
+  NERF_REQUIRE(((uintptr_t)packed & 255) == 0, "nerf_mlp_scatter_params: packed buffer must be 256-byte aligned");
+  hipLaunchKernelGGL(scatter_params_kernel, dim3(512), dim3(256), 0, as_stream(stream), params_f32, table, static_cast<char*>(packed));
+  return check_launch("nerf_mlp_scatter_params");
+}
diff --git a/project-nerf_amd/csrc/mlp_wgrad.h b/project-nerf_amd/csrc/mlp_wgrad.h
--- a/project-nerf_amd/csrc/mlp_wgrad.h
+++ b/project-nerf_amd/csrc/mlp_wgrad.h
@@ -68,7 +68,11 @@
   { WgradJob j = make_job(w, o.dsmall, 1024, 1, o.hc2, 2, 0, 0, 9); j.a_nat = 1; j.split_n = 1; j.w_off = c3; j.w_ld = 64; j.o_valid = 3; j.acc_valid = 64; wa.jobs[4] = j; }
 }
 
+struct StepTailDesc {
+  int pending, reserved;
+  WgradArgs args;
+};
 int wgrad_launch(WgradArgs& args, int64_t n_samples, float* grads, hipStream_t stream, float* slab = nullptr,
-                 size_t slab_bytes = 0, size_t zero_lo = 0, size_t zero_hi = 0);
+                 size_t slab_bytes = 0, size_t zero_lo = 0, size_t zero_hi = 0, StepTailDesc* keep_tiles = nullptr);
 
 }
diff --git a/project-nerf_amd/csrc/mlp_wgrad.hip b/project-nerf_amd/csrc/mlp_wgrad.hip
--- a/project-nerf_amd/csrc/mlp_wgrad.hip
+++ b/project-nerf_amd/csrc/mlp_wgrad.hip
@@ -2,6 +2,7 @@
 #include "mlp_chain.h"
 #include "mlp_stash.h"
 #include "mlp_wgrad.h"
+#include "step_tail.h"
 
 namespace nerf {
 using namespace plan;
@@ -643,35 +644,70 @@
   }
 }
 
+__device__ __forceinline__ float tile_sum(const float* __restrict__ tile, const WgradJob& job, int i) {
+  float s0 = 0.0f, s1 = 0.0f, s2 = 0.0f, s3 = 0.0f;
+  int t = 0;
+  for (; t + 4 <= job.n_parts; t += 4) {
+    s0 += tile[(long long)(t + 0) * job.p_stride + i];
+    s1 += tile[(long long)(t + 1) * job.p_stride + i];
+    s2 += tile[(long long)(t + 2) * job.p_stride + i];
+    s3 += tile[(long long)(t + 3) * job.p_stride + i];
+  }
+  for (; t < job.n_parts; ++t) s0 += tile[(long long)t * job.p_stride + i];
+  return (s0 + s1) + (s2 + s3);
+}
+
+__device__ __forceinline__ int tile_param(const WgradJob& job, int i, int n_w, int n_b, int n_all) {
+  return i < n_w ? job.w_off + i
+       : i < n_b ? ((job.ones || job.bias_nat_col >= 0) ? job.bias_off + (i - n_w) : -1)
+       : i < n_all - 1 ? job.w2_off + (i - n_b)
+                       : job.bias2_off;
+}
+
 __global__ void __launch_bounds__(256) wgrad_reduce_kernel(const WgradArgs args) {
   const WgradJob& job = args.jobs[blockIdx.y];
   const int n_w = job.o_valid * job.w_ld, n_b = n_w + job.o_valid, n_all = n_b + job.n2;
   const float* tile = args.slab + job.slab_off;
   for (int i = blockIdx.x * blockDim.x + threadIdx.x; i < n_all; i += gridDim.x * blockDim.x) {
-    float s0 = 0.0f, s1 = 0.0f, s2 = 0.0f, s3 = 0.0f;
-    int t = 0;
-    for (; t + 4 <= job.n_parts; t += 4) {
-      s0 += tile[(long long)(t + 0) * job.p_stride + i];
-      s1 += tile[(long long)(t + 1) * job.p_stride + i];
-      s2 += tile[(long long)(t + 2) * job.p_stride + i];
-      s3 += tile[(long long)(t + 3) * job.p_stride + i];
-    }
-    for (; t < job.n_parts; ++t) s0 += tile[(long long)t * job.p_stride + i];
-    const float sum = (s0 + s1) + (s2 + s3);
-    float* dst = i < n_w ? args.grads + job.w_off + i
-               : i < n_b ? ((job.ones || job.bias_nat_col >= 0) ? args.grads + job.bias_off + (i - n_w) : nullptr)
-               : i < n_all - 1 ? args.grads + job.w2_off + (i - n_b)
-                               : args.grads + job.bias2_off;
+    const float sum = tile_sum(tile, job, i);
+    const int at = tile_param(job, i, n_w, n_b, n_all);
+    float* dst = at >= 0 ? args.grads + at : nullptr;
     if (dst != nullptr) *dst = args.slab_accumulate ? *dst + sum : sum;
   }
 }
 
+struct StepTail {
+  float* params; float* exp_avg; float* exp_avg_sq;
+  const int* scatter;
+  char* packed;
+  float lr, beta1, beta2, eps, wd, inv_bc1, inv_sqrt_bc2;
+  float gs;
+};
+__global__ void __launch_bounds__(256) step_tail_kernel(const WgradArgs args, const StepTail a) {
+  const WgradJob& job = args.jobs[blockIdx.y];
+  const int n_w = job.o_valid * job.w_ld, n_b = n_w + job.o_valid, n_all = n_b + job.n2;
+  const float* tile = args.slab + job.slab_off;
+  for (int i = blockIdx.x * blockDim.x + threadIdx.x; i < n_all; i += gridDim.x * blockDim.x) {
+    const int at = tile_param(job, i, n_w, n_b, n_all);
+    if (at < 0) continue;
+    float p = a.params[at], m = a.exp_avg[at], v = a.exp_avg_sq[at];
+    const int fwd = a.scatter[2 * at], bwd = a.scatter[2 * at + 1];
+    const float sum = tile_sum(tile, job, i);
+    args.grads[at] = sum;
+    adam_update(p, sum * a.gs, m, v, a.lr, a.beta1, a.beta2, a.eps, a.wd, a.inv_bc1, a.inv_sqrt_bc2);
+    a.exp_avg[at] = m;
+    a.exp_avg_sq[at] = v;
+    a.params[at] = p;
+    scatter_param(p, fwd, bwd, a.packed);
+  }
+}
+
 }
 
 using namespace nerf;
 
 int nerf_launch_wgrad(const char* stash, const StashLayout& sl, const char* work, const BwdLayout& bl,
-                      int64_t n, float* grads, int part, hipStream_t stream, size_t zero_lo, size_t zero_hi) {
+                      int64_t n, float* grads, int part, hipStream_t stream, size_t zero_lo, size_t zero_hi, StepTailDesc* keep_tiles) {
   WgradArgs args{};
   const size_t np = (size_t)sl.n_pad, eb = sl.fp8 ? 1 : 2;
   if (sl.fp8 != bl.fp8) return fail(NERF_EINVAL, "nerf_mlp_bwd: stash and workspace disagree on the image width");
@@ -745,12 +781,13 @@
   }
   args.n_jobs = nj;
   float* slab = bl.slab_bytes ? reinterpret_cast<float*>(const_cast<char*>(work) + bl.slab) : nullptr;
-  return wgrad_launch(args, n, grads, stream, slab, bl.slab_bytes, zero_lo, zero_hi);
+  return wgrad_launch(args, n, grads, stream, slab, bl.slab_bytes, zero_lo, zero_hi, keep_tiles);
 }
 
 int nerf::wgrad_launch(WgradArgs& args, int64_t n, float* grads, hipStream_t stream, float* slab, size_t slab_bytes,
-                       size_t zero_lo, size_t zero_hi) {
+                       size_t zero_lo, size_t zero_hi, StepTailDesc* keep_tiles) {
   int nj = args.n_jobs;
+  if (keep_tiles != nullptr) keep_tiles->pending = 0;
   const int overhead = options().wgrad_overhead;
   for (int j = 0; j < nj; ++j) {
     WgradJob& jb = args.jobs[j];
@@ -854,8 +891,58 @@
   else hipLaunchKernelGGL(mlp_wgrad_kernel<false>, dim3(grid), dim3(512), kWgLds + kWgScratch, stream, args);
   if (args.slab != nullptr) {
     if (int rc = check_launch("nerf_mlp_bwd (wgrad)"); rc != NERF_OK) return rc;
+    if (keep_tiles != nullptr) {
+      keep_tiles->args = args;
+      keep_tiles->pending = 1;
+      return NERF_OK;
+    }
     hipLaunchKernelGGL(wgrad_reduce_kernel, dim3(160, args.n_jobs), dim3(256), 0, stream, args);
     return check_launch("nerf_mlp_bwd (wgrad reduce)");
   }
   return check_launch("nerf_mlp_bwd (wgrad)");
 }
+
+extern "C" size_t nerf_mlp_step_tail_desc_bytes(void) { return sizeof(StepTailDesc); }
+
+extern "C" int nerf_mlp_step_tail_pending(const void* tail_desc) {
+  return tail_desc != nullptr && static_cast<const StepTailDesc*>(tail_desc)->pending == 1 ? 1 : 0;
+}
+
+extern "C" int nerf_mlp_bwd_wgrad_tiles(const void* stash, const void* workspace, int64_t n, float* grads_f32, void* tail_desc,
+                                        nerf_stream_t stream) {
+  NERF_REQUIRE(n > 0 && n < (int64_t)1 << 31, "nerf_mlp_bwd_wgrad_tiles: n=%lld out of range", (long long)n);
+  NERF_REQUIRE(stash && workspace && grads_f32 && tail_desc, "nerf_mlp_bwd_wgrad_tiles: NULL pointer");
+  NERF_REQUIRE(((uintptr_t)tail_desc & 7) == 0, "nerf_mlp_bwd_wgrad_tiles: tail_desc must be 8-byte aligned");
+  StepTailDesc* desc = static_cast<StepTailDesc*>(tail_desc);
+  desc->pending = 0;
+  if (!options().step_tail)
+    return nerf_launch_wgrad(static_cast<const char*>(stash), stash_layout(n), static_cast<const char*>(workspace), bwd_layout(n), n,
+                             grads_f32, 0, as_stream(stream), 0, (size_t)kParamCount, nullptr);
+  return nerf_launch_wgrad(static_cast<const char*>(stash), stash_layout(n), static_cast<const char*>(workspace), bwd_layout(n), n,
+                           grads_f32, 0, as_stream(stream), 0, (size_t)kParamCount, desc);
+}
+
+extern "C" int nerf_mlp_step_tail(void* tail_desc, float* params, float* exp_avg, float* exp_avg_sq, int64_t n_params, int step,
+                                  float lr, float beta1, float beta2, float eps, float weight_decay, const int* scatter_table,
+                                  void* packed, nerf_stream_t stream) {
+  NERF_REQUIRE(tail_desc != nullptr, "nerf_mlp_step_tail: tail_desc is NULL");
+  StepTailDesc* desc = static_cast<StepTailDesc*>(tail_desc);
+  NERF_REQUIRE(desc->pending == 1, "nerf_mlp_step_tail: no unreduced tiles pending (nerf_mlp_bwd_wgrad_tiles first; it reduces on its own "
+               "below %lld samples and with the options wgrad_atomic on or step_tail off)", (long long)kSlabMinSamples);
+  NERF_REQUIRE(n_params == kParamCount && step >= 1, "nerf_mlp_step_tail: n_params=%lld (%d) step=%d", (long long)n_params, kParamCount, step);
+  NERF_REQUIRE(params && exp_avg && exp_avg_sq && scatter_table && packed, "nerf_mlp_step_tail: NULL pointer");
+  NERF_REQUIRE(((uintptr_t)packed & 255) == 0, "nerf_mlp_step_tail: packed buffer must be 256-byte aligned");
+  const WgradArgs& args = desc->args;
+  NERF_REQUIRE(args.slab != nullptr && args.slab_accumulate == 0 && args.n_jobs > 0 && args.n_jobs <= kMaxJobs,
+               "nerf_mlp_step_tail: descriptor does not hold a decoder launch");
+  const double bc1 = 1.0 - pow((double)beta1, step), bc2 = 1.0 - pow((double)beta2, step);
+  StepTail a{};
+  a.params = params; a.exp_avg = exp_avg; a.exp_avg_sq = exp_avg_sq;
+  a.scatter = scatter_table; a.packed = static_cast<char*>(packed);
+  a.lr = lr; a.beta1 = beta1; a.beta2 = beta2; a.eps = eps; a.wd = weight_decay;
+  a.inv_bc1 = (float)(1.0 / bc1); a.inv_sqrt_bc2 = (float)(1.0 / sqrt(bc2));
+  a.gs = 1.0f;
+  desc->pending = 0;
+  hipLaunchKernelGGL(step_tail_kernel, dim3(160, args.n_jobs), dim3(256), 0, as_stream(stream), args, a);
+  return check_launch("nerf_mlp_step_tail");
+}
diff --git a/project-nerf_amd/csrc/step_tail.h b/project-nerf_amd/csrc/step_tail.h
--- /dev/null
+++ b/project-nerf_amd/csrc/step_tail.h
@@ -0,0 +1,31 @@
+#pragma once
+#include "common.h"
+#include "mlp_plan.h"
+
+namespace nerf {
+
+__device__ __forceinline__ void adam_update(float& p, float g, float& m, float& v, float lr, float beta1, float beta2,
+                                            float eps, float wd, float inv_bc1, float inv_sqrt_bc2) {
+  float pi = p;
+  if (wd != 0.0f) pi *= (1.0f - lr * wd);
+  const float mi = beta1 * m + (1.0f - beta1) * g;
+  const float vi = beta2 * v + (1.0f - beta2) * g * g;
+  m = mi;
+  v = vi;
+  p = pi - (lr * inv_bc1) * (mi / (sqrtf(vi) * inv_sqrt_bc2 + eps));
+}
+
+constexpr int kScatterNone = -1, kScatterBias = -2;
+constexpr size_t kScatterInts = 2 * (size_t)plan::kParamCount + 1;
+
+__device__ __forceinline__ void scatter_param(float p, int fwd, int bwd, char* __restrict__ packed) {
+  if (bwd == kScatterBias) {
+    *reinterpret_cast<float*>(packed + fwd) = p;
+    return;
+  }
+  const __bf16 b = (__bf16)p;
+  if (fwd >= 0) *reinterpret_cast<__bf16*>(packed + fwd) = b;
+  if (bwd >= 0) *reinterpret_cast<__bf16*>(packed + bwd) = b;
+}
+
+}
diff --git a/project-nerf_amd/engine.py b/project-nerf_amd/engine.py
--- a/project-nerf_amd/engine.py
+++ b/project-nerf_amd/engine.py
@@ -54,6 +54,10 @@
         self._scalars = torch.zeros(2, 1024, device=self.device)
         self._slots = LapSlots(self._scalars)
         self._infer_stale = False
+        self._ticket = torch.zeros(ops.TICKET_WORDS, dtype=torch.int32, device=self.device)
+        self._tail_desc = ops.step_tail_desc()
+        if world_size == 1:
+            ops.mlp_scatter_table(self.device)
         self.grid_resolution, self.bound, self.grid_threshold = int(grid_resolution), float(bound), float(grid_threshold)
         self.grid: Optional[Tensor] = None
         self.binary_grid: Optional[Tensor] = None
@@ -146,7 +150,7 @@
 
     def compute_gradients(self, rays_o: Tensor, rays_d: Tensor, target: Tensor, n_samples: int = 64,
                    u: Optional[Tensor] = None, sync_grads=None, sync_grads_async=None, mark=None,
-                   z: Optional[Tensor] = None, grid: bool = False, prepared=None) -> Tensor:
+                   z: Optional[Tensor] = None, grid: bool = False, prepared=None, _defer_reduce: bool = False) -> Tensor:
         if grid or prepared is not None:
             if z is not None:
                 raise ValueError("compute_gradients: the grid step draws its own depths (z is for the dense step)")
@@ -163,19 +167,22 @@
         rgb, sigma = ops.mlp_fwd(self.packed, rays_o, rays_d, z, stash)
         mark("fwd")
         loss, amax = self._slots.take()
+        ticket = self._ticket if ops._lib.get_option("step_tail") else None
+        kept = torch.empty((), device=self.device) if ticket is not None else None
         d_rgb, d_sigma, _ = ops.composite_mse_bwd(rgb.view(R, n_samples, 3), sigma.view(R, n_samples), z, rays_d, self.bg,
-                                                  target, loss, amax_accum=amax)
+                                                  target, loss, amax_accum=amax, ticket=ticket, loss_copy=kept)
         mark("loss")
         if sync_grads_async is not None:
             ops.mlp_bwd_overlapped(self.packed, stash, rgb, sigma, d_rgb.view(n, 3), d_sigma.view(n), self.grads,
                                    self._buf("bwd", ops.mlp_bwd_workspace_bytes(n)), sync_grads_async, amax=amax, mark=mark)
         else:
             ops.mlp_bwd(self.packed, stash, rgb, sigma, d_rgb.view(n, 3), d_sigma.view(n), self.grads,
-                        self._buf("bwd", ops.mlp_bwd_workspace_bytes(n)), amax=amax, mark=mark)
+                        self._buf("bwd", ops.mlp_bwd_workspace_bytes(n)), amax=amax, mark=mark,
+                        tail_desc=self._tail_desc if _defer_reduce else None)
         mark("wgrad")
         if sync_grads is not None:
             sync_grads(self.grads)
-        return LapSlots.keep(loss)
+        return kept if kept is not None else LapSlots.keep(loss)
 
     def apply_gradients(self) -> None:
         self.step_count += 1
@@ -186,9 +193,16 @@
     def train_step(self, rays_o: Tensor, rays_d: Tensor, target: Tensor, n_samples: int = 64,
                    u: Optional[Tensor] = None, sync_grads=None, sync_grads_async=None, mark=None,
                    z: Optional[Tensor] = None, grid: bool = False, prepared=None) -> Tensor:
+        fused = not grid and prepared is None and self.world_size == 1 and sync_grads is None and sync_grads_async is None
         loss = self.compute_gradients(rays_o, rays_d, target, n_samples, u=u, sync_grads=sync_grads,
-                                      sync_grads_async=sync_grads_async, mark=mark, z=z, grid=grid, prepared=prepared)
-        self.apply_gradients()
+                                      sync_grads_async=sync_grads_async, mark=mark, z=z, grid=grid, prepared=prepared,
+                                      _defer_reduce=fused)
+        if fused and ops.step_tail_pending(self._tail_desc):
+            self.step_count += 1
+            ops.mlp_step_tail(self._tail_desc, self.params, self.exp_avg, self.exp_avg_sq, self.step_count, self.lr, self.packed)
+            self._infer_stale = True
+        else:
+            self.apply_gradients()
         if mark is not None:
             mark("adam+pack")
         return loss
diff --git a/project-nerf_amd/ops.py b/project-nerf_amd/ops.py
--- a/project-nerf_amd/ops.py
+++ b/project-nerf_amd/ops.py
@@ -417,9 +417,13 @@
     return d_rgb, d_sigma, d_extra
 
 
+TICKET_WORDS = 33
+
+
 def composite_mse_bwd(rgb: Tensor, sigma: Tensor, z: Tensor, rays_d: Tensor, bg: Optional[Tensor], target: Tensor,
                       loss_accum: Tensor, slots: Optional[Tensor] = None, amax_accum: Optional[Tensor] = None,
-                      loss_weight: Optional[float] = None, want_pred: bool = False):
+                      loss_weight: Optional[float] = None, want_pred: bool = False, ticket: Optional[Tensor] = None,
+                      loss_copy: Optional[Tensor] = None):
     lib = _lib.load()
     rgb, sigma, z, rays_d, target = _dev(rgb, "rgb"), _dev(sigma, "sigma"), _dev(z, "z"), _dev(rays_d, "rays_d"), _dev(target, "target")
     R, S = z.shape
@@ -428,6 +432,13 @@
     d_rgb, d_sigma = torch.empty_like(rgb), torch.empty_like(sigma)
     pred = torch.empty(R, 3, device=z.device) if want_pred else None
     w = 1.0 / (3 * R) if loss_weight is None else loss_weight
+    if ticket is not None:
+        if _dev(ticket, "ticket", torch.int32).numel() < TICKET_WORDS:
+            raise ValueError(f"ticket: {TICKET_WORDS} int32 words needed")
+        _lib.check(lib.nerf_composite_mse_bwd_ticket(_p(rgb), _p(sigma), _p(slots), _p(z), _p(rays_d), _p(bg), bg_rows, _p(target), w, R, S,
+                                                     _p(pred), _p(loss_accum), _p(d_rgb), _p(d_sigma), _p(amax_accum), _p(sum_ws(z.device)),
+                                                     _p(ticket), _p(loss_copy), _stream()), "nerf_composite_mse_bwd_ticket")
+        return d_rgb, d_sigma, pred
     _lib.check(lib.nerf_composite_mse_bwd(_p(rgb), _p(sigma), _p(slots), _p(z), _p(rays_d), _p(bg), bg_rows, _p(target), w, R, S,
                                           _p(pred), _p(loss_accum), _p(d_rgb), _p(d_sigma), _p(amax_accum), _p(sum_ws(z.device)), _stream()),
                "nerf_composite_mse_bwd")
@@ -547,7 +558,7 @@
 
 def mlp_bwd(packed: Tensor, stash: Tensor, rgb: Tensor, sigma: Tensor, d_rgb: Tensor, d_sigma: Tensor,
             grads: Optional[Tensor] = None, workspace: Optional[Tensor] = None, amax: Optional[Tensor] = None,
-            mark=None) -> Tensor:
+            mark=None, tail_desc=None) -> Tensor:
     lib = _lib.load()
     rgb, sigma = _dev(rgb, "rgb"), _dev(sigma, "sigma")
     d_rgb, d_sigma = _dev(d_rgb, "d_rgb"), _dev(d_sigma, "d_sigma")
@@ -564,8 +575,61 @@
                                              _p(workspace), _p(amax), _stream()), "nerf_mlp_bwd_dgrad_ex")
         if mark is not None:
             mark("dgrad")
-        _lib.check(lib.nerf_mlp_bwd_wgrad(_p(stash), _p(workspace), n, _p(grads), _stream()), "nerf_mlp_bwd_wgrad")
+        if tail_desc is not None:
+            _lib.check(lib.nerf_mlp_bwd_wgrad_tiles(_p(stash), _p(workspace), n, _p(grads), tail_desc, _stream()), "nerf_mlp_bwd_wgrad_tiles")
+        else:
+            _lib.check(lib.nerf_mlp_bwd_wgrad(_p(stash), _p(workspace), n, _p(grads), _stream()), "nerf_mlp_bwd_wgrad")
     return grads
+
+
+def step_tail_desc():
+    import ctypes
+    return ctypes.create_string_buffer(_lib.load().nerf_mlp_step_tail_desc_bytes())
+
+
+def step_tail_pending(tail_desc) -> bool:
+    return bool(_lib.load().nerf_mlp_step_tail_pending(tail_desc))
+
+
+_SCATTER_TABLE = {}
+
+
+def mlp_scatter_table(device) -> Tensor:
+    key = torch.device(device)
+    if key.index is None:
+        key = torch.device(key.type, torch.cuda.current_device())
+    if key not in _SCATTER_TABLE:
+        lib = _lib.load()
+        with torch.cuda.device(key):
+            table = torch.empty(lib.nerf_mlp_scatter_table_bytes() // 4, dtype=torch.int32, device=key)
+            _lib.check(lib.nerf_mlp_scatter_table(_p(table), _stream()), "nerf_mlp_scatter_table")
+            host = table.cpu()
+        pairs, clashes = host[:-1].view(-1, 2), int(host[-1])
+        places = pairs[pairs >= 0]
+        if pairs.shape[0] != MLP_PARAM_COUNT or clashes != 0 or bool((pairs[:, 0] < 0).any()) or places.unique().numel() != places.numel() \
+                or bool((pairs[:, 1] < -2).any()) or int(places.max()) + 2 > lib.nerf_mlp_packed_bytes():
+            raise _lib.NerfHipError(f"nerf_mlp_scatter_table: unsound table ({clashes} parameters claimed twice, "
+                                    f"{int((pairs[:, 0] < 0).sum())} without a place, {places.numel() - places.unique().numel()} places shared)")
+        _SCATTER_TABLE[key] = table
+    return _SCATTER_TABLE[key]
+
+
+def mlp_scatter_params(params: Tensor, packed: Tensor) -> None:
+    params = _dev(params, "params")
+    if params.numel() != MLP_PARAM_COUNT:
+        raise ValueError(f"params must have {MLP_PARAM_COUNT} elements, got {params.numel()}")
+    _lib.check(_lib.load().nerf_mlp_scatter_params(_p(params), _p(mlp_scatter_table(params.device)), _p(_dev(packed, "packed", torch.uint8)),
+                                                   _stream()), "nerf_mlp_scatter_params")
+
+
+def mlp_step_tail(tail_desc, params: Tensor, exp_avg: Tensor, exp_avg_sq: Tensor, step: int, lr: float, packed: Tensor,
+                  beta1: float = 0.9, beta2: float = 0.999, eps: float = 1e-8, weight_decay: float = 0.0) -> None:
+    for t, nm in ((params, "params"), (exp_avg, "exp_avg"), (exp_avg_sq, "exp_avg_sq")):
+        if _dev(t, nm) is not t:
+            raise ValueError(f"{nm} must be contiguous")
+    _lib.check(_lib.load().nerf_mlp_step_tail(tail_desc, _p(params), _p(exp_avg), _p(exp_avg_sq), params.numel(), step, lr, beta1, beta2, eps,
+                                              weight_decay, _p(mlp_scatter_table(params.device)), _p(_dev(packed, "packed", torch.uint8)),
+                                              _stream()), "nerf_mlp_step_tail")
 
 
 def mlp_bwd_overlapped(packed: Tensor, stash: Tensor, rgb: Tensor, sigma: Tensor, d_rgb: Tensor, d_sigma: Tensor,
```
